# orange-vertex/depthmapX

Hardware: AMD Instinct MI355X
Metric: grid cells/sec for VISPREP makeGraph + VGA global on N×N grid (higher is better)
Workload: dtype f64

## Files before the change

depthmapx_amd/_native.py:

```python
import ctypes
import os

import numpy as np

_HERE = os.path.dirname(os.path.abspath(__file__))
LIB_PATH = os.environ.get("DMX_LIB") or os.path.join(_HERE, "_lib", "libdmx.so")

DMX_OK = 0
STATUS_NAMES = {-1: "DMX_ERR_ARG", -2: "DMX_ERR_HIP", -3: "DMX_ERR_CAPACITY", -4: "DMX_ERR_STATE",
                -5: "DMX_ERR_UNSUPPORTED", -6: "DMX_ERR_OUTSIDE", -7: "DMX_ERR_CANCELLED"}
PROGRESS_FN = ctypes.CFUNCTYPE(ctypes.c_int32, ctypes.c_void_p, ctypes.c_int32, ctypes.c_int64, ctypes.c_int64)

_vp, _i64, _i32, _dbl, _cs = ctypes.c_void_p, ctypes.c_int64, ctypes.c_int, ctypes.c_double, ctypes.c_char_p
SIGNATURES = {
    "dmx_abi_version": (_i32, []),
    "dmx_last_error": (ctypes.c_char_p, []),
    "dmx_ctx_create": (_i32, [_i32, _vp]),
    "dmx_ctx_free": (_i32, [_vp]),
    "dmx_ctx_last_timing": (_i32, [_vp, _vp, _vp]),
    "dmx_ctx_last_stats": (_i32, [_vp, _vp, _i32]),
    "dmx_pointmap_create": (_i32, [_vp, _dbl, _vp, _i64, _vp]),
    "dmx_pointmap_free": (_i32, [_vp]),
    "dmx_pointmap_fill": (_i32, [_vp, _dbl, _dbl, _vp]),
    "dmx_pointmap_fill_device": (_i32, [_vp, _vp, _dbl, _dbl, _vp]),
    "dmx_pointmap_make_points": (_i32, [_vp, _dbl, _dbl, _i32, _vp]),
    "dmx_graph_special_nodes": (_i32, [_vp, _vp, _vp]),
    "dmx_pointmap_make_points_device": (_i32, [_vp, _vp, _dbl, _dbl, _i32, _vp]),
    "dmx_ctx_last_fill": (_i32, [_vp, _vp, _vp, _vp]),
    "dmx_pointmap_info": (_i32, [_vp, _vp, _vp, _vp, _vp, _vp]),
    "dmx_pointmap_state": (_i32, [_vp, _vp]),
    "dmx_pointmap_cell_lines": (_i32, [_vp, _vp, _vp, _vp]),
    "dmx_makegraph": (_i32, [_vp, _vp, _dbl, _i32, _i64, _i64, _vp]),
    "dmx_makegraph_balance": (_i32, [_vp, _vp, _dbl, _i32, _i32, _i64, _vp]),
    "dmx_graph_free": (_i32, [_vp]),
    "dmx_graph_info": (_i32, [_vp, _vp, _vp, _vp, _vp]),
    "dmx_graph_copy": (_i32, [_vp, _vp, _vp, _vp, _vp]),
    "dmx_graph_copy_range": (_i32, [_vp, _i64, _i64, _vp, _vp, _vp, _i64, _vp, _vp]),
    "dmx_graph_blob_size": (_i32, [_vp, _vp]),
    "dmx_graph_blob_write_device": (_i32, [_vp, _vp, _i64]),
    "dmx_graph_assemble_device": (_i32, [_vp, _vp, _vp, _vp, _i32, _vp]),
    "dmx_vga_global": (_i32, [_vp, _vp, _dbl, _i32, _i64, _i64, _vp, _vp]),
    "dmx_vga_global_device": (_i32, [_vp, _vp, _dbl, _i32, _i64, _i64, _vp]),
    "dmx_metric_stepdepth": (_i32, [_vp, _vp, _vp, _i64, _vp]),
    "dmx_visual_stepdepth": (_i32, [_vp, _vp, _vp, _i64, _vp]),
    "dmx_vga_global_device_list": (_i32, [_vp, _vp, _dbl, _i32, _vp, _i64, _vp]),
    "dmx_graph_set_prep_shard": (_i32, [_vp, _i64, _i64, _vp, _vp]),
    "dmx_vga_local": (_i32, [_vp, _vp, _i32, _i64, _i64, _vp]),
    "dmx_vga_thruvision": (_i32, [_vp, _vp, _i64, _i64, _vp, _vp]),
    "dmx_graph_connections": (_i32, [_vp, _vp, _i64, _i64, _i32, _vp, _vp, _i64, _vp]),
    "dmx_graph_connections_csv": (_i32, [_vp, _vp, _i64, _i64, _cs, _vp, _vp, _i64, _vp]),
    "dmx_ctx_last_connections": (_i32, [_vp, _vp, _vp, _vp]),
    "dmx_agent_schedule": (_i32, [_vp, ctypes.c_uint32, _i32, _dbl, _i32, _vp, _i64, _i32, _vp, _vp, _vp, _i64, _vp]),
    "dmx_agents": (_i32, [_vp, _vp, _i32, _i32, _i64, _vp, _vp, _vp, _vp, _vp, _vp, _vp, _vp, _i64]),
    "dmx_ctx_last_agents": (_i32, [_vp, _vp, _vp]),
    "dmx_ctx_last_agents_detail": (_i32, [_vp, _vp, _vp]),
    "dmx_vga_isovist": (_i32, [_vp, _vp, _i32, _i64, _i64, _vp, _vp, _vp, _vp, _i64, _vp]),
    "dmx_ctx_last_isovist": (_i32, [_vp, _vp, _vp, _vp]),
    "dmx_isovists": (_i32, [_vp, _vp, _i64, _vp, _vp, _vp, _i64, _i32, _vp, _vp, _vp, _i64, _vp]),
    "dmx_chunk_occlusion": (_i32, [_vp, _vp, _vp, _vp, _i64, _vp]),
    "dmx_chunk_set_occlusion": (_i32, [_vp, _vp, _vp, _vp]),
    "dmx_vga_metric": (_i32, [_vp, _vp, _dbl, _i32, _i64, _i64, _vp]),
    "dmx_vga_angular": (_i32, [_vp, _vp, _dbl, _i32, _i64, _i64, _vp]),
    "dmx_angular_stepdepth": (_i32, [_vp, _vp, _vp, _i64, _vp]),
    "dmx_release_cached_memory": (_i32, []),
    "dmx_ctx_set_progress": (_i32, [_vp, PROGRESS_FN, _vp, _dbl]),
    "dmx_ctx_cancel": (_i32, [_vp]),
    "dmx_ctx_last_stepdepth": (_i32, [_vp, _vp, _vp, _vp]),
    "dmx_ctx_last_stepdepth_detail": (_i32, [_vp, _vp]),
    "dmx_ctx_last_stepdepth_attempts": (_i32, [_vp, _vp]),
    "dmx_ctx_last_stepdepth_batched": (_i32, [_vp, _vp]),
    "dmx_ctx_last_phase_cycles": (_i32, [_vp, _vp]),
    "dmx_ctx_last_mk_reruns": (_i32, [_vp, _vp, ctypes.c_int64, _vp]),
    "dmx_chunk_write": (_i32, [_vp, _i64, _vp, _vp, _i64, _vp, _i32, _vp, _vp, _vp, _vp, _i32, _i32, _vp, _i64, _vp]),
    "dmx_pointmap_set_state": (_i32, [_vp, _vp]),
    "dmx_chunk_parse": (_i32, [_vp, _i64, _vp]),
    "dmx_chunk_free": (_i32, [_vp]),
    "dmx_chunk_info": (_i32, [_vp, _vp, _vp, _vp, _vp, _vp, _vp, _vp, _vp, _vp]),
    "dmx_chunk_column": (_i32, [_vp, _i32, _vp, _i32, _vp, _vp]),
    "dmx_chunk_arrays": (_i32, [_vp, _vp, _vp, _vp, _vp]),
    "dmx_chunk_load": (_i32, [_vp, _vp, _vp, _vp, _vp]),
    "dmx_graph_from_runs": (_i32, [_vp, _vp, _i64, _vp, _vp, _i64, _vp, _vp, _vp]),
    "dmx_graph_set_merges": (_i32, [_vp, _vp, _i64]),
    "dmx_graph_set_drawing": (_i32, [_vp, _vp, _i64]),
    "dmx_pointmap_set_merges": (_i32, [_vp, _vp, _i64]),
    "dmx_chunk_merges": (_i32, [_vp, _vp, _vp]),
    "dmx_chunk_rows": (_i32, [_vp, _vp, _vp]),
    "dmx_chunk_merge_records": (_i32, [_vp, _vp, _vp]),
    "dmx_chunk_flags": (_i32, [_vp, _vp, _vp, _vp, _vp]),
    "dmx_chunk_set_column": (_i32, [_vp, _cs, _vp, _vp, _i32, _i32]),
    "dmx_chunk_set_displayed": (_i32, [_vp, _i32]),
    "dmx_chunk_set_name": (_i32, [_vp, _cs]),
    "dmx_chunk_select_cells": (_i32, [_vp, _vp, _i64]),
    "dmx_chunk_unmake": (_i32, [_vp, _i32]),
    "dmx_chunk_serialize": (_i32, [_vp, _vp, _i64, _vp]),
    "dmx_graph_chunk_write": (_i32, [_vp, _cs, _i32, _vp, _vp, _vp, _vp, _i32, _i32, _vp, _i64, _vp]),
    "dmx_chunk_scan": (_i32, [_vp, _i64, _vp, _vp, _vp, _vp, _vp]),
    "dmx_chunk_load_bytes": (_i32, [_vp, _vp, _i64, _vp, _vp, _vp]),
    "dmx_graphfile_read": (_i32, [_cs, _vp]),
    "dmx_graphfile_free": (_i32, [_vp]),
    "dmx_graphfile_write": (_i32, [_vp, _cs]),
    "dmx_graphfile_info": (_i32, [_vp, _vp, _vp, _vp, _vp, _vp, _vp]),
    "dmx_graphfile_lines": (_i32, [_vp, _vp]),
    "dmx_graphfile_set_view": (_i32, [_vp, _i32, _i32]),
    "dmx_graphfile_pointmap": (_i32, [_vp, _i32, _vp, _vp]),
    "dmx_graphfile_put_pointmap": (_i32, [_vp, _i32, _vp, _i64]),
    "dmx_graphfile_new_pointmap_name": (_i32, [_vp, _vp, _i32]),
    "dmx_view_vga_top": (_i32, [_i32]),
}


ALLREDUCE_FN = ctypes.CFUNCTYPE(ctypes.c_int, ctypes.c_void_p, ctypes.c_int64, ctypes.c_int, ctypes.c_void_p)


class DmxError(RuntimeError):
    def __init__(self, status, message):
        super().__init__("%s (%d): %s" % (STATUS_NAMES.get(status, "?"), status, message))
        self.status = status


_lib = None


def _share_hip_runtime_with_torch():
    try:
        import torch
    except Exception:
        pass


def lib():
    global _lib
    if _lib is None:
        _share_hip_runtime_with_torch()
        if not os.path.exists(LIB_PATH):
            raise DmxError(-2, "native library %s is missing: run depthmapx_amd.build.build()" % LIB_PATH)
        L = ctypes.CDLL(LIB_PATH)
        for name, (res, args) in SIGNATURES.items():
            if os.environ.get("DMX_LIB") and not hasattr(L, name):
                continue
            fn = getattr(L, name)
            fn.restype = res
            fn.argtypes = args
        _lib = L
    return _lib


def check(status):
    if status != DMX_OK:
        raise DmxError(status, lib().dmx_last_error().decode(errors="replace"))
    return status


def ptr(a):
    return None if a is None else a.ctypes.data_as(ctypes.c_void_p)
```

depthmapx_amd/csrc/api/vga_global.hip:

```cpp

static void prep_range(const dmx_graph* g, int64_t& b, int64_t& e) {
    b = 0; e = g->nnodes;
    if (g->prep_fn && g->prep_e >= 0) { b = g->prep_b; e = g->prep_e; }
}
static int prep_allreduce(dmx_graph* g, void* p, int64_t count, int dtype) {
    if (!g->prep_fn || count <= 0) return DMX_OK;
    HIPCHK(hipStreamSynchronize(g->ctx->stream));
    if (g->prep_fn(p, count, dtype, g->prep_user) != 0)
        return fail(DMX_ERR_STATE, "prep all-reduce callback failed");
    return DMX_OK;
}
static int prepare_symmetry(dmx_graph* g);
static int build_scan_order(dmx_graph* g);
static int prepare_uf(dmx_graph* g) {
    if (g->scan_ready) return DMX_OK;
    if (int rc = prepare_symmetry(g)) return rc;
    dmx_ctx* ctx = g->ctx;
    hipStream_t s = ctx->stream;
    PointMapHost& h = *g->pm->host;
    const int cols = h.cols(), rows = h.rows();
    const int tw = (cols + 7) / 8, th = (rows + 7) / 8;
    const int64_t C = (int64_t)cols * rows, N = g->nnodes;
    DevBuf<int> cov;
    DevBuf<unsigned long long> cnt;
    HIPCHK(cnt.alloc(1));
    HIPCHK(hipMemsetAsync(cnt.p, 0, 8, s));
    const bool have_uf = g->uf_count >= 0;
    if (!have_uf) {
        HIPCHK(cov.alloc((size_t)4 * C));
        HIPCHK(g->uf_tiles.alloc((size_t)tw * th));
        HIPCHK(g->notuf_tiles.alloc((size_t)tw * th));
        HIPCHK(hipMemsetAsync(cov.p, 0, (size_t)4 * C * 4, s));
        int64_t pb, pe;
        prep_range(g, pb, pe);
        if (pe > pb) {
            hipLaunchKernelGGL(cov_scatter_kernel, dim3((unsigned)std::min<int64_t>(pe - pb, 4096)), dim3(256), 0, s,
                               cols, rows, pe - pb, g->node_run_start.p + pb, g->node_nruns.p + pb, g->pool.p, cov.p);
            HIPCHK(hipGetLastError());
        }
        if (int rc = prep_allreduce(g, cov.p, (int64_t)4 * C, DMX_I32)) return rc;
        hipLaunchKernelGGL(cov_lines_kernel, dim3((cols + rows + 127) / 128, 4), dim3(128), 0, s, cols, rows, cov.p);
        HIPCHK(hipGetLastError());
        hipLaunchKernelGGL(cov_tiles_kernel, dim3((tw * th + 255) / 256), dim3(256), 0, s, cols, rows, tw, th,
                           g->pm->d_cell_node.p, cov.p, g->uf_tiles.p, g->notuf_tiles.p, cnt.p);
        HIPCHK(hipGetLastError());
    }
    unsigned long long ufc = have_uf ? (unsigned long long)g->uf_count : 0ull;
    if (!have_uf) HIPCHK(copy_sync(s, &ufc, cnt.p, 8, hipMemcpyDeviceToHost));
    if (int rc = build_scan_order(g)) return rc;
    g->uf_count = (int64_t)ufc;
    g->scan_ready = true;
    return DMX_OK;
}

static int build_scan_order(dmx_graph* g) {
    dmx_ctx* ctx = g->ctx;
    hipStream_t s = ctx->stream;
    PointMapHost& h = *g->pm->host;
    const int rows = h.rows();
    const int64_t C = (int64_t)h.cols() * rows, N = g->nnodes;
    std::vector<int32_t> nr((size_t)std::max<int64_t>(N, 1));
    if (N) HIPCHK(copy_sync(s, nr.data(), g->node_nruns.p, N * 4, hipMemcpyDeviceToHost));
    std::vector<int64_t> ss((size_t)std::max<int64_t>(N, 1));
    int64_t acc = 0;
    for (int64_t k = 0; k < N; k++) { ss[k] = acc; acc += nr[k]; }
    DevBuf<int64_t>& d_ss = g->scan_start;
    HIPCHK(d_ss.alloc(std::max<int64_t>(N, 1)));
    HIPCHK(g->scan_pool.alloc(std::max<int64_t>(acc, 1)));
    HIPCHK(g->cell_scan_start.alloc(C));
    HIPCHK(g->cell_nruns.alloc(C));
    HIPCHK(hipMemsetAsync(g->cell_nruns.p, 0, C * 4, s));
    if (N) {
        HIPCHK(hipMemcpyAsync(d_ss.p, ss.data(), N * 8, hipMemcpyHostToDevice, s));
        hipLaunchKernelGGL(scan_pool_kernel, dim3((unsigned)std::min<int64_t>(N, 8192)), dim3(256), 0, s, rows,
                           g->pm->d_node_cell.p, N, g->node_run_start.p, g->node_nruns.p, g->bin_nruns.p, g->pool.p, d_ss.p,
                           g->scan_pool.p, g->cell_scan_start.p, g->cell_nruns.p);
        HIPCHK(hipGetLastError());
    }
    HIPCHK(hipStreamSynchronize(s));
    g->scan_released = false;
    return DMX_OK;
}

static int restore_scan_order(dmx_graph* g) {
    if (!g->scan_released) return DMX_OK;
    g->pmask.reset(); g->ppre.reset(); g->poff.reset();
    g->tvis.reset(); g->ftvis.reset(); g->tvsum.reset(); g->tvnz.reset(); g->tvblk.reset(); g->ttvis.reset();
    g->tvw = 0;
    g->tiles_ready = false;
    return build_scan_order(g);
}

static int prepare_symmetry(dmx_graph* g) {
    if (g->symmetric >= 0) return DMX_OK;
    const char* force = getenv("DMX_VGA_KERNEL");
    if (force && std::string(force) == "topdown") {
        g->symmetric = 0;
        g->sym_diff.reset(); g->sym_ho.reset(); g->sym_fused = false;
        return DMX_OK;
    }
    dmx_ctx* ctx = g->ctx;
    hipStream_t s = ctx->stream;
    PointMapHost& h = *g->pm->host;
    const int cols = h.cols(), rows = h.rows();
    const int64_t C = (int64_t)cols * rows, N = g->nnodes;
    const int kSpecLimit = 4096;
    DevBuf<unsigned long long> prefix, diff_own, ho_own;
    DevBuf<int32_t> flist;
    DevBuf<int> fcount;
    HIPCHK(flist.alloc(kSpecLimit));
    HIPCHK(fcount.alloc(1));
    HIPCHK(hipMemsetAsync(fcount.p, 0, 4, s));
    const int maxlines = cols + rows;
    unsigned long long *diff = nullptr, *ho = nullptr;
    if (g->sym_fused) {
        diff = g->sym_diff.p;
        ho = g->sym_ho.p;
        ctx->last_stats[39] = 0;
    } else {
        const double t_sym = now_s();
        HIPCHK(prefix.alloc((size_t)4 * C));
        HIPCHK(diff_own.alloc((size_t)4 * C));
        HIPCHK(ho_own.alloc(std::max<int64_t>(N, 1)));
        diff = diff_own.p;
        ho = ho_own.p;
        HIPCHK(hipMemsetAsync(diff, 0, (size_t)4 * C * 8, s));
        HIPCHK(hipMemsetAsync(ho, 0, (size_t)std::max<int64_t>(N, 1) * 8, s));
        hipLaunchKernelGGL(sym_lines_kernel, dim3((maxlines + 127) / 128, 4), dim3(128), 0, s, cols, rows,
                           g->pm->d_cell_node.p, prefix.p, 0);
        HIPCHK(hipGetLastError());
        int64_t pb, pe;
        prep_range(g, pb, pe);
        if (pe > pb) {
            hipLaunchKernelGGL(sym_scatter_kernel, dim3((unsigned)std::min<int64_t>(pe - pb, 4096)), dim3(256), 0, s,
                               cols, rows, g->pm->d_node_cell.p + pb, pe - pb, g->node_run_start.p + pb,
                               g->node_nruns.p + pb, g->pool.p, prefix.p, diff, ho + pb);
            HIPCHK(hipGetLastError());
        }
        if (int rc = prep_allreduce(g, diff, (int64_t)4 * C, DMX_I64)) return rc;
        if (int rc = prep_allreduce(g, ho, N, DMX_I64)) return rc;
        HIPCHK(hipStreamSynchronize(s));
        ctx->last_stats[39] = (long long)((now_s() - t_sym) * 1e6);
    }
    hipLaunchKernelGGL(sym_lines_kernel, dim3((maxlines + 127) / 128, 4), dim3(128), 0, s, cols, rows,
                       g->pm->d_cell_node.p, diff, 1);
    HIPCHK(hipGetLastError());
    if (N) {
        hipLaunchKernelGGL(sym_flag_kernel, dim3((unsigned)((N + 255) / 256)), dim3(256), 0, s, rows,
                           g->pm->d_node_cell.p, N, C, diff, ho, fcount.p, flist.p, kSpecLimit);
        HIPCHK(hipGetLastError());
    }
    const int tw = (cols + 7) / 8, th = (rows + 7) / 8;
    DevBuf<unsigned long long> ufcnt;
    HIPCHK(ufcnt.alloc(1));
    HIPCHK(hipMemsetAsync(ufcnt.p, 0, 8, s));
    HIPCHK(g->uf_tiles.alloc((size_t)tw * th));
    HIPCHK(g->notuf_tiles.alloc((size_t)tw * th));
    hipLaunchKernelGGL(uf_hi_tiles_kernel, dim3((tw * th + 255) / 256), dim3(256), 0, s, cols, rows, tw, th,
                       g->pm->d_cell_node.p, diff, g->uf_tiles.p, g->notuf_tiles.p, ufcnt.p);
    HIPCHK(hipGetLastError());
    int nspec = 0;
    unsigned long long ufc = 0;
    HIPCHK(hipMemcpyAsync(&nspec, fcount.p, 4, hipMemcpyDeviceToHost, s));
    HIPCHK(hipMemcpyAsync(&ufc, ufcnt.p, 8, hipMemcpyDeviceToHost, s));
    HIPCHK(hipStreamSynchronize(s));
    g->sym_diff.reset(); g->sym_ho.reset(); g->sym_fused = false;
    g->uf_count = (int64_t)ufc;
    g->nspecial = nspec;
    if (nspec == 0) { g->symmetric = 1; return DMX_OK; }
    if (nspec > kSpecLimit) { g->symmetric = 0; return DMX_OK; }
    std::vector<int32_t> specs((size_t)nspec);
    HIPCHK(copy_sync(g->ctx->stream, specs.data(), flist.p, nspec * 4, hipMemcpyDeviceToHost));
    std::sort(specs.begin(), specs.end());
    g->special_nodes = specs;
    std::vector<uint8_t> is_spec((size_t)N, 0);
    std::vector<int32_t> sidx((size_t)N, -1);
    for (int i = 0; i < nspec; i++) { is_spec[specs[i]] = 1; sidx[specs[i]] = i; }
    DevBuf<uint8_t> d_is;
    DevBuf<int32_t> d_specs, d_out;
    DevBuf<int> d_outn;
    HIPCHK(d_is.alloc(N));
    HIPCHK(d_specs.alloc(nspec));
    HIPCHK(d_out.alloc((size_t)nspec * nspec));
    HIPCHK(d_outn.alloc(nspec));
    HIPCHK(copy_sync(g->ctx->stream, d_is.p, is_spec.data(), N, hipMemcpyHostToDevice));
    HIPCHK(copy_sync(g->ctx->stream, d_specs.p, specs.data(), nspec * 4, hipMemcpyHostToDevice));
    HIPCHK(hipMemsetAsync(d_outn.p, 0, nspec * 4, s));
    hipLaunchKernelGGL(sym_special_out_kernel, dim3(nspec), dim3(256), 0, s, rows, d_specs.p, nspec,
                       g->pm->d_node_cell.p, g->pm->d_cell_node.p, d_is.p, g->node_run_start.p, g->node_nruns.p,
                       g->pool.p, d_out.p, d_outn.p, nspec);
    HIPCHK(hipGetLastError());
    std::vector<int32_t> outn((size_t)nspec), out((size_t)nspec * nspec);
    HIPCHK(hipMemcpyAsync(outn.data(), d_outn.p, nspec * 4, hipMemcpyDeviceToHost, s));
    HIPCHK(hipMemcpyAsync(out.data(), d_out.p, (size_t)nspec * nspec * 4, hipMemcpyDeviceToHost, s));
    HIPCHK(hipStreamSynchronize(s));
    std::vector<std::vector<char>> A((size_t)nspec, std::vector<char>((size_t)nspec, 0));
    for (int a = 0; a < nspec; a++) {
        if (outn[a] < 0) return fail(DMX_ERR_STATE, "internal: special-node list count out of range");
        for (int j = 0; j < std::min(outn[a], nspec); j++) {
            const int32_t v = out[(size_t)a * nspec + j];
            if (v < 0 || v >= N || sidx[v] < 0) return fail(DMX_ERR_STATE, "internal: special-node list entry out of range");
            A[a][sidx[v]] = 1;
        }
    }
    std::vector<std::vector<int32_t>> extra((size_t)nspec), missing((size_t)nspec);
    for (int a = 0; a < nspec; a++)
        for (int b = 0; b < nspec; b++)
            if (A[a][b] && !A[b][a]) {
                extra[b].push_back(specs[a]);
                missing[a].push_back(specs[b]);
            }
    std::vector<int32_t> eoff(1, 0), moff(1, 0), ev, mv;
    for (int i = 0; i < nspec; i++) {
        ev.insert(ev.end(), extra[i].begin(), extra[i].end());
        mv.insert(mv.end(), missing[i].begin(), missing[i].end());
        eoff.push_back((int32_t)ev.size());
        moff.push_back((int32_t)mv.size());
    }
    HIPCHK(g->spec_index.alloc(N));
    HIPCHK(g->extra_off.alloc(eoff.size()));
    HIPCHK(g->missing_off.alloc(moff.size()));
    HIPCHK(g->extra.alloc(std::max<size_t>(ev.size(), 1)));
    HIPCHK(g->missing.alloc(std::max<size_t>(mv.size(), 1)));
    HIPCHK(copy_sync(g->ctx->stream, g->spec_index.p, sidx.data(), N * 4, hipMemcpyHostToDevice));
    HIPCHK(copy_sync(g->ctx->stream, g->extra_off.p, eoff.data(), eoff.size() * 4, hipMemcpyHostToDevice));
    HIPCHK(copy_sync(g->ctx->stream, g->missing_off.p, moff.data(), moff.size() * 4, hipMemcpyHostToDevice));
    if (!ev.empty()) HIPCHK(copy_sync(g->ctx->stream, g->extra.p, ev.data(), ev.size() * 4, hipMemcpyHostToDevice));
    if (!mv.empty()) HIPCHK(copy_sync(g->ctx->stream, g->missing.p, mv.data(), mv.size() * 4, hipMemcpyHostToDevice));
    g->symmetric = 1;
    return DMX_OK;
}

static int prepare_pmask(dmx_graph* g, int rows, int tw, int th, int tvw, int64_t Ct, bool wide) {
    dmx_ctx* ctx = g->ctx;
    hipStream_t s = ctx->stream;
    DevBuf<int64_t> cnt, scratch;
    HIPCHK(cnt.alloc(Ct));
    HIPCHK(g->poff.alloc(Ct + 1));
    HIPCHK(g->ppre.alloc((size_t)Ct * tvw));
    HIPCHK(scratch.alloc(scan_scratch_size(Ct)));
    hipLaunchKernelGGL(tile_pcount_kernel, dim3((unsigned)((Ct + 3) / 4)), dim3(256), 0, s, Ct, tvw, g->tvis.p, g->ftvis.p,
                       cnt.p, g->ppre.p);
    HIPCHK(hipGetLastError());
    scan_excl(s, cnt.p, Ct, g->poff.p, scratch.p);
    HIPCHK(hipGetLastError());
    int64_t total = 0;
    HIPCHK(copy_sync(s, &total, g->poff.p + Ct, 8, hipMemcpyDeviceToHost));
    size_t free_b = 0, total_b = 0;
    HIPCHK(hipMemGetInfo(&free_b, &total_b));
    const size_t mask_b = (size_t)total * 8;
    bool build = total > 0 && mask_b <= free_b / policy::kMemShareDiv;
    const int pmcap = wide ? PM_CAP_WIDE : PM_CAP;
    if (wide && total > 0 && tile_pmask_lds(tvw, pmcap) <= policy::kLdsPassBudget) {
        const size_t reserve = 16ull << 30;
        const size_t free_all = free_b + cached_bytes();
        const size_t scan_b = g->scan_pool.p ? g->scan_pool.n * sizeof(Run) + (size_t)g->nnodes * 8 +
                                                   (size_t)g->cell_scan_start.n * 12 : 0;
        if (mask_b + reserve <= free_all) {
            build = true;
        } else if (g->scan_pool.p && mask_b + reserve <= free_all + scan_b) {
            g->scan_pool.reset(); g->scan_start.reset(); g->cell_scan_start.reset(); g->cell_nruns.reset();
            g->scan_released = true;
            hipLaunchKernelGGL(tile_pool_order_kernel, dim3((unsigned)((g->nnodes + 255) / 256)), dim3(256), 0, s, rows, tw,
                               g->pm->d_node_cell.p, g->nnodes, g->node_run_start.p, g->tscan_start.p);
            HIPCHK(hipGetLastError());
            VLOG("vga prep: scan order released for %.1f GB of partial-tile masks\n", mask_b / 1e9);
            build = true;
            if (getenv("DMX_VGA_PMASK_FAIL"))
                return fail(DMX_ERR_HIP, "injected failure after the scan order was released");
        } else {
            build = false;
        }
    }
    if (!build) {
        g->poff.reset();
        g->ppre.reset();
        return DMX_OK;
    }
    HIPCHK(g->pmask.alloc((size_t)total));
    HIPCHK(hipMemsetAsync(g->pmask.p, 0, mask_b, s));
    const int64_t N = g->nnodes;
    if (N > 0) {
        const int64_t nb = std::min<int64_t>(N, (int64_t)ctx->num_cu * 16);
        hipLaunchKernelGGL(tile_pmask_kernel, dim3((unsigned)nb), dim3(64 * TV_WAVES), tile_pmask_lds(tvw, pmcap), s, rows,
                           tw, th, g->pm->d_node_cell.p, N, g->node_run_start.p, g->node_nruns.p, g->pool.p, g->tvis.p,
                           g->ftvis.p, g->poff.p, g->pmask.p, pmcap);
        HIPCHK(hipGetLastError());
    }
    return DMX_OK;
}

static void prep_state_stats(dmx_ctx* ctx, const dmx_graph* g) {
    long long f = 0;
    if (g->scan_pool.p) f |= 1;
    if (g->scan_released) f |= 2;
    if (g->tvis.p) f |= 4;
    if (g->ftvis.p) f |= 8;
    if (g->ttvis.p) f |= 16;
    if (g->pmask.p) f |= 32;
    if (g->tvsum.p || g->tvnz.p) f |= 64;
    ctx->last_stats[40] = f;
    ctx->last_stats[41] = (long long)((g->tvis.p ? g->tvis.n * 8 : 0) + (g->ftvis.p ? g->ftvis.n * 8 : 0) +
                                      (g->ttvis.p ? g->ttvis.n * 8 : 0) + (g->tvsum.p ? g->tvsum.n * 8 : 0) + (g->tvnz.p ? g->tvnz.n * 8 : 0) +
                                      (g->tvblk.p ? g->tvblk.n * 8 : 0));
    ctx->last_stats[42] = (long long)(g->scan_pool.p ? g->scan_pool.n * sizeof(Run) : 0);
}

static size_t tile_lds_layout(int tw, int th, bool* fg, bool* rbm) {
    const size_t nt = (size_t)tw * th, wr_ = (tw + 63) / 64, wc_ = (th + 63) / 64;
    const size_t lds_f = nt * 8, lds_h = (size_t)VGA_HMAX * 4;
    const size_t lds_sc = (size_t)(th * wr_ + tw * wc_) * 8, lds_rbcb = (size_t)(th * wr_ + th * 8 * wr_ + tw * 8 * wc_) * 8;
    const size_t lds_cap = (size_t)160 * 1024 - 1024;
    const char* rb_env = getenv("DMX_VGA_RB");
    const bool rb_ok = !(rb_env && atoi(rb_env) == 0);
    *fg = false;
    *rbm = false;
    if (rb_ok && lds_f + lds_rbcb + lds_h <= lds_cap) { *rbm = true; return lds_f + lds_rbcb + lds_h; }
    if (lds_f + lds_sc + lds_h <= lds_cap) return lds_f + lds_sc + lds_h;
    if (rb_ok && lds_rbcb + lds_h <= lds_cap) { *fg = true; *rbm = true; return lds_rbcb + lds_h; }
    if (lds_sc + lds_h <= lds_cap) { *fg = true; return lds_sc + lds_h; }
    return 0;
}

static int prepare_tiles(dmx_graph* g) {
    if (g->tiles_ready) return DMX_OK;
    if (g->scan_released)
        if (int rc = restore_scan_order(g)) return rc;
    dmx_ctx* ctx = g->ctx;
    hipStream_t s = ctx->stream;
    PointMapHost& h = *g->pm->host;
    const int cols = h.cols(), rows = h.rows();
    const int tw = (cols + 7) / 8, th = (rows + 7) / 8, nt = tw * th;
    const int64_t N = g->nnodes, Ct = (int64_t)nt * 64;
    HIPCHK(g->tscan_start.alloc(Ct));
    HIPCHK(g->tnruns.alloc(Ct));
    HIPCHK(g->heads.alloc((size_t)KH * Ct));
    HIPCHK(g->cr.alloc((size_t)CRK * nt));
    HIPCHK(g->regular_tiles.alloc(nt));
    HIPCHK(hipMemsetAsync(g->tnruns.p, 0, Ct * 4, s));
    HIPCHK(hipMemsetAsync(g->tscan_start.p, 0, Ct * 8, s));
    HIPCHK(hipMemsetAsync(g->heads.p, 0xFF, (size_t)KH * Ct * sizeof(Run), s));
    std::vector<unsigned long long> uf((size_t)nt);
    HIPCHK(hipMemcpyAsync(uf.data(), g->uf_tiles.p, nt * 8, hipMemcpyDeviceToHost, s));
    HIPCHK(hipStreamSynchronize(s));
    for (int32_t k : g->special_nodes) {
        const int c = g->pm->node_cell[k];
        const int x = c / rows, y = c % rows;
        uf[(size_t)(y >> 3) * tw + (x >> 3)] &= ~(1ull << ((y & 7) * 8 + (x & 7)));
    }
    HIPCHK(hipMemcpyAsync(g->regular_tiles.p, uf.data(), nt * 8, hipMemcpyHostToDevice, s));
    if (N) {
        hipLaunchKernelGGL(tile_heads_kernel, dim3((unsigned)((N + 255) / 256)), dim3(256), 0, s, rows, tw,
                           g->pm->d_node_cell.p, N, g->node_nruns.p, g->scan_pool.p, g->scan_start.p,
                           g->tscan_start.p, g->tnruns.p, g->heads.p, (size_t)Ct);
        HIPCHK(hipGetLastError());
    }
    const int dmax = std::max(cols, rows);
    const size_t lds = (size_t)8 * (dmax + 2) * 4;
    if (lds > policy::kLdsPassBudget) return fail(DMX_ERR_CAPACITY, "grid too long for the tile-common-run pass");
    hipLaunchKernelGGL(tile_cr_kernel, dim3((unsigned)std::min<int64_t>(nt, (int64_t)ctx->num_cu * 8)), dim3(CR_THREADS),
                       lds, s, cols, rows, tw, th, g->regular_tiles.p, g->pm->d_cell_node.p, g->node_run_start.p,
                       g->node_nruns.p, g->scan_start.p, g->scan_pool.p, g->pool.p, dmax, g->cr.p);
    HIPCHK(hipGetLastError());
    const int tvw = th * ((tw + 63) / 64);
    const size_t tv_bytes = (size_t)Ct * tvw * 8;
    size_t free_b = 0, total_b = 0;
    HIPCHK(hipMemGetInfo(&free_b, &total_b));
    const char* tv_env = getenv("DMX_VGA_TVIS");
    const bool tv_on = !(tv_env && atoi(tv_env) == 0);
    const char* ftv_env = getenv("DMX_VGA_FTVIS");
    const bool ftv_on = !(ftv_env && atoi(ftv_env) == 0);
    const bool wide = tvw > 256;
    const size_t free_all = free_b + cached_bytes();
    bool fg_grid = false, rbm_grid = false;
    tile_lds_layout(tw, th, &fg_grid, &rbm_grid);
    bool ftv = ftv_on && (!wide || (fg_grid && 2 * tv_bytes + (24ull << 30) <= free_all));
    bool tv_build = tv_on && N && tv_bytes <= (32ull << 30) &&
                    (wide ? tv_bytes <= free_all / policy::kMemShareWideDiv : tv_bytes * (ftv ? 2 : 1) <= free_b / policy::kMemShareDiv);
    if (g->prep_fn) {
        DevBuf<int64_t> veto;
        HIPCHK(veto.alloc(1));
        const int64_t v = (tv_build ? 0 : 1) + (ftv ? 0 : (1ll << 20));
        HIPCHK(hipMemcpyAsync(veto.p, &v, 8, hipMemcpyHostToDevice, s));
        if (int rc = prep_allreduce(g, veto.p, 1, DMX_I64)) return rc;
        int64_t vs = 0;
        HIPCHK(copy_sync(g->ctx->stream, &vs, veto.p, 8, hipMemcpyDeviceToHost));
        tv_build = (vs & ((1ll << 20) - 1)) == 0;
        ftv = (vs >> 20) == 0;
    }
    if (tv_build) {
        HIPCHK(g->tvis.alloc(Ct * tvw));
        HIPCHK(hipMemsetAsync(g->tvis.p, 0, tv_bytes, s));
        if (ftv) {
            HIPCHK(g->ftvis.alloc(Ct * tvw));
            HIPCHK(hipMemsetAsync(g->ftvis.p, 0, tv_bytes, s));
        }
        const int ncw = (nt + 3) / 4;
        const size_t tv_lds = ((size_t)(ncw + 1) / 2 + (size_t)(tvw + (ncw + 1) / 2)) * 8;
        if (tv_lds > policy::kLdsPassBudget) return fail(DMX_ERR_CAPACITY, "grid too large for the tile-visibility pass");
        int64_t pb, pe;
        prep_range(g, pb, pe);
        if (pe > pb) {
            const int64_t nb = std::min<int64_t>(pe - pb, (int64_t)ctx->num_cu * 16);
            hipLaunchKernelGGL(tile_vis_kernel, dim3((unsigned)nb), dim3(64 * TV_WAVES), tv_lds, s, rows, tw, th,
                               g->pm->d_node_cell.p + pb, pe - pb, g->node_run_start.p + pb, g->node_nruns.p + pb,
                               g->pool.p, g->notuf_tiles.p, g->tvis.p, ftv ? g->ftvis.p : nullptr);
            HIPCHK(hipGetLastError());
        }
        if (int rc = prep_allreduce(g, g->tvis.p, Ct * tvw, DMX_I64)) return rc;
        if (ftv)
            if (int rc = prep_allreduce(g, g->ftvis.p, Ct * tvw, DMX_I64)) return rc;
        const char* tt_env = getenv("DMX_VGA_TTVIS");
        if (ftv && !(tt_env && atoi(tt_env) == 0)) {
            HIPCHK(g->ttvis.alloc((size_t)2 * nt * tvw));
            hipLaunchKernelGGL(tile_tt_kernel, dim3((unsigned)((nt + 3) / 4)), dim3(256), 0, s, nt, tvw, g->regular_tiles.p,
                               g->ftvis.p, g->tvis.p, g->ttvis.p, g->ttvis.p + (size_t)nt * tvw);
            HIPCHK(hipGetLastError());
        }
        const char* pm_env = getenv("DMX_VGA_PMASK");
        if (ftv && !(pm_env && atoi(pm_env) == 0) && (!wide || ((tvw + 63) / 64 <= 64 && nt <= 65535)))
            if (int rc = prepare_pmask(g, rows, tw, th, tvw, Ct, wide)) return rc;
        if (wide && (tvw + 63) / 64 <= 64) {
            HIPCHK(g->tvsum.alloc((size_t)Ct * ((tvw + 63) / 64)));
            hipLaunchKernelGGL(tile_vsum_kernel, dim3((unsigned)((Ct + 3) / 4)), dim3(256), 0, s, Ct, tvw, g->tvis.p,
                               g->tvsum.p);
            HIPCHK(hipGetLastError());
        }
        const char* nz_env = getenv("DMX_VGA_TVNZ");
        if (VGA_TVNZ && !wide && ftv && g->pmask.p && !(nz_env && atoi(nz_env) == 0)) {
            HIPCHK(g->tvnz.alloc((size_t)Ct * ((tvw + 63) / 64)));
            hipLaunchKernelGGL(tile_vsum_kernel, dim3((unsigned)((Ct + 3) / 4)), dim3(256), 0, s, Ct, tvw, g->tvis.p,
                               g->tvnz.p);
            HIPCHK(hipGetLastError());
        }
        if (!wide && ftv && g->pmask.p && ((tw + 7) / 8) * ((th + 7) / 8) <= 256) {
            HIPCHK(g->tvblk.alloc((size_t)Ct * 4));
            hipLaunchKernelGGL(tile_vblk_kernel, dim3((unsigned)((Ct + 3) / 4)), dim3(256), 0, s, Ct, tvw, (tw + 63) / 64,
                               (tw + 7) / 8, g->tvis.p, g->tvblk.p);
            HIPCHK(hipGetLastError());
        }
        g->tvw = tvw;
    }
    HIPCHK(hipStreamSynchronize(s));
    g->tiles_ready = true;
    return DMX_OK;
}

#ifndef VGA_NT_BIG
#define VGA_NT_BIG 1024
#endif
static int ordered_search(dmx_ctx* ctx, dmx_graph* g, double radius, const std::vector<int32_t>& src,
                          const std::vector<int32_t>& seed_cells, float* outp, int64_t* d_levels, int32_t* d_cell_level) {
    const PointMapHost& h = *g->pm->host;
    const int64_t C = h.cells(), N = g->nnodes;
    const bool vsd = !seed_cells.empty();
    const int64_t nsearch = vsd ? 1 : (int64_t)src.size();
    if (nsearch == 0) return DMX_OK;
    size_t free_b = 0, total_b = 0;
    HIPCHK(hipMemGetInfo(&free_b, &total_b));
    const size_t per = (size_t)C * 5 + (size_t)N * 8;
    const int64_t blocks = std::max<int64_t>(1, std::min<int64_t>({nsearch, (int64_t)ctx->num_cu,
                                                                    (int64_t)((free_b + cached_bytes()) / policy::kMemShareDiv / per)}));
    DevBuf<uint8_t> misc;
    DevBuf<int16_t> ext;
    DevBuf<int32_t> vec, d_src, d_seeds, hist, nlev;
    DevBuf<unsigned long long> junk;
    HIPCHK(misc.alloc((size_t)blocks * C));
    HIPCHK(ext.alloc((size_t)blocks * 2 * C));
    HIPCHK(vec.alloc((size_t)blocks * 2 * std::max<int64_t>(N, 1)));
    OrderedParams P;
    P.rows = h.rows(); P.C = C; P.N = N;
    P.node_run_start = g->node_run_start.p; P.node_nruns = g->node_nruns.p; P.pool = g->pool.p;
    P.cell_node = g->pm->d_cell_node.p; P.node_cell = g->pm->d_node_cell.p; P.node_flags = g->pm->d_node_flags.p;
    P.merge_cell = g->merges.empty() ? nullptr : g->d_merge_cell.p;
    P.src = nullptr; P.nsrc = 0; P.radius = (int)radius; P.hist_all = nullptr; P.nlev_all = nullptr;
    P.hmax = (radius == -1.0) ? 4096 : (int)std::min<double>(4096.0, radius + 2.0);
    P.seeds = nullptr; P.nseeds = 0; P.cell_level = d_cell_level;
    P.misc = misc.p; P.ext = ext.p; P.vec = vec.p;
    P.error = ctx->counters.p + 1;
    P.work_counter = ctx->counters.p + 0;
    P.ctl = ctx->d_ctl;
    ctx->h_ctl->progress = 0;
    HIPCHK(hipMemsetAsync(ctx->counters.p, 0, 2 * sizeof(int), ctx->stream));
    if (vsd) {
        HIPCHK(d_seeds.alloc(seed_cells.size()));
        HIPCHK(hipMemcpyAsync(d_seeds.p, seed_cells.data(), seed_cells.size() * 4, hipMemcpyHostToDevice, ctx->stream));
        P.seeds = d_seeds.p; P.nseeds = (int)seed_cells.size();
    } else {
        HIPCHK(d_src.alloc(src.size()));
        HIPCHK(hist.alloc((size_t)nsearch * P.hmax));
        HIPCHK(nlev.alloc(nsearch));
        HIPCHK(hipMemcpyAsync(d_src.p, src.data(), src.size() * 4, hipMemcpyHostToDevice, ctx->stream));
        P.src = d_src.p; P.nsrc = (int)src.size(); P.hist_all = hist.p; P.nlev_all = nlev.p;
    }
    DevBuf<OrderedParams> dP;
    HIPCHK(dP.alloc(1));
    HIPCHK(hipMemcpyAsync(dP.p, &P, sizeof(P), hipMemcpyHostToDevice, ctx->stream));
    hipLaunchKernelGGL(vga_ordered_kernel, dim3((unsigned)blocks), dim3(ORD_NT), 0, ctx->stream, (const OrderedParams*)dP.p);
    HIPCHK(hipGetLastError());
    HIPCHK(wait_progress(ctx, DMX_PHASE_VGA, nsearch, 1));
    CANCEL_POINT(ctx);
    int err = 0;
    HIPCHK(copy_sync(ctx->stream, &err, ctx->counters.p + 1, sizeof(int), hipMemcpyDeviceToHost));
    if (err) return fail(DMX_ERR_UNSUPPORTED, "VGA BFS in the reference's order deeper than 4096 levels");
    if (!vsd) {
        HIPCHK(junk.alloc(32));
        hipLaunchKernelGGL(vga_measures_kernel, dim3((unsigned)((nsearch + 255) / 256)), dim3(256), 0, ctx->stream,
                           (int64_t)0, nsearch, hist.p, nlev.p, outp, d_levels, junk.p, (const int32_t*)d_src.p, P.hmax, true);
        HIPCHK(hipGetLastError());
    }
    HIPCHK(hipStreamSynchronize(ctx->stream));
    VLOG("reference-order searches: %lld on %lld workgroups\n", (long long)nsearch, (long long)blocks);
    return DMX_OK;
}

static int vga_order_rerun(dmx_ctx* ctx, dmx_graph* g, double radius, const uint8_t* d_oflag, float* outp,
                           int64_t* d_levels) {
    const int64_t N = g->nnodes;
    std::vector<uint8_t> fl((size_t)N);
    HIPCHK(copy_sync(ctx->stream, fl.data(), d_oflag, (size_t)N, hipMemcpyDeviceToHost));
    std::vector<int32_t> src;
    for (int64_t k = 0; k < N; k++)
        if (fl[k]) src.push_back((int32_t)k);
    const double t0 = now_s();
    int rc = ordered_search(ctx, g, radius, src, {}, outp, d_levels, nullptr);
    ctx->last_vga_s += now_s() - t0;
    ctx->last_stats[38] = (int64_t)src.size();
    return rc;
}

extern "C++" template <int NT, bool SPECIAL, bool RBM, bool FG>
static int launch_tile(dmx_ctx* ctx, const VgaTileParams& Q, int64_t nsrc, size_t lds, int64_t* blocks_out,
                       DevBuf<unsigned long long>& xg, DevBuf<int4>& queue, DevBuf<int32_t>& list) {
    {
        const int64_t nt = (int64_t)Q.tw * Q.th;
        const char* why = nullptr;
        if (Q.tw != (Q.cols + 7) / 8 || Q.th != (Q.rows + 7) / 8 || nt <= 0) why = "tile grid does not cover the cells";
        else if (lds > (size_t)160 * 1024) why = "dynamic LDS above 160 KiB";
        else if (!FG && (size_t)nt * 8 > lds) why = "frontier bitmap larger than the dynamic LDS";
        else if (Q.tvis && Q.tvw != Q.th * ((Q.tw + 63) / 64)) why = "tile-visibility row width differs from the tile grid";
        else if (!FG && Q.pmask && Q.tvw > 256) why = "row words past the fused phase-C test (256)";
        else if (Q.tvnz && (FG || Q.tvw > 256)) why = "narrow row summaries on a wide grid";
        else if (Q.tvblk && (FG || ((Q.tw + 7) / 8) * ((Q.th + 7) / 8) > 256)) why = "tile-block summaries past 256 blocks";
        else if (Q.pmask && !FG && nt > 32767) why = "narrow mask hint: tile index above 15 bits";
        else if (Q.asym_tiles && Q.alist_cap <= 0) why = "asymmetric mode without an A-cell list";
        if (why) return fail(DMX_ERR_STATE, (std::string("VGA tile launch: ") + why).c_str());
        hipFuncAttributes fa;
        HIPCHK(hipFuncGetAttributes(&fa, reinterpret_cast<const void*>(&vga_tile_kernel<NT, SPECIAL, RBM, FG>)));
        if (fa.sharedSizeBytes + lds > (size_t)160 * 1024)
            return fail(DMX_ERR_STATE, "VGA tile launch: static plus dynamic LDS above 160 KiB");
    }
    int occ = 0;
    HIPCHK(hipOccupancyMaxActiveBlocksPerMultiprocessor(&occ, vga_tile_kernel<NT, SPECIAL, RBM, FG>, NT, lds));
    if (occ < 1) occ = 1;
    const int64_t blocks = std::max<int64_t>(1, std::min<int64_t>((int64_t)ctx->num_cu * occ, nsrc));
    const int64_t nt = (int64_t)Q.tw * Q.th;
    HIPCHK(xg.alloc((size_t)blocks * (FG ? 3 : 2) * nt));
// ... 394 lines not shown
    DevBuf<int32_t> frontier;
    HIPCHK(frontier.alloc((size_t)blocks * 2 * std::max<int64_t>(N, 1)));
    DevBuf<unsigned long long> gbm_buf;
    if (gbm) HIPCHK(gbm_buf.alloc((size_t)blocks * 3 * tw * th));
    DevBuf<float> d_out;
    float* outp = out;
    if (!out_on_device) {
        HIPCHK(d_out.alloc(std::max<int64_t>(N, 1) * 7));
        outp = d_out.p;
    }
    DevBuf<int64_t> d_lv;
    if (levels) HIPCHK(d_lv.alloc(std::max<int64_t>(N, 1) * 3));
    HIPCHK(hipMemsetAsync(ctx->counters.p, 0, 16 * sizeof(int), ctx->stream));
    HIPCHK(hipMemsetAsync(ctx->stats.p, 0, 32 * sizeof(unsigned long long), ctx->stream));
    VgaParams P;
    P.cols = h.cols(); P.rows = h.rows(); P.tw = tw; P.th = th;
    P.seed_tiles = g->pm->d_seed_tiles.p; P.uf_tiles = g->uf_tiles.p; P.uf_count = g->uf_count;
    P.node_cell = g->pm->d_node_cell.p; P.cell_node = g->pm->d_cell_node.p; P.node_flags = g->pm->d_node_flags.p;
    P.node_run_start = g->node_run_start.p; P.node_nruns = g->node_nruns.p; P.pool = g->pool.p;
    P.src_begin = sb; P.src_end = se; P.radius = (int)radius; P.gates_only = gates_only;
    P.work_counter = ctx->counters.p + 0; P.error = ctx->counters.p + 1;
    P.frontier = frontier.p; P.nnodes = N; P.maxlev = maxlev;
    P.out = outp; P.levels_out = levels ? d_lv.p : nullptr;
    P.stats = ctx->stats.p;
    VgaDoParams Q;
    Q.cols = h.cols(); Q.rows = h.rows(); Q.tw = tw; Q.th = th;
    Q.seed_tiles = g->notuf_tiles.p; Q.uf_tiles = g->uf_tiles.p; Q.nonexp_tiles = g->pm->d_nonexp_tiles.p;
    Q.node_cell = P.node_cell; Q.cell_node = P.cell_node; Q.node_flags = P.node_flags;
    Q.node_run_start = P.node_run_start; Q.node_nruns = P.node_nruns; Q.pool = P.pool;
    Q.cell_scan_start = g->cell_scan_start.p; Q.cell_nruns = g->cell_nruns.p; Q.scan_pool = g->scan_pool.p;
    Q.src_begin = sb; Q.src_end = se; Q.radius = P.radius; Q.gates_only = gates_only;
    Q.uf_count = g->uf_count; Q.symmetric = g->symmetric;
    const bool corr = g->symmetric == 1 && g->nspecial > 0;
    Q.spec_index = corr ? g->spec_index.p : nullptr;
    Q.extra_off = corr ? g->extra_off.p : nullptr;
    Q.extra = corr ? g->extra.p : nullptr;
    Q.missing_off = corr ? g->missing_off.p : nullptr;
    Q.missing = corr ? g->missing.p : nullptr;
    Q.alpha = policy::hook_int("DMX_VGA_ALPHA", policy::kVgaDoAlpha);
    Q.kshort = policy::hook_int("DMX_VGA_KSHORT", policy::kVgaDoShortList);
    Q.work_counter = P.work_counter; Q.scratch = frontier.p; Q.nnodes = N; Q.maxlev = maxlev;
    Q.out = outp; Q.levels_out = P.levels_out; Q.error = P.error; Q.stats = P.stats;
    Q.gbm = gbm ? gbm_buf.p : nullptr;
    Q.nmp = (int)(g->merges.size() / 2);
    Q.mpairs = Q.nmp ? g->d_mpairs.p : nullptr;
    if (!use_do && Q.nmp) return fail(DMX_ERR_UNSUPPORTED, "the top-down v1 kernel does not follow merge links");
    Q.nmamb = Q.nmp && radius != -1.0 ? g->nmamb : 0;
    Q.mamb = Q.nmamb ? g->d_mamb.p : nullptr;
    DevBuf<int32_t> mseen;
    DevBuf<uint8_t> oflag;
    if (Q.nmamb) {
        HIPCHK(mseen.alloc((size_t)blocks * Q.nmamb));
        HIPCHK(hipMemsetAsync(mseen.p, 0, (size_t)blocks * Q.nmamb * 4, ctx->stream));
        Q.mseen = mseen.p;
        HIPCHK(oflag.alloc(N));
        HIPCHK(hipMemsetAsync(oflag.p, 0, (size_t)N, ctx->stream));
        Q.oflag = oflag.p;
    }
    HIPCHK(hipEventRecord(ctx->ev0, ctx->stream));
    if (nsrc > 0) {
        if (gbm) hipLaunchKernelGGL(vga_do_kernel<true>, dim3((unsigned)blocks), dim3(DO_THREADS), lds, ctx->stream, Q);
        else if (use_do) hipLaunchKernelGGL(vga_do_kernel<false>, dim3((unsigned)blocks), dim3(DO_THREADS), lds, ctx->stream, Q);
        else hipLaunchKernelGGL(vga_global_kernel, dim3((unsigned)blocks), dim3(VGA_THREADS), lds, ctx->stream, P);
        HIPCHK(hipGetLastError());
    }
    HIPCHK(hipEventRecord(ctx->ev1, ctx->stream));
    ctx->h_ctl->progress = 0;
    HIPCHK(wait_progress(ctx, DMX_PHASE_VGA, nsrc, 1));
    CANCEL_POINT(ctx);
    float ms = 0;
    HIPCHK(hipEventElapsedTime(&ms, ctx->ev0, ctx->ev1));
    ctx->last_vga_s = ms * 1e-3;
    int hc[2];
    HIPCHK(copy_sync(ctx->stream, hc, ctx->counters.p, sizeof(hc), hipMemcpyDeviceToHost));
    if (hc[1] & ~KERR_ORDER) return fail(DMX_ERR_CAPACITY, "VGA BFS exceeded its level/frontier capacity");
    ctx->last_stats[38] = 0;
    if (hc[1] & KERR_ORDER)
        if (int rc2 = vga_order_rerun(ctx, g, radius, oflag.p, outp, P.levels_out)) return rc2;
    unsigned long long st[8];
    HIPCHK(copy_sync(ctx->stream, st, ctx->stats.p, sizeof(st), hipMemcpyDeviceToHost));
    ctx->last_stats[8] = (long long)st[5];
    ctx->last_stats[9] = (long long)st[6];
    ctx->last_stats[10] = gbm ? 1 : 0;
    for (int i = 13; i < 24; i++) ctx->last_stats[i] = 0;
    ctx->last_stats[3] = (long long)(use_do ? (g->symmetric ? 2 : 1) : 0) | ((long long)g->nspecial << 8);
    ctx->last_stats[4] = (long long)st[0];
    ctx->last_stats[5] = (long long)(st[3] | (st[4] << 32));
    ctx->last_stats[6] = (long long)st[2];
    ctx->last_stats[7] = nsrc;
    if (!out_on_device && nsrc > 0)
        HIPCHK(copy_sync(ctx->stream, out + sb * 7, d_out.p + sb * 7, nsrc * 7 * 4, hipMemcpyDeviceToHost));
    if (levels && nsrc > 0)
        HIPCHK(copy_sync(ctx->stream, levels + sb * 3, d_lv.p + sb * 3, nsrc * 3 * 8, hipMemcpyDeviceToHost));
    return DMX_OK;
}

int dmx_vga_global(dmx_ctx* ctx, dmx_graph* g, double radius, int gates_only, int64_t sb, int64_t se, float* out,
                   int64_t* levels) {
    SAME_DEVICE(ctx, g);
    if (int rc = prepare_merges(g)) return rc;
    return vga_impl(ctx, g, radius, gates_only, sb, se, out, false, levels);
}

int dmx_vga_global_device(dmx_ctx* ctx, dmx_graph* g, double radius, int gates_only, int64_t sb, int64_t se,
                          float* out_device) {
    SAME_DEVICE(ctx, g);
    if (int rc = prepare_merges(g)) return rc;
    return vga_impl(ctx, g, radius, gates_only, sb, se, out_device, true, nullptr);
}

int dmx_vga_global_device_list(dmx_ctx* ctx, dmx_graph* g, double radius, int gates_only, const int64_t* nodes,
                               int64_t n, float* out_device) {
    SAME_DEVICE(ctx, g);
    if (!ctx || !g || !out_device || (n > 0 && !nodes)) return fail(DMX_ERR_ARG, "bad arguments");
    if (int rc = prepare_merges(g)) return rc;
    if (g->node_begin != 0 || g->node_end != g->nnodes)
        return fail(DMX_ERR_STATE, "VGA needs the whole graph (assemble the shards first)");
    HIPCHK(hipSetDevice(ctx->device));
    const int64_t N = g->nnodes;
    std::vector<int32_t> lst((size_t)std::max<int64_t>(n, 1));
    for (int64_t i = 0; i < n; i++) {
        if (nodes[i] < 0 || nodes[i] >= N) return fail(DMX_ERR_ARG, "source node out of range");
        lst[i] = (int32_t)nodes[i];
    }
    int rc = prepare_uf(g);
    if (rc) return rc;
    rc = prepare_symmetry(g);
    if (rc) return rc;
    PointMapHost& h = *g->pm->host;
    const int tw = (h.cols() + 7) / 8, th = (h.rows() + 7) / 8;
    if (g->symmetric == 1 && !ctx->tile_disabled) {
        DevBuf<int32_t> d_list;
        HIPCHK(d_list.alloc(lst.size()));
        HIPCHK(hipMemcpyAsync(d_list.p, lst.data(), lst.size() * 4, hipMemcpyHostToDevice, ctx->stream));
        rc = vga_tile_impl(ctx, g, radius, gates_only, 0, n, out_device, true, nullptr, tw, th, nullptr, 0, nullptr, d_list.p);
        if (rc != DMX_ERR_CAPACITY) return rc;
    }
    const bool was_disabled = ctx->tile_disabled;
    ctx->tile_disabled = true;
    double total = 0.0;
    for (int64_t i = 0; i < n;) {
        int64_t j = i + 1;
        while (j < n && lst[j] == lst[j - 1] + 1) j++;
        rc = vga_impl(ctx, g, radius, gates_only, lst[i], (int64_t)lst[j - 1] + 1, out_device, true, nullptr);
        if (rc) break;
        total += ctx->last_vga_s;
        i = j;
    }
    ctx->tile_disabled = was_disabled;
    if (rc) return rc;
    ctx->last_vga_s = total;
    return DMX_OK;
}
```

depthmapx_amd/csrc/dmx_api.hip:

```cpp
#include <hip/hip_runtime.h>

#include <execinfo.h>
#include <signal.h>
#include <unistd.h>

#include <algorithm>
#include <array>
#include <chrono>
#include <cstdio>
#include <cstring>
#include <map>
#include <memory>
#include <mutex>
#include <string>
#include <thread>
#include <vector>

#include "../../include/dmx.h"
#include "policy.hpp"
#include "host/bsptree.hpp"
#include "host/graphfile.hpp"
#include "host/graphio.hpp"
#include "host/pointmap.hpp"
#include "kernels/makegraph.hip"
// ... 9 lines not shown
#include "kernels/isovist.hip"
#include "kernels/isovist_points.hip"
#include "kernels/chunk_codec.hip"
#include "kernels/connections.hip"
#include "kernels/agents.hip"

using namespace dmx;

namespace {
thread_local std::string g_err;
double now_s() {
    return std::chrono::duration<double>(std::chrono::steady_clock::now().time_since_epoch()).count();
}
bool verbose() {
    static int v = -1;
    if (v < 0) {
        const char* e = getenv("DMX_VERBOSE");
        v = (e && *e && strcmp(e, "0") != 0) ? 1 : 0;
    }
    return v == 1;
}
#define VLOG(...)                                      \
    do {                                               \
        if (verbose()) fprintf(stderr, "[dmx] " __VA_ARGS__); \
    } while (0)
hipError_t copy_sync(hipStream_t s, void* dst, const void* src, size_t bytes, hipMemcpyKind kind) {
    hipError_t e = hipMemcpyAsync(dst, src, bytes, kind, s);
    if (e != hipSuccess) return e;
    return hipStreamSynchronize(s);
}
int fail(int code, const std::string& msg) {
    g_err = msg;
    return code;
}
#define HIPCHK(expr)                                                                              \
    do {                                                                                          \
        hipError_t e_ = (expr);                                                                   \
        if (e_ != hipSuccess) return fail(DMX_ERR_HIP, std::string(#expr) + ": " + hipGetErrorString(e_)); \
    } while (0)

struct BlockCache {
    static constexpr size_t kMin = 64ull << 20;
    std::mutex m;
    std::multimap<std::pair<int, size_t>, void*> free_blocks;
    std::map<void*, std::pair<int, size_t>> live;
    size_t cached = 0;
    void release_all() {
        for (auto& kv : free_blocks) (void)hipFree(kv.second);
        free_blocks.clear();
        cached = 0;
    }
    size_t cached_on(int dev) const {
        size_t b = 0;
        for (auto it = free_blocks.lower_bound({dev, 0}); it != free_blocks.end() && it->first.first == dev; ++it)
            b += it->first.second;
        return b;
    }
};
BlockCache& block_cache() {
    static BlockCache* c = new BlockCache();
    return *c;
}
size_t cached_bytes() {
    BlockCache& c = block_cache();
    int dev = 0;
    (void)hipGetDevice(&dev);
    std::lock_guard<std::mutex> g(c.m);
    return c.cached_on(dev);
}
hipError_t cached_malloc(void** p, size_t bytes) {
    BlockCache& c = block_cache();
    int dev = 0;
    (void)hipGetDevice(&dev);
    if (bytes >= BlockCache::kMin) {
        bool hit = false;
        {
            std::lock_guard<std::mutex> g(c.m);
            auto it = c.free_blocks.lower_bound({dev, bytes});
            if (it != c.free_blocks.end() && it->first.first == dev && it->first.second - it->first.second / 8 <= bytes) {
                *p = it->second;
                c.cached -= it->first.second;
                c.live[*p] = it->first;
                c.free_blocks.erase(it);
                hit = true;
            }
        }
        if (hit) return hipDeviceSynchronize();
    }
    hipError_t e = hipMalloc(p, bytes);
    if (e != hipSuccess) {
        std::lock_guard<std::mutex> g(c.m);
        if (c.cached) {
            (void)hipGetLastError();
            c.release_all();
            e = hipMalloc(p, bytes);
        }
    }
    if (e == hipSuccess && bytes >= BlockCache::kMin) {
        std::lock_guard<std::mutex> g(c.m);
        c.live[*p] = {dev, bytes};
    }
    return e;
}
void cached_free(void* p) {
    BlockCache& c = block_cache();
    {
        std::lock_guard<std::mutex> g(c.m);
        auto it = c.live.find(p);
        if (it != c.live.end()) {
            c.free_blocks.insert({it->second, p});
            c.cached += it->second.second;
            c.live.erase(it);
            return;
        }
    }
    (void)hipFree(p);
}

template <typename T> struct DevBuf {
    T* p = nullptr;
    size_t n = 0;
    ~DevBuf() { reset(); }
    void reset() {
        if (p) cached_free(p);
        p = nullptr;
        n = 0;
    }
    hipError_t alloc(size_t count) {
        if (count <= n && p) return hipSuccess;
        reset();
        hipError_t e = cached_malloc((void**)&p, std::max<size_t>(count, 1) * sizeof(T));
        if (e == hipSuccess) n = count;
        return e;
    }
};
}

struct dmx_ctx {
    int device = 0;
    bool tile_disabled = false;
    hipStream_t stream = nullptr;
    hipStream_t codec_stream = nullptr;
    hipEvent_t ev0 = nullptr, ev1 = nullptr;
    int num_cu = 0;
    double last_mk_s = 0, last_vga_s = 0, last_sd_s = 0;
    long long last_sd_stats[3] = {0, 0, 0};
    int last_sd_attempts = 0;
    long long last_sd_extra[2] = {0, 0};
    int last_sd_mode = 0;
    long long last_sd_batched[5] = {0, 0, 0, 0, 0};
    long long phase_cycles[5] = {0, 0, 0, 0, 0};
    DevBuf<int> counters;
    DevBuf<unsigned long long> stats;
    long long last_stats[51] = {};
    std::vector<int64_t> last_mk_reruns;
    DmxCtl* h_ctl = nullptr;
    DmxCtl* d_ctl = nullptr;
    dmx_progress_fn progress = nullptr;
    void* progress_user = nullptr;
    double progress_interval = 0.5;
    hipEvent_t ev_poll = nullptr;
    double last_fill_s[2] = {0, 0};
    double last_iso_bsp_s = 0, last_iso_kernel_s = 0;
    long long last_iso[4] = {0, 0, 0, 0};
    double sqrt_err = 0.0;
    long long sqrt_err_nmax = 0;
    long long last_fill_levels = 0;
    double last_conn_s[2] = {0, 0};
    long long last_conn[4] = {0, 0, 0, 0};
    double last_agents_s = 0, last_agents_host_s = 0;
    long long last_agents[7] = {};
};

struct dmx_pointmap {
    std::unique_ptr<PointMapHost> host;
    int uploaded_for = -1;
    uint64_t version = 1, uploaded_version = 0;
    int wall_sides = 0;
    bool uploaded_nowall = false;
    int64_t nnodes = 0;
    std::vector<int32_t> node_cell;
    DevBuf<uint32_t> d_cellw;
    DevBuf<double> d_segs;
    DevBuf<int32_t> d_node_cell;
    DevBuf<int32_t> d_cell_node;
    DevBuf<uint8_t> d_node_flags;
    DevBuf<unsigned long long> d_seed_tiles;
    DevBuf<unsigned long long> d_nonexp_tiles;
};

struct dmx_graph {
    dmx_ctx* ctx = nullptr;
    dmx_pointmap* pm = nullptr;
    std::vector<int32_t> merges;
    bool merges_ready = false;
    DevBuf<int2> d_mpairs;
    DevBuf<int2> d_mamb;
    int nmamb = 0;
    DevBuf<int32_t> d_merge_cell;
    int64_t nnodes = 0, node_begin = 0, node_end = 0;
    int64_t nruns = 0;
    DevBuf<Run> pool;
    DevBuf<int64_t> node_run_start;
    DevBuf<int32_t> node_nruns;
    DevBuf<int32_t> bin_nruns;
    DevBuf<uint16_t> bin_count;
    DevBuf<float> bin_dist;
    DevBuf<float> attrs;
    DevBuf<uint8_t> gridconn;
    DevBuf<unsigned long long> uf_tiles;
    DevBuf<unsigned long long> notuf_tiles;
    int64_t uf_count = -1;
    bool scan_ready = false;
    bool scan_released = false;
    DevBuf<Run> scan_pool;
    DevBuf<int64_t> cell_scan_start;
    DevBuf<int32_t> cell_nruns;
    DevBuf<int64_t> scan_start;
    int symmetric = -1;
    int nspecial = 0;
    std::vector<int32_t> special_nodes;
    DevBuf<int32_t> spec_index, extra_off, extra, missing_off, missing;
    DevBuf<unsigned long long> sym_prefix, sym_diff, sym_ho;
    bool sym_fused = false;
    bool tiles_ready = false;
    DevBuf<int64_t> tscan_start;
    DevBuf<int32_t> tnruns;
    DevBuf<Run> heads, cr;
    DevBuf<unsigned long long> tvis;
    DevBuf<unsigned long long> ftvis;
    DevBuf<unsigned long long> ttvis;
    DevBuf<unsigned long long> tvsum;
    DevBuf<unsigned long long> tvnz;
    DevBuf<unsigned long long> tvblk;
    DevBuf<unsigned long long> pmask;
    DevBuf<int64_t> poff;
    DevBuf<uint16_t> ppre;
    int tvw = 0;
    DevBuf<unsigned long long> regular_tiles;
    int64_t prep_b = 0, prep_e = -1;
    dmx_allreduce_fn prep_fn = nullptr;
    void* prep_user = nullptr;
    std::vector<double> drawing;
    bool has_drawing = false;
    int asym_state = 0;
    std::string asym_why;
    std::unique_ptr<dmx_pointmap> aref_pm;
    std::unique_ptr<dmx_graph> aref;
    DevBuf<unsigned long long> asym_tiles;
    int64_t nasym = 0;
    ~dmx_graph();
};
dmx_graph::~dmx_graph() = default;

namespace {

void inherit_merges(dmx_graph* g) {
    const std::vector<int32_t>& pc = g->pm->host->merge();
    g->merges.clear();
    for (size_t c = 0; c < pc.size(); c++)
        if (pc[c] > (int32_t)c) { g->merges.push_back((int32_t)c); g->merges.push_back(pc[c]); }
    g->merges_ready = false;
}

int prepare_merges(dmx_graph* g) {
    if (!g || g->merges_ready || g->merges.empty()) return DMX_OK;
    HIPCHK(hipSetDevice(g->ctx->device));
    const PointMapHost& h = *g->pm->host;
    const int64_t C = h.cells(), m = (int64_t)g->merges.size() / 2;
    const auto& st = h.state();
    const int rows = h.rows();
    auto cf_odd = [&](int32_t c) {
        const int x = c / rows, y = c % rows;
        return (st[c] & CELL_CONTEXTFILLED) && !((x % 2) == 0 && (y % 2) == 0);
    };
    std::vector<int32_t> per_cell((size_t)C, -1);
    std::vector<int2> pairs((size_t)m), amb;
    for (int64_t i = 0; i < m; i++) {
        const int32_t a = g->merges[2 * i], b = g->merges[2 * i + 1];
        if (!(st[a] & CELL_FILLED) || !(st[b] & CELL_FILLED)) return fail(DMX_ERR_ARG, "merge link to a cell without a node");
        per_cell[a] = b;
        per_cell[b] = a;
        pairs[i] = make_int2(a, b);
        if (cf_odd(a) != cf_odd(b)) amb.push_back(cf_odd(a) ? make_int2(a, b) : make_int2(b, a));
    }
    HIPCHK(g->d_mpairs.alloc(m));
    HIPCHK(g->d_merge_cell.alloc(C));
    HIPCHK(hipMemcpyAsync(g->d_mpairs.p, pairs.data(), m * sizeof(int2), hipMemcpyHostToDevice, g->ctx->stream));
    HIPCHK(hipMemcpyAsync(g->d_merge_cell.p, per_cell.data(), C * 4, hipMemcpyHostToDevice, g->ctx->stream));
    g->nmamb = (int)amb.size();
    if (g->nmamb) {
        HIPCHK(g->d_mamb.alloc(amb.size()));
        HIPCHK(hipMemcpyAsync(g->d_mamb.p, amb.data(), amb.size() * sizeof(int2), hipMemcpyHostToDevice, g->ctx->stream));
    }
    HIPCHK(hipStreamSynchronize(g->ctx->stream));
    g->merges_ready = true;
    return DMX_OK;
}

static void clean_distance(const PointMapHost& h, std::vector<uint32_t>& cellw, int sides) {
    const int W = h.cols(), H = h.rows();
    std::vector<uint32_t> d((size_t)W * H);
    for (int x = 0; x < W; x++)
        for (int y = 0; y < H; y++) {
            const size_t c = (size_t)x * H + y;
            const bool clean = (cellw[c] & 0xFFu) == 1u;
            const bool online = ((sides & 1) && x == 0) || ((sides & 2) && x == W - 1) || ((sides & 4) && y == 0) ||
                                ((sides & 8) && y == H - 1);
            const bool wallc = online && (cellw[c] & 0xFFu) == 2u;
            uint32_t b = CELL_DIST_MAX;
            if (!(sides & 1)) b = std::min(b, (uint32_t)(x + 1));
            if (!(sides & 2)) b = std::min(b, (uint32_t)(W - x));
            if (!(sides & 4)) b = std::min(b, (uint32_t)(y + 1));
            if (!(sides & 8)) b = std::min(b, (uint32_t)(H - y));
            d[c] = (clean || wallc) ? b : 0u;
        }
    for (int x = 0; x < W; x++)
        for (int y = 0; y < H; y++) {
            const size_t c = (size_t)x * H + y;
            uint32_t v = d[c];
            if (!v) continue;
            if (y > 0) v = std::min(v, d[c - 1] + 1);
            if (x > 0) {
                const size_t l = c - H;
                v = std::min(v, d[l] + 1);
                if (y > 0) v = std::min(v, d[l - 1] + 1);
                if (y + 1 < H) v = std::min(v, d[l + 1] + 1);
            }
            d[c] = v;
        }
    for (int x = W - 1; x >= 0; x--)
        for (int y = H - 1; y >= 0; y--) {
            const size_t c = (size_t)x * H + y;
            uint32_t v = d[c];
            if (!v) continue;
            if (y + 1 < H) v = std::min(v, d[c + 1] + 1);
            if (x + 1 < W) {
                const size_t r = c + H;
                v = std::min(v, d[r] + 1);
                if (y > 0) v = std::min(v, d[r - 1] + 1);
                if (y + 1 < H) v = std::min(v, d[r + 1] + 1);
            }
            d[c] = v;
        }
    for (size_t c = 0; c < d.size(); c++)
        if ((cellw[c] & 0xFFu) == 1u) cellw[c] = (std::min(d[c], CELL_DIST_MAX) << 8) | 1u;
}

static int closed_sides(int W, int H, const std::vector<uint32_t>& cellw) {
    if (W < 3 || H < 3) return 0;
    int sides = 15;
    for (int y = 1; y < H - 1; y++) {
        if (cellw[(size_t)y] & 1u) sides &= ~1;
        if (cellw[(size_t)(W - 1) * H + y] & 1u) sides &= ~2;
    }
    for (int x = 1; x < W - 1; x++) {
        if (cellw[(size_t)x * H] & 1u) sides &= ~4;
        if (cellw[(size_t)x * H + H - 1] & 1u) sides &= ~8;
    }
    return sides;
}

int upload_pointmap(dmx_ctx* ctx, dmx_pointmap* pm) {
    PointMapHost& h = *pm->host;
    if (!h.lines_blocked()) h.block_lines();
    const bool nowall = getenv("DMX_MK_NOWALL") != nullptr;
    if (pm->uploaded_version == pm->version && pm->uploaded_for == ctx->device && pm->uploaded_nowall == nowall) return DMX_OK;
    if (pm->uploaded_for >= 0 && pm->uploaded_for != ctx->device) {
        pm->d_cellw.reset(); pm->d_segs.reset(); pm->d_node_cell.reset(); pm->d_cell_node.reset();
        pm->d_node_flags.reset(); pm->d_seed_tiles.reset(); pm->d_nonexp_tiles.reset();
        pm->uploaded_for = -1;
// ... 94 lines not shown
}

size_t makegraph_lds(int gcap, int bcap, int D) {
    size_t b = 0;
    b += 16 * (size_t)gcap * 2 + 16 * (size_t)bcap;
    b += 4 * 32 * 3 + 4 * 32;
    b += 16 * (size_t)bcap;
    b += 4 * (size_t)gcap + 8 * (size_t)gcap + 4 * (size_t)bcap + 4 * ((size_t)gcap + 4);
    b += 4 * (size_t)std::min(D + 4, MK_OPEN_LDS);
    return (b + 15) & ~(size_t)15;
}

}

namespace {
struct sigaction g_prev_abrt, g_prev_segv;
void dmx_crash_handler(int sig, siginfo_t* info, void* uc) {
    void* frames[64];
    const int n = backtrace(frames, 64);
    const char hdr[] = "[dmx] native backtrace:\n";
    (void)!write(2, hdr, sizeof(hdr) - 1);
    backtrace_symbols_fd(frames, n, 2);
    struct sigaction* prev = sig == SIGABRT ? &g_prev_abrt : &g_prev_segv;
    sigaction(sig, prev, nullptr);
    if (prev->sa_flags & SA_SIGINFO) {
        if (prev->sa_sigaction) prev->sa_sigaction(sig, info, uc);
    } else if (prev->sa_handler != SIG_DFL && prev->sa_handler != SIG_IGN) {
        prev->sa_handler(sig);
    }
    raise(sig);
}
void install_crash_handler() {
    static bool done = false;
    const char* e = getenv("DMX_ABORT_BACKTRACE");
    if (done || !e || strcmp(e, "1") != 0) return;
    done = true;
    void* warm[2];
    backtrace(warm, 2);
    struct sigaction sa;
    memset(&sa, 0, sizeof(sa));
    sa.sa_sigaction = dmx_crash_handler;
    sa.sa_flags = SA_SIGINFO;
    sigemptyset(&sa.sa_mask);
    sigaction(SIGABRT, &sa, &g_prev_abrt);
    sigaction(SIGSEGV, &sa, &g_prev_segv);
}
}

extern "C" {

int dmx_abi_version(void) { return DMX_ABI_VERSION; }
const char* dmx_last_error(void) { return g_err.c_str(); }

int dmx_ctx_create(int device, dmx_ctx** out) {
    if (!out) return fail(DMX_ERR_ARG, "out is NULL");
    int ndev = 0;
    HIPCHK(hipGetDeviceCount(&ndev));
    if (device < 0 || device >= ndev) return fail(DMX_ERR_ARG, "device ordinal out of range");
    HIPCHK(hipSetDevice(device));
    install_crash_handler();
    auto* c = new dmx_ctx();
    c->device = device;
    hipDeviceProp_t prop;
    HIPCHK(hipGetDeviceProperties(&prop, device));
    c->num_cu = prop.multiProcessorCount;
    HIPCHK(hipStreamCreateWithFlags(&c->stream, hipStreamNonBlocking));
    HIPCHK(hipEventCreate(&c->ev0));
    HIPCHK(hipEventCreate(&c->ev1));
    HIPCHK(c->counters.alloc(16));
    HIPCHK(c->stats.alloc(32));
    HIPCHK(hipEventCreateWithFlags(&c->ev_poll, hipEventDisableTiming));
    HIPCHK(hipHostMalloc((void**)&c->h_ctl, sizeof(DmxCtl), hipHostMallocMapped | hipHostMallocCoherent));
    std::memset(c->h_ctl, 0, sizeof(DmxCtl));
    HIPCHK(hipHostGetDevicePointer((void**)&c->d_ctl, c->h_ctl, 0));
    *out = c;
    return DMX_OK;
}

int dmx_ctx_set_progress(dmx_ctx* ctx, dmx_progress_fn fn, void* user, double interval_s) {
    if (!ctx || interval_s != interval_s) return fail(DMX_ERR_ARG, "bad arguments");
    ctx->progress = fn;
    ctx->progress_user = user;
    ctx->progress_interval = interval_s > 0.0 ? interval_s : 0.5;
    return DMX_OK;
}

int dmx_ctx_cancel(dmx_ctx* ctx) {
    if (!ctx || !ctx->h_ctl) return fail(DMX_ERR_ARG, "bad context");
    __atomic_store_n(&ctx->h_ctl->cancel, 1, __ATOMIC_SEQ_CST);
    return DMX_OK;
}

static hipError_t wait_progress(dmx_ctx* ctx, int32_t phase, int64_t total, int64_t unit) {
    if (!ctx->progress) return hipStreamSynchronize(ctx->stream);
    hipError_t e = hipEventRecord(ctx->ev_poll, ctx->stream);
    if (e != hipSuccess) return e;
    double next = now_s() + ctx->progress_interval;
    for (;;) {
        e = hipEventQuery(ctx->ev_poll);
        if (e == hipSuccess) break;
        if (e != hipErrorNotReady) return e;
        if (now_s() >= next) {
            const int64_t done = std::min<int64_t>(total, (int64_t)__atomic_load_n(&ctx->h_ctl->progress,
                                                                                  __ATOMIC_RELAXED) * unit);
            if (ctx->progress(ctx->progress_user, phase, done, total)) dmx_ctx_cancel(ctx);
            next = now_s() + ctx->progress_interval;
        }
        std::this_thread::sleep_for(std::chrono::microseconds(500));
    }
    if (!__atomic_load_n(&ctx->h_ctl->cancel, __ATOMIC_SEQ_CST) && ctx->progress(ctx->progress_user, phase, total, total))
        dmx_ctx_cancel(ctx);
    return hipSuccess;
}

static bool take_cancel(dmx_ctx* ctx) {
    if (!__atomic_load_n(&ctx->h_ctl->cancel, __ATOMIC_SEQ_CST)) return false;
    __atomic_store_n(&ctx->h_ctl->cancel, 0, __ATOMIC_SEQ_CST);
    return true;
}
#define SAME_DEVICE(ctx, g)                                                                          \
    do {                                                                                             \
        if ((ctx) && (g) && (g)->ctx && (g)->ctx->device != (ctx)->device)                           \
            return fail(DMX_ERR_ARG, "graph was built on another device than the context's");        \
    } while (0)
#define CANCEL_POINT(ctx)                                                        \
    do {                                                                         \
        if (take_cancel(ctx)) return fail(DMX_ERR_CANCELLED, "operation cancelled"); \
    } while (0)

int dmx_release_cached_memory(void) {
    BlockCache& c = block_cache();
    std::lock_guard<std::mutex> g(c.m);
    c.release_all();
    return DMX_OK;
}

int dmx_ctx_free(dmx_ctx* c) {
    if (!c) return DMX_OK;
    (void)hipSetDevice(c->device);
    c->counters.reset();
    c->stats.reset();
    if (c->ev0) (void)hipEventDestroy(c->ev0);
    if (c->ev1) (void)hipEventDestroy(c->ev1);
    if (c->ev_poll) (void)hipEventDestroy(c->ev_poll);
    if (c->h_ctl) (void)hipHostFree(c->h_ctl);
    if (c->codec_stream) (void)hipStreamDestroy(c->codec_stream);
    if (c->stream) (void)hipStreamDestroy(c->stream);
    delete c;
    return DMX_OK;
}

int dmx_ctx_last_stats(dmx_ctx* c, int64_t* out, int n) {
    if (!c || !out) return fail(DMX_ERR_ARG, "bad arguments");
    for (int i = 0; i < n && i < 51; i++) out[i] = c->last_stats[i];
    return DMX_OK;
}

int dmx_ctx_last_timing(dmx_ctx* c, double* mk, double* vga) {
    if (!c) return fail(DMX_ERR_ARG, "ctx is NULL");
    if (mk) *mk = c->last_mk_s;
    if (vga) *vga = c->last_vga_s;
    return DMX_OK;
}

#include "api/pointmap.hip"
#include "api/makegraph.hip"
#include "api/shard.hip"
#include "api/vga_global.hip"
#include "api/vga_other.hip"
#include "api/thruvision.hip"
#include "api/connections.hip"
#include "api/agents.hip"
#include "api/isovist.hip"
#include "api/isovist_points.hip"
#include "api/stepdepth.hip"
#include "api/chunk.hip"
#include "api/graphfile.hip"

}
```

depthmapx_amd/csrc/kernels/vga_do.hip:

```cpp
#include "common.hpp"

namespace dmx {

struct VgaDoParams {
    int cols, rows, tw, th;
    const unsigned long long* seed_tiles;
    const unsigned long long* uf_tiles;
    const unsigned long long* nonexp_tiles;
    const int32_t* node_cell;
    const int32_t* cell_node;
    const uint8_t* node_flags;
    const int64_t* node_run_start;
    const int32_t* node_nruns;
    const Run* pool;
    const int64_t* cell_scan_start;
    const int32_t* cell_nruns;
    const Run* scan_pool;
    int64_t src_begin, src_end;
    int radius, gates_only;
    int64_t uf_count;
    int symmetric;
    const int32_t* spec_index;
    const int32_t* extra_off;
    const int32_t* extra;
// ... 427 lines not shown
                                   unsigned long long* diff, unsigned long long* ho) {
    const int64_t C = (int64_t)cols * rows;
    for (int64_t k = blockIdx.x; k < n; k += gridDim.x) {
        const int c = node_cell[k];
        const unsigned long long su = cell_weight((unsigned long long)c);
        const int64_t rs = node_run_start[k];
        const int nr = node_nruns[k];
        unsigned long long acc = 0;
        for (int r = threadIdx.x; r < nr; r += blockDim.x) acc += sym_run_scatter(pool[rs + r], su, cols, rows, prefix, diff);
        for (int off = 32; off >= 1; off >>= 1) acc += __shfl_xor(acc, off);
        __shared__ unsigned long long red[16];
        if ((threadIdx.x & 63) == 0) red[threadIdx.x >> 6] = acc;
        __syncthreads();
        if (threadIdx.x == 0) {
            unsigned long long t = 0;
            for (int w = 0; w < (int)(blockDim.x >> 6); w++) t += red[w];
            ho[k] = t;
        }
        __syncthreads();
    }
}

__global__ void sym_flag_kernel(int rows, const int32_t* node_cell, int64_t n, int64_t C, const unsigned long long* hi4,
                                const unsigned long long* ho, int* count, int32_t* list, int cap) {
    const int64_t k = (int64_t)blockIdx.x * blockDim.x + threadIdx.x;
    if (k >= n) return;
    const int64_t c = node_cell[k];
    const unsigned long long hi = hi4[c] + hi4[C + c] + hi4[2 * C + c] + hi4[3 * C + c];
    if (hi != ho[k]) {
        const int pos = atomicAdd(count, 1);
        if (pos < cap) list[pos] = (int32_t)k;
    }
}

__global__ void cov_scatter_kernel(int cols, int rows, int64_t n, const int64_t* node_run_start, const int32_t* node_nruns,
                                   const Run* pool, int* diff) {
    const int64_t C = (int64_t)cols * rows;
    for (int64_t k = blockIdx.x; k < n; k += gridDim.x) {
        const int64_t rs = node_run_start[k];
        const int nr = node_nruns[k];
        for (int r = threadIdx.x; r < nr; r += blockDim.x) {
            const Run ru = pool[rs + r];
            const int dir = run_dir(ru);
            int dx, dy;
            dir_step(dir, dx, dy);
            const int ex = ru.x1 + dx, ey = ru.y1 + dy;
            int* D = diff + (int64_t)dir * C;
            atomicAdd(&D[(int64_t)ru.x0 * rows + ru.y0], 1);
            if (ex >= 0 && ex < cols && ey >= 0 && ey < rows) atomicAdd(&D[(int64_t)ex * rows + ey], -1);
        }
    }
}
__global__ void cov_lines_kernel(int cols, int rows, int* arr) {
    const int64_t C = (int64_t)cols * rows;
    const int dir = blockIdx.y;
    const int line = blockIdx.x * blockDim.x + threadIdx.x;
    int x, y, dx, dy;
    if (!line_start(dir, line, cols, rows, x, y)) return;
    dir_step(dir, dx, dy);
    int* A = arr + (int64_t)dir * C;
    int acc = 0;
    for (; x >= 0 && x < cols && y >= 0 && y < rows; x += dx, y += dy) {
        const int64_t c = (int64_t)x * rows + y;
        acc += A[c];
        A[c] = acc;
    }
}
__global__ void cov_tiles_kernel(int cols, int rows, int tw, int th, const int32_t* cell_node, const int* cov,
                                 unsigned long long* uf, unsigned long long* notuf, unsigned long long* count) {
    const int64_t C = (int64_t)cols * rows;
    const int t = blockIdx.x * blockDim.x + threadIdx.x;
    if (t >= tw * th) return;
    const int tx = t % tw, ty = t / tw;
    unsigned long long w = 0;
    for (int b = 0; b < 64; b++) {
        const int x = tx * 8 + (b & 7), y = ty * 8 + (b >> 3);
        if (x >= cols || y >= rows) continue;
        const int64_t c = (int64_t)x * rows + y;
        if (cell_node[c] >= 0 && (cov[c] + cov[C + c] + cov[2 * C + c] + cov[3 * C + c]) > 0) w |= 1ull << b;
    }
    uf[t] = w;
    notuf[t] = ~w;
    if (w) atomicAdd(count, (unsigned long long)__popcll(w));
}

__global__ void uf_hi_tiles_kernel(int cols, int rows, int tw, int th, const int32_t* cell_node,
                                   const unsigned long long* hi4, unsigned long long* uf, unsigned long long* notuf,
                                   unsigned long long* count) {
    const int64_t C = (int64_t)cols * rows;
    const int t = blockIdx.x * blockDim.x + threadIdx.x;
    if (t >= tw * th) return;
    const int tx = t % tw, ty = t / tw;
    unsigned long long w = 0;
    for (int b = 0; b < 64; b++) {
        const int x = tx * 8 + (b & 7), y = ty * 8 + (b >> 3);
        if (x >= cols || y >= rows) continue;
        const int64_t c = (int64_t)x * rows + y;
        if (cell_node[c] >= 0 && (hi4[c] + hi4[C + c] + hi4[2 * C + c] + hi4[3 * C + c]) != 0ull) w |= 1ull << b;
    }
    uf[t] = w;
    notuf[t] = ~w;
    if (w) atomicAdd(count, (unsigned long long)__popcll(w));
}

__global__ void scan_pool_kernel(int rows, const int32_t* node_cell, int64_t n, const int64_t* node_run_start,
                                 const int32_t* node_nruns, const int32_t* bin_nruns, const Run* pool,
                                 const int64_t* scan_start, Run* scan_pool, int64_t* cell_scan_start, int32_t* cell_nruns) {
    __shared__ int cnt[8][16], cur[8][16], ng[8], pre[33];
    for (int64_t k = blockIdx.x; k < n; k += gridDim.x) {
        const int64_t rs = node_run_start[k], ss = scan_start[k];
        const int nr = node_nruns[k];
        if (threadIdx.x < 128) cnt[threadIdx.x >> 4][threadIdx.x & 15] = 0;
        if (threadIdx.x < 32) pre[threadIdx.x + 1] = bin_nruns[k * 32 + threadIdx.x];
        if (threadIdx.x == 0) pre[0] = 0;
        __syncthreads();
        if (threadIdx.x == 0)
            for (int b = 1; b <= 32; b++) pre[b] += pre[b - 1];
        __syncthreads();
        for (int r = threadIdx.x; r < nr; r += blockDim.x) {
            int b = 0;
            while (pre[b + 1] <= r) b++;
            const Run ru = pool[rs + r];
            const int len = max(ru.x1 - ru.x0, max(ru.y1 - ru.y0, ru.y0 - ru.y1)) + 1;
            atomicAdd(&cnt[b >> 2][15 - min(15, 31 - __clz(len))], 1);
        }
        __syncthreads();
        if (threadIdx.x < 8) {
            const int g = threadIdx.x;
            int acc = 0;
            for (int b = 0; b < 16; b++) { cur[g][b] = acc; acc += cnt[g][b]; }
            ng[g] = acc;
        }
        if (threadIdx.x == 0) {
            const int c = node_cell[k];
            cell_scan_start[c] = ss;
            cell_nruns[c] = nr;
        }
        __syncthreads();
        for (int r = threadIdx.x; r < nr; r += blockDim.x) {
            int b = 0;
            while (pre[b + 1] <= r) b++;
            const int g = b >> 2;
            const Run ru = pool[rs + r];
            const int len = max(ru.x1 - ru.x0, max(ru.y1 - ru.y0, ru.y0 - ru.y1)) + 1;
            const int p = atomicAdd(&cur[g][15 - min(15, 31 - __clz(len))], 1);
            int idx = 0;
            for (int h = 0; h < 8; h++) idx += min(p, ng[h]) + ((h < g && ng[h] > p) ? 1 : 0);
            scan_pool[ss + idx] = ru;
        }
        __syncthreads();
    }
}

__global__ void sym_special_out_kernel(int rows, const int32_t* specials, int nspec, const int32_t* node_cell,
                                       const int32_t* cell_node, const uint8_t* is_special, const int64_t* node_run_start,
                                       const int32_t* node_nruns, const Run* pool, int32_t* out, int* out_n, int cap) {
    const int si = blockIdx.x;
    if (si >= nspec) return;
    const int k = specials[si];
    const int64_t rs = node_run_start[k];
    const int nr = node_nruns[k];
    for (int r = threadIdx.x; r < nr; r += blockDim.x) {
        const Run ru = pool[rs + r];
        int dx, dy;
        dir_step(run_dir(ru), dx, dy);
        int x = ru.x0, y = ru.y0;
        for (;;) {
            const int v = cell_node[(int64_t)x * rows + y];
            if (v >= 0 && is_special[v]) {
                const int pos = atomicAdd(&out_n[si], 1);
                if (pos < cap) out[(int64_t)si * cap + pos] = v;
            }
            if (x == ru.x1 && y == ru.y1) break;
            x += dx;
            y += dy;
        }
    }
}

}
```

depthmapx_amd/csrc/kernels/vga_tile.hip:

```cpp
#include "common.hpp"

namespace dmx {

constexpr int KH = 8;
constexpr int CRK = 4;
constexpr int BEXT_DEFAULT = 0;
constexpr int VGA_HMAX = 64;

struct VgaTileParams {
    int cols, rows, tw, th;
    const unsigned long long* seed_tiles;
    const unsigned long long* regular_tiles;
    const unsigned long long* nonexp_tiles;
    const Run* cr;
    const Run* heads;
    const int64_t* tscan_start;
    const int32_t* tnruns;
    const Run* scan_pool;
    const unsigned long long* tvis;
    const unsigned long long* ftvis;
    const unsigned long long* ttvis;
    const unsigned long long* ttany;
    const unsigned long long* pmask;
    const int64_t* poff;
// ... 1845 lines not shown
                        if (!RBM) atomicOr(&Fsc[tx * wc + (ty >> 6)], 1ull << (ty & 63));
                    }
                }
                F[t] = x;
                }
                const unsigned long long om = __ballot(open);
                if (om) {
                    int base = 0;
                    if (lane == 0) base = atomicAdd(&S.tn[(level + 1) & 1], __popcll(om));
                    base = __shfl(base, 0);
                    if (open) TLn[base + lanes_below(om)] = t;
                }
            }
            for (int off = 32; off >= 1; off >>= 1) {
                c_loc += __shfl_xor(c_loc, off);
                m_loc += __shfl_xor(m_loc, off);
            }
            if (lane == 0 && c_loc) { atomicAdd(&S.cnt, c_loc); atomicAdd(&S.mass, m_loc); }
            if (P.nmp && (P.radius == -1 || level + 1 < P.radius)) {
                __syncthreads();
                merge_level_pass(P.mpairs, P.nmp, rows, tw, NT, F, Vg, false, P.seed_tiles, Fsr, RBM ? nullptr : Fsc, wr,
                                 wc, P.cell_level, level + 1, &S.mcorr, &S.mdisc, &S.mass);
                if (P.nmamb && !seeded) {
                    __syncthreads();
                    merge_order_check(P.mamb, P.nmamb, rows, tw, NT, F, Vg, false, P.seed_tiles,
                                      P.mseen + (size_t)blockIdx.x * P.nmamb, (int32_t)node + 1, P.error, P.oflag, node);
                }
            }
            if (RBM) {
                __syncthreads();
                const int th = P.th;
                for (int i = tid; i < th * wr + tw * wc; i += NT) {
                    unsigned long long b[8];
#pragma unroll
                    for (int k = 0; k < 8; k++) b[k] = 0ull;
                    if (i < th * wr) {
                        const int ty = i / wr, w = i % wr;
                        const unsigned long long* fr = F + ty * tw + w * 64;
                        for (unsigned long long m = Fsr[ty * wr + w]; m; m &= m - 1) {
                            const int j = __ffsll((long long)m) - 1;
                            const unsigned long long f = fr[j];
#pragma unroll
                            for (int k = 0; k < 8; k++) b[k] |= (unsigned long long)(((f >> (8 * k)) & 0xFFull) != 0ull) << j;
                        }
#pragma unroll
                        for (int k = 0; k < 8; k++) RB[(ty * 8 + k) * wr + w] = b[k];
                    } else {
                        const int q = i - th * wr, tx = q / wc, w = q % wc;
                        const int n = min(64, th - w * 64);
                        for (int j = 0; j < n; j++) {
                            unsigned long long y = F[(w * 64 + j) * tw + tx];
                            y |= y >> 32;
                            y |= y >> 16;
                            y |= y >> 8;
#pragma unroll
                            for (int k = 0; k < 8; k++) b[k] |= ((y >> k) & 1ull) << j;
                        }
#pragma unroll
                        for (int k = 0; k < 8; k++) CB[(tx * 8 + k) * wc + w] = b[k];
                    }
                }
            }
            sync_global();
            if (!FG && P.tvblk && tid < P.th * wr) {
                const unsigned long long fw = Fsr[tid];
                if (fw) {
                    int wd;
                    unsigned long long lo, hi;
                    blk_place(fw, tid, wr, (tw + 7) >> 3, wd, lo, hi);
                    atomicOr(&S.fblk[wd], lo);
                    if (hi) atomicOr(&S.fblk[min(wd + 1, 3)], hi);
                }
            }
            const long long cnt = uni64(S.cnt), mass = uni64(S.mass);
            const long long mcorr = uni64(S.mcorr), mdisc = uni64(S.mdisc);
            if (tid == 0) { const unsigned long long n = __builtin_amdgcn_s_memtime(); ST(12, n - tmark); tmark = n; }
            __syncthreads();
            if (tid == 0) {
                S.cnt = 0; S.mass = 0; S.qn = 0; S.hn = 0; S.item = 0; S.bn = 0; S.mcorr = 0; S.mdisc = 0;
                S.q2n = 0; S.b2n = 0; S.en = 0; S.eitem = 0;
                S.tn[level & 1] = 0;
                S.disc += cnt + mdisc;
                S.m_u -= cnt + mdisc;
                S.m_f = mass;
            }
            __syncthreads();
            if (cnt == 0) break;
            if (level + 1 >= VGA_HMAX) { overflow = true; break; }
            if (tid == 0) hist[level + 1] = (int)(cnt - mcorr);
            level++;
            nlev = level + 1;
            if (tid == 0) ST(bottom_up ? 3 : 4, 1);
        }
        __syncthreads();
        if (overflow) {
            if (tid == 0) { atomicOr(P.error, KERR_LEVELS); P.nlev_out[node] = 0; }
            continue;
        }
        {
            unsigned r = rt;
            for (int off = 32; off >= 1; off >>= 1) r += __shfl_xor(r, off);
            if (lane == 0 && r) ST(0, r);
            rt = 0;
            unsigned m = nlt;
            for (int off = 32; off >= 1; off >>= 1) m += __shfl_xor(m, off);
            if (lane == 0 && m) ST(30, m);
            nlt = 0;
        }
        for (int l = tid; l < nlev; l += NT) P.hist_out[node * VGA_HMAX + l] = hist[l];
        if (tid == 0) P.nlev_out[node] = nlev;
        __syncthreads();
    }
    for (int off = 32; off >= 1; off >>= 1) rt += __shfl_xor(rt, off);
    if (lane == 0 && rt) ST(0, rt);
    for (int off = 32; off >= 1; off >>= 1) nlt += __shfl_xor(nlt, off);
    if (lane == 0 && nlt) ST(30, nlt);
    __syncthreads();
    for (int i = tid; i < 32; i += NT)
        if (SC[i]) {
            if (i == 23 || (VGA_CSTAT && i == 22)) atomicMax(&P.stats[i], SC[i]);
            else atomicAdd(&P.stats[i], SC[i]);
        }
#undef ST
}

__device__ __forceinline__ int run_len(Run ru) {
    return max(ru.x1 - ru.x0, max(ru.y1 - ru.y0, ru.y0 - ru.y1)) + 1;
}

__global__ void tile_heads_kernel(int rows, int tw, const int32_t* node_cell, int64_t n, const int32_t* node_nruns,
                                  const Run* scan_pool, const int64_t* scan_start, int64_t* tscan_start, int32_t* tnruns,
                                  Run* heads, size_t hstride) {
    const int64_t k = (int64_t)blockIdx.x * blockDim.x + threadIdx.x;
    if (k >= n) return;
    const int c = node_cell[k];
    const int id = tile_id_of(c / rows, c % rows, tw);
    const int64_t ss = scan_start[k];
    const int nr = node_nruns[k];
    tscan_start[id] = ss;
    tnruns[id] = nr;
    int o = 0;
    for (int pass = 0; pass < 2; pass++)
        for (int h = 0; h < KH && h < nr; h++) {
            const Run ru = scan_pool[ss + h];
            const bool diag = ru.x0 != ru.x1 && ru.y0 != ru.y1;
            if (diag == (pass == 1)) heads[(o++) * hstride + id] = ru;
        }
}

constexpr int TV_WAVES = 8;
__device__ __forceinline__ void tv_count(uint32_t* cnt, int t, int c) {
    atomicAdd(&cnt[t >> 2], (uint32_t)c << (8 * (t & 3)));
}
__global__ void __launch_bounds__(64 * TV_WAVES) tile_vis_kernel(int rows, int tw, int th, const int32_t* node_cell,
                                                                 int64_t n, const int64_t* node_run_start,
                                                                 const int32_t* node_nruns, const Run* pool,
                                                                 const unsigned long long* seed_tiles,
                                                                 unsigned long long* tvis, unsigned long long* ftvis) {
    extern __shared__ __attribute__((aligned(16))) unsigned long long tvlds[];
    const int nt = tw * th, ncw = (nt + 3) / 4;
    const int wr = (tw + 63) / 64, tvw = th * wr;
    constexpr int TB = 64 * TV_WAVES;
    const int tid = threadIdx.x;
    uint8_t* nsc = (uint8_t*)tvlds;
    unsigned long long* row = tvlds + (ncw + 1) / 2;
    uint32_t* cnt = (uint32_t*)(row + tvw);
    if (ftvis)
        for (int t = tid; t < nt; t += TB) nsc[t] = (uint8_t)__popcll(~seed_tiles[t]);
    for (int64_t k = blockIdx.x; k < n; k += gridDim.x) {
        __syncthreads();
        for (int w = tid; w < tvw; w += TB) row[w] = 0ull;
        if (ftvis)
            for (int w = tid; w < ncw; w += TB) cnt[w] = 0u;
        __syncthreads();
        const int64_t rs = node_run_start[k];
        const int nr = node_nruns[k];
        for (int r = tid; r < nr; r += TB) {
            const Run ru = pool[rs + r];
            if (ru.y0 == ru.y1) {
                const int y = ru.y0, ty = y >> 3, t0 = ru.x0 >> 3, t1 = ru.x1 >> 3;
                for (int w = t0 >> 6; w <= (t1 >> 6); w++) {
                    const int lo = max(t0 - w * 64, 0), hi = min(t1 - w * 64, 63);
                    atomicOr(&row[ty * wr + w], (~0ull << lo) & (~0ull >> (63 - hi)));
                }
                if (ftvis)
                    for (int tx = t0; tx <= t1; tx++) {
                        const int a = max((int)ru.x0, tx * 8) & 7, b = min((int)ru.x1, tx * 8 + 7) & 7;
                        const unsigned long long m = (unsigned long long)((0xFFu >> (7 - b)) & (0xFFu << a) & 0xFFu) << ((y & 7) * 8);
                        const int t = ty * tw + tx;
                        const int c = __popcll(m & ~seed_tiles[t]);
                        if (c) tv_count(cnt, t, c);
                    }
            } else if (ru.x0 == ru.x1) {
                const int x = ru.x0, tx = x >> 3;
                const unsigned long long colm = 0x0101010101010101ull << (x & 7);
                for (int ty = ru.y0 >> 3; ty <= (ru.y1 >> 3); ty++) {
                    atomicOr(&row[ty * wr + (tx >> 6)], 1ull << (tx & 63));
                    if (ftvis) {
                        const int a = max((int)ru.y0, ty * 8) & 7, b = min((int)ru.y1, ty * 8 + 7) & 7;
                        const unsigned long long m = colm & (~0ull >> (8 * (7 - b))) & (~0ull << (8 * a));
                        const int t = ty * tw + tx;
                        const int c = __popcll(m & ~seed_tiles[t]);
                        if (c) tv_count(cnt, t, c);
                    }
                }
            } else {
                const int dy = (ru.y1 > ru.y0) ? 1 : -1;
                int x = ru.x0, y = ru.y0;
                while (x <= ru.x1) {
                    int n;
                    const unsigned long long m = diag_tile_mask(x, y, dy, ru.x1, n);
                    const int tx = x >> 3, ty = y >> 3;
                    atomicOr(&row[ty * wr + (tx >> 6)], 1ull << (tx & 63));
                    if (ftvis) {
                        const int t = ty * tw + tx;
                        const int c = __popcll(m & ~seed_tiles[t]);
                        if (c) tv_count(cnt, t, c);
                    }
                    x += n;
                    y += dy * n;
                }
            }
        }
        __syncthreads();
        const int c = node_cell[k];
        const int id = tile_id_of(c / rows, c % rows, tw);
        unsigned long long* out = tvis + (size_t)id * tvw;
        for (int w = tid; w < tvw; w += TB) out[w] = row[w];
        if (ftvis) {
            unsigned long long* fout = ftvis + (size_t)id * tvw;
            for (int w = tid; w < tvw; w += TB) {
                unsigned long long m = row[w], f = 0ull;
                const int tyw = w / wr, tx0 = (w % wr) * 64;
                while (m) {
                    const int j = __ffsll((long long)m) - 1;
                    m &= m - 1;
                    const int t = tyw * tw + tx0 + j;
                    const int cv = (cnt[t >> 2] >> (8 * (t & 3))) & 0xFF;
                    if (cv == nsc[t] && cv > 0) f |= 1ull << j;
                }
                fout[w] = f;
            }
        }
    }
}

__global__ void tile_pcount_kernel(int64_t Ct, int tvw, const unsigned long long* tvis, const unsigned long long* ftvis,
                                   int64_t* pcount, uint16_t* ppre) {
    const int lane = threadIdx.x & 63;
    const int64_t id = (int64_t)blockIdx.x * (blockDim.x >> 6) + (threadIdx.x >> 6);
    if (id >= Ct) return;
    int run = 0;
    for (int k = 0; k * 64 < tvw; k++) {
        const int w = k * 64 + lane;
        const int c = w < tvw ? __popcll(tvis[id * tvw + w] & ~ftvis[id * tvw + w]) : 0;
        const int incl = wave_incl_scan(c);
        if (w < tvw) ppre[id * tvw + w] = (uint16_t)(run + incl - c);
        run += __builtin_amdgcn_readlane(incl, 63);
    }
    if (lane == 0) pcount[id] = run;
}

constexpr int PM_CAP = 4096;
constexpr int PM_CAP_WIDE = 8192;
__host__ __device__ inline size_t tile_pmask_lds(int tvw, int pmcap) { return (size_t)tvw * 12 + (size_t)pmcap * 8; }
__global__ void __launch_bounds__(64 * TV_WAVES) tile_pmask_kernel(int rows, int tw, int th, const int32_t* node_cell,
                                                                   int64_t n, const int64_t* node_run_start,
                                                                   const int32_t* node_nruns, const Run* pool,
                                                                   const unsigned long long* tvis,
                                                                   const unsigned long long* ftvis, const int64_t* poff,
                                                                   unsigned long long* pmask, int pmcap) {
    extern __shared__ __attribute__((aligned(16))) unsigned long long pmlds[];
    __shared__ int ptotal;
    const int wr = (tw + 63) / 64, tvw = th * wr;
    unsigned long long* part = pmlds;
    unsigned long long* lm = part + tvw;
    int* pre = (int*)(lm + pmcap);
    constexpr int TB = 64 * TV_WAVES;
    const int tid = threadIdx.x, lane = tid & 63;
    for (int64_t k = blockIdx.x; k < n; k += gridDim.x) {
        const int c = node_cell[k];
        const int id = tile_id_of(c / rows, c % rows, tw);
        __syncthreads();
        if (tid < 64) {
            int run = 0;
            for (int kk = 0; kk * 64 < tvw; kk++) {
                const int w = kk * 64 + lane;
                const unsigned long long p = w < tvw ? (tvis[(size_t)id * tvw + w] & ~ftvis[(size_t)id * tvw + w]) : 0ull;
                const int cnt = __popcll(p);
                const int incl = wave_incl_scan(cnt);
                if (w < tvw) {
                    part[w] = p;
                    pre[w] = run + incl - cnt;
                }
                run += __builtin_amdgcn_readlane(incl, 63);
            }
            if (lane == 0) ptotal = run;
        }
        __syncthreads();
        const int P = ptotal;
        const bool in_lds = P <= pmcap;
        unsigned long long* gout = pmask + poff[id];
        if (in_lds)
            for (int i = tid; i < P; i += TB) lm[i] = 0ull;
        __syncthreads();
        auto put = [&](int tx, int ty, unsigned long long m) {
            const int w = ty * wr + (tx >> 6), b = tx & 63;
            const unsigned long long pwv = part[w];
            if (!((pwv >> b) & 1ull)) return;
            const int slot = pre[w] + __popcll(pwv & ((1ull << b) - 1ull));
            if (in_lds) atomicOr(&lm[slot], m);
            else atomicOr(&gout[slot], m);
        };
        const int64_t rs = node_run_start[k];
        const int nr = node_nruns[k];
        for (int r = tid; r < nr; r += TB) {
            const Run ru = pool[rs + r];
            if (ru.y0 == ru.y1) {
                const int y = ru.y0, ty = y >> 3;
                for (int tx = ru.x0 >> 3; tx <= (ru.x1 >> 3); tx++) {
                    const int a = max((int)ru.x0, tx * 8) & 7, b = min((int)ru.x1, tx * 8 + 7) & 7;
                    put(tx, ty, (unsigned long long)((0xFFu >> (7 - b)) & (0xFFu << a) & 0xFFu) << ((y & 7) * 8));
                }
            } else if (ru.x0 == ru.x1) {
                const int x = ru.x0, tx = x >> 3;
                const unsigned long long colm = 0x0101010101010101ull << (x & 7);
                for (int ty = ru.y0 >> 3; ty <= (ru.y1 >> 3); ty++) {
                    const int a = max((int)ru.y0, ty * 8) & 7, b = min((int)ru.y1, ty * 8 + 7) & 7;
                    put(tx, ty, colm & (~0ull >> (8 * (7 - b))) & (~0ull << (8 * a)));
                }
            } else {
                const int dy = (ru.y1 > ru.y0) ? 1 : -1;
                int x = ru.x0, y = ru.y0;
                while (x <= ru.x1) {
                    int nn;
                    const unsigned long long m = diag_tile_mask(x, y, dy, ru.x1, nn);
                    put(x >> 3, y >> 3, m);
                    x += nn;
                    y += dy * nn;
                }
            }
        }
        __syncthreads();
        if (in_lds)
            for (int i = tid; i < P; i += TB) gout[i] = lm[i];
    }
}

__global__ void tile_pool_order_kernel(int rows, int tw, const int32_t* node_cell, int64_t n, const int64_t* node_run_start,
                                       int64_t* tscan_start) {
    const int64_t k = (int64_t)blockIdx.x * blockDim.x + threadIdx.x;
    if (k >= n) return;
    const int c = node_cell[k];
    tscan_start[tile_id_of(c / rows, c % rows, tw)] = node_run_start[k];
}

__global__ void tile_tt_kernel(int nt, int tvw, const unsigned long long* regular_tiles, const unsigned long long* ftvis,
                               const unsigned long long* tvis, unsigned long long* ttvis, unsigned long long* ttany) {
    const int lane = threadIdx.x & 63;
    const int t = blockIdx.x * (blockDim.x >> 6) + (threadIdx.x >> 6);
    if (t >= nt) return;
    const unsigned long long R = regular_tiles[t];
    for (int w = lane; w < tvw; w += 64) {
        unsigned long long acc = R ? ~0ull : 0ull, any = 0ull;
        for (unsigned long long m = R; m; m &= m - 1) {
            const int b = __ffsll((long long)m) - 1;
            acc &= ftvis[((size_t)t * 64 + b) * tvw + w];
            any |= tvis[((size_t)t * 64 + b) * tvw + w];
        }
        ttvis[(size_t)t * tvw + w] = acc;
        ttany[(size_t)t * tvw + w] = any;
    }
}

__global__ void tile_vsum_kernel(int64_t Ct, int tvw, const unsigned long long* tvis, unsigned long long* tvsum) {
    const int lane = threadIdx.x & 63;
    const int64_t c = (int64_t)blockIdx.x * (blockDim.x >> 6) + (threadIdx.x >> 6);
    if (c >= Ct) return;
    const int tvsw = (tvw + 63) / 64;
    const unsigned long long* row = tvis + (size_t)c * tvw;
    for (int j = 0; j < tvsw; j++) {
        const int w = j * 64 + lane;
        const unsigned long long bits = __ballot(w < tvw && row[w] != 0ull);
        if (lane == 0) tvsum[(size_t)c * tvsw + j] = bits;
    }
}

__global__ void tile_vblk_kernel(int64_t Ct, int tvw, int wr, int nbc, const unsigned long long* tvis, unsigned long long* tvblk) {
    const int lane = threadIdx.x & 63;
    const int64_t c = (int64_t)blockIdx.x * (blockDim.x >> 6) + (threadIdx.x >> 6);
    if (c >= Ct) return;
    const unsigned long long* row = tvis + (size_t)c * tvw;
    unsigned long long a0 = 0ull, a1 = 0ull, a2 = 0ull, a3 = 0ull;
    for (int w = lane; w < tvw; w += 64) {
        const unsigned long long t = row[w];
        if (t == 0ull) continue;
        int wd;
        unsigned long long lo, hi;
        blk_place(t, w, wr, nbc, wd, lo, hi);
        a0 |= wd == 0 ? lo : 0ull;
        a1 |= wd == 1 ? lo : (wd == 0 ? hi : 0ull);
        a2 |= wd == 2 ? lo : (wd == 1 ? hi : 0ull);
        a3 |= wd == 3 ? lo : (wd == 2 ? hi : 0ull);
    }
    for (int off = 32; off >= 1; off >>= 1) {
        a0 |= __shfl_xor(a0, off);
        a1 |= __shfl_xor(a1, off);
        a2 |= __shfl_xor(a2, off);
        a3 |= __shfl_xor(a3, off);
    }
    if (lane < 4) tvblk[(size_t)c * 4 + lane] = lane == 0 ? a0 : lane == 1 ? a1 : lane == 2 ? a2 : a3;
}

struct LSeg {
    int x0, y0, dx, dy, len;
};
__device__ __forceinline__ LSeg lseg_of(Run ru) {
    LSeg s;
    s.x0 = ru.x0;
    s.y0 = ru.y0;
    if (ru.y0 == ru.y1) { s.dx = 1; s.dy = 0; s.len = ru.x1 - ru.x0 + 1; }
    else if (ru.x0 == ru.x1) { s.dx = 0; s.dy = 1; s.len = ru.y1 - ru.y0 + 1; }
    else { s.dx = 1; s.dy = (ru.y1 > ru.y0) ? 1 : -1; s.len = ru.x1 - ru.x0 + 1; }
    return s;
}
__device__ __forceinline__ void lseg_overlap(const LSeg& c, const LSeg& s, int* pa, int* pb) {
    *pa = 1;
    *pb = 0;
    const int ux = s.x0 - c.x0, uy = s.y0 - c.y0;
    const int det = -c.dx * s.dy + s.dx * c.dy;
    if (det == 0) {
        if (ux * c.dy - uy * c.dx != 0) return;
        const int a = c.dx ? ux : uy;
        *pa = max(a, 0);
        *pb = min(a + s.len - 1, c.len - 1);
        return;
    }
    const int pn = -ux * s.dy + s.dx * uy, qn = c.dx * uy - c.dy * ux;
    if (pn % det != 0 || qn % det != 0) return;
    const int p = pn / det, q = qn / det;
    if (p < 0 || p >= c.len || q < 0 || q >= s.len) return;
    *pa = p;
    *pb = p;
}

constexpr int CR_THREADS = 256;
__global__ void __launch_bounds__(CR_THREADS) tile_cr_kernel(int cols, int rows, int tw, int th,
                                                             const unsigned long long* regular_tiles,
                                                             const int32_t* cell_node, const int64_t* node_run_start,
                                                             const int32_t* node_nruns, const int64_t* scan_start,
                                                             const Run* scan_pool, const Run* pool, int dmax, Run* cr) {
    extern __shared__ __attribute__((aligned(16))) int diff[];
    __shared__ LSeg cand[8];
    __shared__ int bestlen[8], beststart[8];
    const int nt = tw * th;
    const int tid = threadIdx.x;
    const int stride = dmax + 2;
    for (int t = blockIdx.x; t < nt; t += gridDim.x) {
        const unsigned long long R = regular_tiles[t];
        const int tx = t % tw, ty = t / tw;
        if (R == 0ull) {
            if (tid < CRK) { Run z; z.x0 = z.y0 = z.x1 = z.y1 = -1; cr[CRK * t + tid] = z; }
            continue;
        }
        const int nreg = __popcll(R);
        int cb = 0, cd = 1 << 30;
        for (int b = 0; b < 64; b++)
            if ((R >> b) & 1ull) {
                const int d = (2 * (b & 7) - 7) * (2 * (b & 7) - 7) + (2 * (b >> 3) - 7) * (2 * (b >> 3) - 7);
                if (d < cd) { cd = d; cb = b; }
            }
        const int ck = cell_node[(tx * 8 + (cb & 7)) * rows + ty * 8 + (cb >> 3)];
        for (int i = tid; i < 8 * stride; i += CR_THREADS) diff[i] = 0;
        if (tid < 8) {
            const int nrc = node_nruns[ck];
            if (tid < nrc) cand[tid] = lseg_of(scan_pool[scan_start[ck] + tid]);
            else cand[tid].len = 0;
        }
        __syncthreads();
        for (int b = 0; b < 64; b++) {
            if (!((R >> b) & 1ull)) continue;
            const int wk = cell_node[(tx * 8 + (b & 7)) * rows + ty * 8 + (b >> 3)];
            const int64_t rs = node_run_start[wk];
            const int nr = node_nruns[wk];
            for (int r = tid; r < nr; r += CR_THREADS) {
                const LSeg s = lseg_of(pool[rs + r]);
                for (int g = 0; g < 8; g++) {
                    const LSeg c = cand[g];
                    if (c.len == 0) continue;
                    int pa, pb;
                    lseg_overlap(c, s, &pa, &pb);
                    if (pa <= pb) {
                        atomicAdd(&diff[g * stride + pa], 1);
                        atomicAdd(&diff[g * stride + pb + 1], -1);
                    }
                }
            }
        }
        __syncthreads();
        if (tid < 8) {
            const LSeg c = cand[tid];
            int bl = 0, bs = 0, cur = 0, run = 0, rstart = 0;
            for (int p = 0; p < c.len; p++) {
                cur += diff[tid * stride + p];
                if (cur == nreg) {
                    if (run == 0) rstart = p;
                    run++;
                    if (run > bl) { bl = run; bs = rstart; }
                } else {
                    run = 0;
                }
            }
            bestlen[tid] = bl;
            beststart[tid] = bs;
        }
        __syncthreads();
        if (tid == 0) {
            int used = 0;
            for (int j = 0; j < CRK; j++) {
                int pick = -1;
                auto key = [&](int g) { return bestlen[g] + ((cand[g].dx == 0 || cand[g].dy == 0) ? (1 << 20) : 0); };
                for (int g = 0; g < 8; g++)
                    if (bestlen[g] > 0 && !((used >> g) & 1) && (pick < 0 || key(g) > key(pick))) pick = g;
                Run z;
                z.x0 = z.y0 = z.x1 = z.y1 = -1;
                if (pick >= 0) {
                    used |= 1 << pick;
                    const LSeg c = cand[pick];
                    const int pa = beststart[pick], pb = pa + bestlen[pick] - 1;
                    z.x0 = (int16_t)(c.x0 + pa * c.dx);
                    z.y0 = (int16_t)(c.y0 + pa * c.dy);
                    z.x1 = (int16_t)(c.x0 + pb * c.dx);
                    z.y1 = (int16_t)(c.y0 + pb * c.dy);
                }
                cr[CRK * t + j] = z;
            }
        }
        __syncthreads();
    }
}

__global__ void node_runs_differ_kernel(int64_t n, const int32_t* bins_a, const int64_t* rs_a, const int32_t* nr_a,
                                        const Run* pool_a, const int32_t* bins_b, const int64_t* rs_b, const int32_t* nr_b,
                                        const Run* pool_b, uint8_t* out) {
    const int64_t k = (int64_t)blockIdx.x * blockDim.x + threadIdx.x;
    if (k >= n) return;
    bool d = nr_a[k] != nr_b[k];
    for (int b = 0; b < 32 && !d; b++) d = bins_a[k * 32 + b] != bins_b[k * 32 + b];
    const unsigned long long* ra = (const unsigned long long*)(pool_a + rs_a[k]);
    const unsigned long long* rb = (const unsigned long long*)(pool_b + rs_b[k]);
    for (int r = 0; r < nr_a[k] && !d; r++) d = ra[r] != rb[r];
    out[k] = d ? 1 : 0;
}

__global__ void vga_measures_kernel(int64_t sb, int64_t se, const int32_t* hist_all, const int32_t* nlev_all, float* out,
                                    int64_t* levels_out, unsigned long long* stats, const int32_t* src_list = nullptr,
                                    int hstride = VGA_HMAX, bool by_index = false) {
    const int64_t i = sb + (int64_t)blockIdx.x * blockDim.x + threadIdx.x;
    if (i >= se) return;
    const int64_t src = src_list ? (int64_t)src_list[i] : i;
    const int64_t hi = by_index ? i : src;
    const int nlev = nlev_all[hi];
    float* o = out + src * 7;
    if (nlev <= 0 || nlev > hstride) {
        for (int i = 0; i < 7; i++) o[i] = -1.0f;
        if (levels_out) { levels_out[src * 3] = 0; levels_out[src * 3 + 1] = 0; levels_out[src * 3 + 2] = 0; }
        return;
    }
    long long tn, td;
    vga_measures(hist_all + hi * hstride, nlev, o, tn, td);
    if (levels_out) {
        levels_out[src * 3 + 0] = tn;
        levels_out[src * 3 + 1] = td;
        levels_out[src * 3 + 2] = nlev;
    }
    atomicAdd(&stats[2], (unsigned long long)tn);
}

}
```

depthmapx_amd/csrc/policy.hpp:

```cpp
#pragma once
#include <cstdint>
#include <cstdlib>

namespace dmx {
namespace policy {

constexpr int64_t kMkSample = 4096;
constexpr double kMkSourceCost = 0.0, kMkChunkCost = 0.7;

constexpr int kVgaTileAlpha = 60;
constexpr int kVgaTileAlphaHbm = 1000;
constexpr int kVgaTileCommonRuns = 4;
constexpr int kVgaSourceChunk = 1;
constexpr int kVgaTileBSplit = 3;
constexpr int kVgaTileCSplit = 1;
constexpr int kVgaTileCCert = 1;
constexpr int kVgaTileWalk = 1;
constexpr int kVgaDoAlpha = 15;
constexpr int kVgaDoShortList = 16;

constexpr int kSdbAmbCap = 1 << 16;
constexpr int kSdbEntCap = 1 << 22;

constexpr int kTvWindow = 64;
constexpr int kTvWindowMaxBytes = 64 * 1024;

constexpr int kIsoGapCap = 32;
constexpr int kIsoBlockCap = 128;
constexpr int kIsoRetryFactor = 16;
constexpr int kIsoCapMax = 1 << 16;
constexpr int kIsoWavesPerCu = 8;
constexpr int kIsoPoolPerNode = 48;
constexpr int kIsoVertexPoolPerPoint = 128;
constexpr int kIsoPointsWavesPerCu = 16;
constexpr int kIsoPointsMorton = 1;

constexpr int64_t kCodecSlabBytes = 64ll << 20;

constexpr int kConnStaticLds = 16 * 1024;
constexpr int64_t kConnTextBudget = 256ll << 20;

constexpr int kMemShareDiv = 4;
constexpr int kMemShareWideDiv = 3;
constexpr int kLdsPassBudget = 150 * 1024;

inline const char* hook(const char* name) { return std::getenv(name); }
inline int hook_int(const char* name, int dflt) {
    const char* e = std::getenv(name);
    return e ? std::atoi(e) : dflt;
}

}
}
```

depthmapx_amd/engine.py:

```python
import ctypes
import math

import numpy as np

from . import _native as N

MAKEGRAPH_COLUMNS = ["Connectivity", "Point First Moment", "Point Second Moment"]
STEPDEPTH_COLUMNS = ["Metric Step Shortest-Path Angle", "Metric Step Shortest-Path Length",
                     "Metric Straight-Line Distance"]
VGA_LOCAL_COLUMNS = ["Visual Clustering Coefficient", "Visual Control", "Visual Controllability"]
VGA_METRIC_COLUMNS = ["Metric Mean Shortest-Path Angle", "Metric Mean Shortest-Path Distance",
                      "Metric Mean Straight-Line Distance", "Metric Node Count"]
VGA_ANGULAR_COLUMNS = ["Angular Mean Depth", "Angular Total Depth", "Angular Node Count"]
VGA_COLUMNS = ["Visual Entropy", "Visual Integration [HH]", "Visual Integration [P-value]",
               "Visual Integration [Tekl]", "Visual Mean Depth", "Visual Node Count",
               "Visual Relativised Entropy"]


def isovist_cone(angle, viewangle, degrees=False):
    angle, viewangle = float(angle), float(viewangle)
    if degrees:
        angle = angle / 180.0 * math.pi
        viewangle = viewangle / 180.0 * math.pi
    if viewangle >= 2 * math.pi:
# ... 1 lines not shown
    left = angle - 0.5 * viewangle
    if left < 0:
        left += 2 * math.pi
    right = angle + 0.5 * viewangle
    if right > 2 * math.pi:
        right -= 2 * math.pi
    return left, right


def isovist_path_cones(polyline, fov):
    p = np.asarray(polyline, dtype=np.float64).reshape(-1, 2)
    fov = float(fov)
    pts = np.ascontiguousarray(p[:-1])
    ang = np.zeros((len(pts), 2), dtype=np.float64)
    if fov < 2.0 * math.pi:
        for i in range(len(pts)):
            vx, vy = float(p[i + 1, 0] - p[i, 0]), float(p[i + 1, 1] - p[i, 1])
            s = 1.0 / math.sqrt(vx * vx + vy * vy)
            vx, vy = vx * s, vy * s
            a = (2.0 * math.pi - math.acos(vx)) if vy < 0 else math.acos(vx)
            first, second = a - fov / 2.0, a + fov / 2.0
            if first < 0.0:
                first += 2.0 * math.pi
            if second > 2.0 * math.pi:
                second -= 2.0 * math.pi
            ang[i] = (first, second)
    return pts, ang


class Context:

    def __init__(self, device=0):
        h = ctypes.c_void_p()
        N.check(N.lib().dmx_ctx_create(int(device), ctypes.byref(h)))
        self.h = h
        self.device = device

    def close(self):
        if getattr(self, "h", None):
            N.lib().dmx_ctx_free(self.h)
            self.h = None

    __del__ = close

    def set_progress(self, fn, interval_s=0.5):
        if fn is None:
            self._progress = None
            N.check(N.lib().dmx_ctx_set_progress(self.h, N.PROGRESS_FN(), None, 0.0))
            return

        def tramp(_user, phase, done, total):
            try:
                return 1 if fn(int(phase), int(done), int(total)) else 0
            except Exception:
                return 1
        self._progress = N.PROGRESS_FN(tramp)
        N.check(N.lib().dmx_ctx_set_progress(self.h, self._progress, None, float(interval_s)))

    def cancel(self):
        N.check(N.lib().dmx_ctx_cancel(self.h))

    def last_fill(self):
        b, f, n = ctypes.c_double(), ctypes.c_double(), ctypes.c_int64()
        N.check(N.lib().dmx_ctx_last_fill(self.h, ctypes.byref(b), ctypes.byref(f), ctypes.byref(n)))
        return b.value, f.value, n.value

    def last_timing(self):
        mk, vg = ctypes.c_double(), ctypes.c_double()
        N.check(N.lib().dmx_ctx_last_timing(self.h, ctypes.byref(mk), ctypes.byref(vg)))
        return mk.value, vg.value

    def last_stepdepth(self):
        t, p, r = ctypes.c_double(), ctypes.c_int64(), ctypes.c_int64()
        N.check(N.lib().dmx_ctx_last_stepdepth(self.h, ctypes.byref(t), ctypes.byref(p), ctypes.byref(r)))
        d = np.zeros(4, dtype=np.int64)
        N.check(N.lib().dmx_ctx_last_stepdepth_detail(self.h, N.ptr(d)))
        a = ctypes.c_int64()
        N.check(N.lib().dmx_ctx_last_stepdepth_attempts(self.h, ctypes.byref(a)))
        b = np.zeros(5, dtype=np.int64)
        N.check(N.lib().dmx_ctx_last_stepdepth_batched(self.h, N.ptr(b)))
        why = "+".join(name for bit, name in ((1, "ent"), (2, "amb"), (4, "fold")) if int(b[4]) & bit)
        return dict(seconds=t.value, expanders_popped=p.value, cells_relaxed=r.value,
                    mode=["serial", "batched", "batched-overflow-serial"][int(d[0])], batches=int(d[1]),
                    improved=int(d[2]), ambiguous=int(d[3]), refills=0 if int(d[0]) == 1 else int(d[1]),
                    attempts=a.value, fold_long=int(b[0]), list_max=int(b[1]), amb_max=int(b[2]),
                    ent_max=int(b[3]), overflow=why or None)

    def last_isovist(self):
        b, k = ctypes.c_double(), ctypes.c_double()
        d = np.zeros(4, dtype=np.int64)
        N.check(N.lib().dmx_ctx_last_isovist(self.h, ctypes.byref(b), ctypes.byref(k), N.ptr(d)))
        return dict(bsp_seconds=b.value, kernel_seconds=k.value, tree_nodes=int(d[0]), tree_depth=int(d[1]),
                    reruns=int(d[2]), max_blocks=int(d[3]))

    def last_connections(self):
        c, e = ctypes.c_double(), ctypes.c_double()
        d = np.zeros(4, dtype=np.int64)
        N.check(N.lib().dmx_ctx_last_connections(self.h, ctypes.byref(c), ctypes.byref(e), N.ptr(d)))
        return dict(count_seconds=c.value, emit_seconds=e.value, bitmap_hbm=int(d[0]), dup_nodes=int(d[1]),
                    dup_cells=int(d[2]), outside_cells=int(d[3]))

    def last_agents(self):
        t, ht = ctypes.c_double(), ctypes.c_double()
        d, e = np.zeros(4, dtype=np.int64), np.zeros(3, dtype=np.int64)
        N.check(N.lib().dmx_ctx_last_agents(self.h, ctypes.byref(t), N.ptr(d)))
        N.check(N.lib().dmx_ctx_last_agents_detail(self.h, ctypes.byref(ht), N.ptr(e)))
        return dict(seconds=t.value, moves=int(d[0]), looks=int(d[1]), host_reruns=int(d[2]), clamped=int(d[3]),
                    host_seconds=ht.value, fallbacks=int(e[0]), diag_taken=int(e[1]), stopped=int(e[2]))

    ISOVIST_POLY_GUESS = 128

    def isovists(self, lines, points, angles=None, region=None, simple=False, polygons=False):
        lines = np.ascontiguousarray(lines, dtype=np.float64).reshape(-1, 4)
        points = np.ascontiguousarray(points, dtype=np.float64).reshape(-1, 2)
        n = len(points)
        if angles is not None:
            angles = np.ascontiguousarray(angles, dtype=np.float64).reshape(-1, 2)
            assert len(angles) == n
        if region is not None:
            region = np.ascontiguousarray(region, dtype=np.float64).reshape(4)
        out = np.full((n, 8), -1.0, dtype=np.float32)
        lib = N.lib()
        args = (self.h, N.ptr(lines), len(lines), N.ptr(region), N.ptr(points), N.ptr(angles), n, int(bool(simple)),
                N.ptr(out))
        if not polygons:
            N.check(lib.dmx_isovists(*args, None, None, 0, None))
            return out
        off = np.zeros(n + 1, dtype=np.int64)
        total = ctypes.c_int64()
        xy = np.empty((max(self.ISOVIST_POLY_GUESS * n, 1), 2), dtype=np.float64)
        for _ in range(2):
            N.check(lib.dmx_isovists(*args, N.ptr(off), N.ptr(xy), len(xy), ctypes.byref(total)))
            if total.value <= len(xy):
                break
            xy = np.empty((total.value, 2), dtype=np.float64)
        return out, off, xy[:total.value]

    def last_mk_reruns(self):
        n = ctypes.c_int64()
        N.check(N.lib().dmx_ctx_last_mk_reruns(self.h, None, 0, ctypes.byref(n)))
        out = np.zeros(max(n.value, 1), dtype=np.int64)
        N.check(N.lib().dmx_ctx_last_mk_reruns(self.h, N.ptr(out), n.value, ctypes.byref(n)))
        out = out[:n.value]
        cap = (out >> 62) & 1
        nodes = out & ((1 << 62) - 1)
        return np.unique(nodes[cap == 0]), np.unique(nodes[cap == 1])

    def last_phase_cycles(self):
        out = np.zeros(5, dtype=np.int64)
        N.check(N.lib().dmx_ctx_last_phase_cycles(self.h, N.ptr(out)))
        return dict(zip(["level1", "tile_common", "heads", "hard", "bookkeeping"], (int(v) for v in out)))

    def last_stats(self):
        out = np.zeros(51, dtype=np.int64)
        N.check(N.lib().dmx_ctx_last_stats(self.h, N.ptr(out), 51))
        keys = ["mk_cells_examined", "mk_visible_pairs", "mk_runs", "vga_kernel", "vga_runs_expanded", "vga_levels",
                "vga_cells_reached", "vga_sources", "vga_fail_cells", "vga_fail_runs", "vga_hbm_bitmaps",
                "vga_cr_tiles", "vga_launch", "vga_pruned_cells", "vga_tvis_bytes", "vga_hard_runs", "vga_hard_hits",
                "vga_hard_cells", "vga_hard_certain", "vga_topdown_cycles", "vga_b_tiles", "vga_b_cells", "vga_tt_tiles", "vga_c_busy", "vga_c_scan", "vga_c_spec", "vga_n_spec", "vga_tt_pruned", "vga_b_row_cycles", "vga_b_cell_tiles",
                "vga_b_cell_cycles", "vga_b_ext_cells", "mk_depth_steps", "mk_chunks", "mk_reruns", "vga_pmask_loads", "vga_pmask_cells", "vga_pmask_bytes",
                "vga_order_reruns", "vga_sym_scatter_us", "vga_prep_flags", "vga_tile_rows_bytes", "vga_scan_bytes",
                "vga_asym_nodes", "tv_lines", "tv_pixel_steps", "tv_window", "mk_diag_inexact", "vga_tl_max", "vga_c_row_cells",
                "vga_c_cert_cells"]
        d = {k: int(v) for k, v in zip(keys, out)}
        lv = d.pop("vga_levels")
        d["vga_bottom_up_levels"], d["vga_top_down_levels"] = lv & 0xFFFFFFFF, lv >> 32
        d["vga_special_nodes"] = d["vga_kernel"] >> 8
        d["vga_frontier_hbm"] = (d["vga_launch"] >> 56) & 1
        d["vga_line_summaries"] = (d["vga_launch"] >> 57) & 1
        d["vga_threads"] = (d["vga_launch"] >> 40) & 0xFFFF
        d["vga_launch"] &= (1 << 32) - 1
        f = d["vga_prep_flags"]
        d["vga_scan_order"], d["vga_scan_released"] = f & 1, (f >> 1) & 1
        d["vga_prep"] = "+".join(n for b, n in enumerate(["scan", "scan-released", "tvis", "ftvis", "ttvis", "masks",
                                                            "tvsum", "asymmetric-mode"]) if (f >> b) & 1) or "none"
        d["vga_asym_mode"] = (f >> 7) & 1
        d["vga_kernel"] = ["topdown-v1", "direction-optimizing(top-down only)",
                           "direction-optimizing", "tile-resolved"][d["vga_kernel"] & 0xFF]
        return d


class PointMap:

    def __init__(self, region, lines, spacing):
        self._region = np.ascontiguousarray(region, dtype=np.float64)
        self._lines = np.ascontiguousarray(lines, dtype=np.float64).reshape(-1, 4)
        h = ctypes.c_void_p()
        N.check(N.lib().dmx_pointmap_create(N.ptr(self._region), float(spacing), N.ptr(self._lines),
                                            len(self._lines), ctypes.byref(h)))
        self.h = h
        self.spacing = float(spacing)

    def close(self):
        if getattr(self, "h", None):
            N.lib().dmx_pointmap_free(self.h)
            self.h = None

    __del__ = close

    def info(self):
        c, r, f = ctypes.c_int32(), ctypes.c_int32(), ctypes.c_int64()
        bx, by = ctypes.c_double(), ctypes.c_double()
        N.check(N.lib().dmx_pointmap_info(self.h, ctypes.byref(c), ctypes.byref(r), ctypes.byref(bx),
                                          ctypes.byref(by), ctypes.byref(f)))
        return dict(cols=c.value, rows=r.value, bottom_left=(bx.value, by.value), filled=f.value)

    @property
    def cols(self):
        return self.info()["cols"]

    @property
    def rows(self):
        return self.info()["rows"]

    FULLFILL, SEMIFILL, AUGMENT = 0, 1, 2

    def make_points(self, x, y, ctx=None, fill_type=0):
        made = ctypes.c_int()
        if ctx is None:
            N.check(N.lib().dmx_pointmap_make_points(self.h, float(x), float(y), int(fill_type), ctypes.byref(made)))
        else:
            N.check(N.lib().dmx_pointmap_make_points_device(ctx.h, self.h, float(x), float(y), int(fill_type),
                                                            ctypes.byref(made)))
        return bool(made.value)

    def state(self):
        i = self.info()
        out = np.zeros(i["cols"] * i["rows"], dtype=np.int32)
        N.check(N.lib().dmx_pointmap_state(self.h, N.ptr(out)))
        return out

    def pixelate(self, x, y):
        i = self.info()
        blx, bly = i["bottom_left"]
        px = int(np.floor((x - blx + self.spacing / 2.0) / self.spacing))
        py = int(np.floor((y - bly + self.spacing / 2.0) / self.spacing))
        px = min(max(px, 0), i["cols"] - 1)
        py = min(max(py, 0), i["rows"] - 1)
        return px * i["rows"] + py

    def region_contains(self, x, y):
        r = self._region
        return r[0] <= x <= r[2] and r[1] <= y <= r[3]

    def cell_lines(self):
        i = self.info()
        total = ctypes.c_int64()
        N.check(N.lib().dmx_pointmap_cell_lines(self.h, None, None, ctypes.byref(total)))
        counts = np.zeros(i["cols"] * i["rows"], dtype=np.int32)
        pieces = np.zeros((max(total.value, 1), 4), dtype=np.float64)
        N.check(N.lib().dmx_pointmap_cell_lines(self.h, N.ptr(counts), N.ptr(pieces), ctypes.byref(total)))
        return counts, pieces[:total.value]

    def set_merges(self, cell_pairs):
        arr = np.ascontiguousarray(cell_pairs, dtype=np.int32).reshape(-1, 2)
        N.check(N.lib().dmx_pointmap_set_merges(self.h, N.ptr(arr), len(arr)))

    def agent_schedule(self, seed=0, timesteps=5000, release_rate=0.1, lifetime=1000, release_cells=None, locseed=0):
        rel = np.ascontiguousarray([] if release_cells is None else release_cells, dtype=np.int32).reshape(-1)
        n = ctypes.c_int64()
        args = (self.h, int(seed) & 0xFFFFFFFF, int(timesteps), float(release_rate), int(lifetime), N.ptr(rel), len(rel),
                int(locseed))
        N.check(N.lib().dmx_agent_schedule(*args, None, None, None, 0, ctypes.byref(n)))
        cell = np.zeros(max(n.value, 1), dtype=np.int32)
        aseed = np.zeros(max(n.value, 1), dtype=np.uint32)
        moves = np.zeros(max(n.value, 1), dtype=np.int32)
        N.check(N.lib().dmx_agent_schedule(*args, N.ptr(cell), N.ptr(aseed), N.ptr(moves), n.value, ctypes.byref(n)))
        return np.stack([cell, aseed.view(np.int32), moves], axis=1)[:n.value]

    def make_graph(self, ctx, boundarygraph=False, maxdist=-1.0, node_begin=0, node_end=-1):
        h = ctypes.c_void_p()
        N.check(N.lib().dmx_makegraph(ctx.h, self.h, float(maxdist), int(bool(boundarygraph)), int(node_begin),
                                      int(node_end), ctypes.byref(h)))
        return Graph(h, ctx, self)

    def shard_bounds(self, ctx, world, stride=256, boundarygraph=False, maxdist=-1.0):
        b = np.zeros(int(world) + 1, dtype=np.int64)
        N.check(N.lib().dmx_makegraph_balance(ctx.h, self.h, float(maxdist), int(bool(boundarygraph)), int(world),
                                              int(stride), N.ptr(b)))
        return [int(v) for v in b]

    def assemble(self, ctx, blob_ptrs, blob_sizes):
        ptrs = (ctypes.c_void_p * len(blob_ptrs))(*blob_ptrs)
        sizes = np.ascontiguousarray(blob_sizes, dtype=np.int64)
        h = ctypes.c_void_p()
        N.check(N.lib().dmx_graph_assemble_device(ctx.h, self.h, ptrs, N.ptr(sizes), len(blob_ptrs),
                                                  ctypes.byref(h)))
        return Graph(h, ctx, self)


class Graph:

    def __init__(self, h, ctx, pm):
        self.h, self.ctx, self.pm = h, ctx, pm

    def close(self):
        if getattr(self, "h", None):
            N.lib().dmx_graph_free(self.h)
            self.h = None

    __del__ = close

    def info(self):
        n, b, e, r = (ctypes.c_int64() for _ in range(4))
        N.check(N.lib().dmx_graph_info(self.h, ctypes.byref(n), ctypes.byref(b), ctypes.byref(e), ctypes.byref(r)))
        return dict(nnodes=n.value, node_begin=b.value, node_end=e.value, nruns=r.value)

    def special_nodes(self):
        n = ctypes.c_int64(0)
        N.check(N.lib().dmx_graph_special_nodes(self.h, None, ctypes.byref(n)))
        out = np.zeros(max(n.value, 1), dtype=np.int32)
        N.check(N.lib().dmx_graph_special_nodes(self.h, N.ptr(out), ctypes.byref(n)))
        return out[:n.value]

    def copy(self, runs=True):
        i = self.info()
        n = i["node_end"] - i["node_begin"]
        attrs = np.zeros((n, 3), dtype=np.float32)
        bins = np.zeros((n, 32, 4), dtype=np.int32)
        gc = np.zeros(n, dtype=np.uint8)
        rr = np.zeros((max(i["nruns"], 1), 4), dtype=np.int16) if runs else None
        N.check(N.lib().dmx_graph_copy(self.h, N.ptr(attrs), N.ptr(bins), N.ptr(rr), N.ptr(gc)))
        out = dict(attrs=attrs, bins=bins, gridconn=gc)
        if runs:
            out["runs"] = rr[:i["nruns"]]
        return out

    def copy_range(self, node_begin, node_end, runs=True):
        n = node_end - node_begin
        attrs = np.zeros((n, 3), dtype=np.float32)
        bins = np.zeros((n, 32, 4), dtype=np.int32)
        gc = np.zeros(n, dtype=np.uint8)
        nr = ctypes.c_int64()
        N.check(N.lib().dmx_graph_copy_range(self.h, int(node_begin), int(node_end), N.ptr(attrs), N.ptr(bins), None,
                                             -1, ctypes.byref(nr), N.ptr(gc)))
        out = dict(attrs=attrs, bins=bins, gridconn=gc)
        if runs:
            rr = np.zeros((max(nr.value, 1), 4), dtype=np.int16)
            N.check(N.lib().dmx_graph_copy_range(self.h, int(node_begin), int(node_end), None, None, N.ptr(rr),
                                                 len(rr), None, None))
            out["runs"] = rr[:nr.value]
        return out

    def write_chunk(self, columns, displayed=0, boundary=False, name=None):
        from . import graphio
        return graphio.write_chunk_device(self, columns, displayed=displayed, boundary=boundary, name=name)

    def set_merges(self, cell_pairs):
        arr = np.ascontiguousarray(cell_pairs, dtype=np.int32).reshape(-1, 2)
        N.check(N.lib().dmx_graph_set_merges(self.h, N.ptr(arr), len(arr)))

    def set_drawing(self, lines):
        arr = np.ascontiguousarray(lines, dtype=np.float64).reshape(-1, 4)
        self._drawing = arr
        N.check(N.lib().dmx_graph_set_drawing(self.h, N.ptr(arr), len(arr)))

    def blob_size(self):
        b = ctypes.c_int64()
        N.check(N.lib().dmx_graph_blob_size(self.h, ctypes.byref(b)))
        return b.value

    def write_blob_device(self, dev_ptr, nbytes):
        N.check(N.lib().dmx_graph_blob_write_device(self.h, ctypes.c_void_p(dev_ptr), int(nbytes)))

    def vga_visual_global(self, radius=-1.0, gates_only=False, src_begin=0, src_end=-1, levels=False):
        n = self.info()["nnodes"]
        out = np.full((n, 7), -1.0, dtype=np.float32)
        lv = np.zeros((n, 3), dtype=np.int64) if levels else None
        N.check(N.lib().dmx_vga_global(self.ctx.h, self.h, float(radius), int(bool(gates_only)), int(src_begin),
                                       int(src_end), N.ptr(out), N.ptr(lv)))
        return (out, lv) if levels else out

    def vga_metric(self, radius=-1.0, gates_only=False, src_begin=0, src_end=-1):
        n = self.info()["nnodes"]
        out = np.full((n, 4), -1.0, dtype=np.float32)
        N.check(N.lib().dmx_vga_metric(self.ctx.h, self.h, float(radius), int(bool(gates_only)), int(src_begin),
                                       int(src_end), N.ptr(out)))
        return out

    def vga_angular(self, radius=-1.0, gates_only=False, src_begin=0, src_end=-1):
        n = self.info()["nnodes"]
        out = np.full((n, 3), -1.0, dtype=np.float32)
        N.check(N.lib().dmx_vga_angular(self.ctx.h, self.h, float(radius), int(bool(gates_only)), int(src_begin),
                                        int(src_end), N.ptr(out)))
        return out

    def angular_step_depth(self, points=None, cells=None):
        sel = [] if cells is None else [int(c) for c in cells]
        for (x, y) in (points or []):
            if not self.pm.region_contains(x, y):
                raise N.DmxError(-6, "Point outside of target region")
            sel.append(self.pm.pixelate(x, y))
        arr = np.ascontiguousarray(sel, dtype=np.int32)
        out = np.full(self.info()["nnodes"], -1.0, dtype=np.float32)
        N.check(N.lib().dmx_angular_stepdepth(self.ctx.h, self.h, N.ptr(arr), len(arr), N.ptr(out)))
        return out

    def vga_visual_local(self, gates_only=False, src_begin=0, src_end=-1):
        n = self.info()["nnodes"]
        out = np.full((n, 3), -1.0, dtype=np.float32)
        N.check(N.lib().dmx_vga_local(self.ctx.h, self.h, int(bool(gates_only)), int(src_begin), int(src_end),
                                      N.ptr(out)))
        return out

    def vga_through_vision(self, src_begin=0, src_end=-1, counts=False):
        n = self.info()["nnodes"]
        out = np.zeros(n, dtype=np.float32)
        cnt = np.zeros(n, dtype=np.int64) if counts else None
        N.check(N.lib().dmx_vga_thruvision(self.ctx.h, self.h, int(src_begin), int(src_end), N.ptr(out),
                                           N.ptr(cnt)))
        return (out, cnt) if counts else out

    def agents(self, table, fov=15, steps=3, trails=0):
        table = np.ascontiguousarray(table, dtype=np.int32).reshape(-1, 3)
        n = len(table)
        cell = np.ascontiguousarray(table[:, 0])
        seed = np.ascontiguousarray(table[:, 1]).view(np.uint32)
        moves = np.ascontiguousarray(table[:, 2])
        i = self.pm.info()
        vbin = -1 if int(fov) == 32 else (int(fov) - 1) // 2
        counts = np.zeros(i["cols"] * i["rows"], dtype=np.uint32)
        final_cell = np.zeros(n, dtype=np.int32)
        final_loc = np.zeros((n, 2), dtype=np.float64)
        stuck = np.zeros(n, dtype=np.uint8)
        ntrail = min(int(trails), n)
        trail = np.full((ntrail, int(moves.max()) if n else 0), -1, dtype=np.int32) if ntrail else None
        N.check(N.lib().dmx_agents(self.ctx.h, self.h, vbin, int(steps), n, N.ptr(cell), N.ptr(seed), N.ptr(moves),
                                   N.ptr(counts), N.ptr(final_cell), N.ptr(final_loc), N.ptr(stuck), N.ptr(trail),
                                   ntrail))
        return dict(counts=counts, final_cell=final_cell, final_loc=final_loc, stuck=stuck,
                    trails=trail if ntrail else np.zeros((0, 0), dtype=np.int32))

    def _node_range(self, node_begin, node_end):
        nb, ne = int(node_begin), int(node_end)
        return nb, ne, max((self.info()["nnodes"] if ne < 0 else ne) - nb, 0)

    def connections(self, node_begin=0, node_end=-1, export=False):
        nb, ne, n = self._node_range(node_begin, node_end)
        off = np.zeros(n + 1, dtype=np.int64)
        total = ctypes.c_int64()
        lib = N.lib()
        N.check(lib.dmx_graph_connections(self.ctx.h, self.h, nb, ne, int(bool(export)), N.ptr(off), None, 0,
                                          ctypes.byref(total)))
        refs = np.zeros(total.value, dtype=np.int32)
        if total.value:
            N.check(lib.dmx_graph_connections(self.ctx.h, self.h, nb, ne, int(bool(export)), N.ptr(off), N.ptr(refs),
                                              len(refs), ctypes.byref(total)))
        return off, refs

    def connections_csv(self, node_begin=0, node_end=-1, delim=","):
        nb, ne, _ = self._node_range(node_begin, node_end)
        size = ctypes.c_int64()
        lib = N.lib()
        d = delim.encode() if isinstance(delim, str) else bytes(delim)
        N.check(lib.dmx_graph_connections_csv(self.ctx.h, self.h, nb, ne, d, None, None, 0, ctypes.byref(size)))
        buf = ctypes.create_string_buffer(max(size.value, 1))
        if size.value:
            N.check(lib.dmx_graph_connections_csv(self.ctx.h, self.h, nb, ne, d, None, buf, size.value,
                                                  ctypes.byref(size)))
        return buf.raw[:size.value]

    ISOVIST_COLUMNS = ["Isovist Area", "Isovist Compactness", "Isovist Drift Angle", "Isovist Drift Magnitude",
                       "Isovist Max Radial", "Isovist Min Radial", "Isovist Occlusivity", "Isovist Perimeter"]

    def vga_isovist(self, simple=False, src_begin=0, src_end=-1, occlusion=False, out=None):
        n = self.info()["nnodes"]
# ... 70 lines not shown
```

include/dmx.h:

```cpp
#ifndef DMX_H
#define DMX_H
#include <stdint.h>

#ifdef __cplusplus
extern "C" {
#endif

#define DMX_ABI_VERSION 1

enum {
    DMX_OK = 0,
    DMX_ERR_ARG = -1,
    DMX_ERR_HIP = -2,
    DMX_ERR_CAPACITY = -3,
    DMX_ERR_STATE = -4,
    DMX_ERR_UNSUPPORTED = -5,
    DMX_ERR_OUTSIDE = -6,
    DMX_ERR_CANCELLED = -7
};

enum {
    DMX_PHASE_MAKEGRAPH = 1,
    DMX_PHASE_VGA = 2
};

typedef struct dmx_ctx dmx_ctx;
typedef struct dmx_pointmap dmx_pointmap;
typedef struct dmx_graph dmx_graph;

int dmx_abi_version(void);
const char* dmx_last_error(void);
int dmx_ctx_create(int device, dmx_ctx** out);
int dmx_ctx_free(dmx_ctx* ctx);
int dmx_release_cached_memory(void);

typedef int32_t (*dmx_progress_fn)(void* user, int32_t phase, int64_t done, int64_t total);
int dmx_ctx_set_progress(dmx_ctx* ctx, dmx_progress_fn fn, void* user, double interval_s);
int dmx_ctx_cancel(dmx_ctx* ctx);
int dmx_ctx_last_timing(dmx_ctx* ctx, double* makegraph_s, double* vga_s);
int dmx_ctx_last_stats(dmx_ctx* ctx, int64_t* out, int n);

int dmx_ctx_last_mk_reruns(dmx_ctx* ctx, int64_t* nodes, int64_t cap, int64_t* n);

int dmx_ctx_last_phase_cycles(dmx_ctx* ctx, int64_t* out5);

int dmx_pointmap_create(const double* region, double spacing, const double* lines, int64_t nlines,
                        dmx_pointmap** out);
int dmx_pointmap_free(dmx_pointmap* pm);
int dmx_pointmap_fill(dmx_pointmap* pm, double x, double y, int* made);
int dmx_pointmap_fill_device(dmx_ctx* ctx, dmx_pointmap* pm, double x, double y, int* made);
int dmx_ctx_last_fill(dmx_ctx* ctx, double* block_s, double* fill_s, int64_t* levels);
int dmx_pointmap_make_points(dmx_pointmap* pm, double x, double y, int fill_type, int* made);
int dmx_pointmap_make_points_device(dmx_ctx* ctx, dmx_pointmap* pm, double x, double y, int fill_type, int* made);
int dmx_pointmap_set_state(dmx_pointmap* pm, const int32_t* state);
int dmx_pointmap_info(const dmx_pointmap* pm, int32_t* cols, int32_t* rows, double* bl_x, double* bl_y,
                      int64_t* filled);
int dmx_pointmap_state(const dmx_pointmap* pm, int32_t* out);
int dmx_pointmap_cell_lines(dmx_pointmap* pm, int32_t* counts, double* pieces, int64_t* total);

int dmx_makegraph(dmx_ctx* ctx, dmx_pointmap* pm, double maxdist, int boundary, int64_t node_begin,
                  int64_t node_end, dmx_graph** out);
int dmx_makegraph_balance(dmx_ctx* ctx, dmx_pointmap* pm, double maxdist, int boundary, int32_t world,
                          int64_t stride, int64_t* bounds);
int dmx_graph_free(dmx_graph* g);
int dmx_graph_info(const dmx_graph* g, int64_t* nnodes, int64_t* node_begin, int64_t* node_end, int64_t* nruns);
int dmx_graph_copy(dmx_graph* g, float* attrs, int32_t* bins, int16_t* runs, uint8_t* gridconn);
int dmx_graph_copy_range(dmx_graph* g, int64_t node_b, int64_t node_e, float* attrs, int32_t* bins, int16_t* runs,
                         int64_t runs_cap, int64_t* nruns_out, uint8_t* gridconn);

int dmx_graph_blob_size(dmx_graph* g, int64_t* bytes);
int dmx_graph_blob_write_device(dmx_graph* g, void* dst_device, int64_t bytes);
int dmx_graph_assemble_device(dmx_ctx* ctx, dmx_pointmap* pm, const void* const* blobs, const int64_t* sizes,
                              int nshards, dmx_graph** out);

int dmx_vga_global(dmx_ctx* ctx, dmx_graph* g, double radius, int gates_only, int64_t src_begin, int64_t src_end,
                   float* out, int64_t* levels);
int dmx_vga_global_device(dmx_ctx* ctx, dmx_graph* g, double radius, int gates_only, int64_t src_begin,
                          int64_t src_end, float* out_device);
int dmx_vga_global_device_list(dmx_ctx* ctx, dmx_graph* g, double radius, int gates_only, const int64_t* nodes,
                               int64_t n, float* out_device);
int dmx_graph_special_nodes(dmx_graph* g, int32_t* nodes, int64_t* n);
int dmx_vga_metric(dmx_ctx* ctx, dmx_graph* g, double radius, int gates_only, int64_t src_begin, int64_t src_end,
                   float* out);
int dmx_vga_angular(dmx_ctx* ctx, dmx_graph* g, double radius, int gates_only, int64_t src_begin, int64_t src_end,
                    float* out);
int dmx_vga_local(dmx_ctx* ctx, dmx_graph* g, int gates_only, int64_t src_begin, int64_t src_end, float* out);
int dmx_vga_thruvision(dmx_ctx* ctx, dmx_graph* g, int64_t src_begin, int64_t src_end,
                       float* out , int64_t* counts );
#define DMX_CONN_EXPORT 1
int dmx_graph_connections(dmx_ctx* ctx, dmx_graph* g, int64_t node_begin, int64_t node_end, int flags,
                          int64_t* off , int32_t* refs , int64_t cap, int64_t* total);
int dmx_graph_connections_csv(dmx_ctx* ctx, dmx_graph* g, int64_t node_begin, int64_t node_end, const char* delim,
                              int64_t* off , char* buf , int64_t cap,
                              int64_t* size);
int dmx_ctx_last_connections(dmx_ctx* ctx, double* count_s, double* emit_s, int64_t* out4);
int dmx_agent_schedule(const dmx_pointmap* pm, uint32_t seed, int32_t timesteps, double release_rate,
                       int32_t lifetime, const int32_t* release_cells, int64_t nrelease, int32_t locseed,
                       int32_t* start_cell, uint32_t* agent_seed, int32_t* moves, int64_t cap, int64_t* nagents);
int dmx_agents(dmx_ctx* ctx, dmx_graph* g, int32_t vbin, int32_t steps, int64_t nagents,
               const int32_t* start_cell, const uint32_t* agent_seed, const int32_t* moves,
               uint32_t* counts , int32_t* final_cell, double* final_loc ,
               uint8_t* stuck, int32_t* trail , int64_t ntrail);
int dmx_ctx_last_agents(dmx_ctx* ctx, double* seconds, int64_t* out4);
int dmx_ctx_last_agents_detail(dmx_ctx* ctx, double* host_seconds, int64_t* out3);
int dmx_vga_isovist(dmx_ctx* ctx, dmx_graph* g, int simple_version, int64_t src_begin, int64_t src_end,
                    float* out , float* occ_dist ,
                    int32_t* occ_counts , int32_t* occ_pixels, int64_t occ_cap,
                    int64_t* occ_total);
int dmx_ctx_last_isovist(dmx_ctx* ctx, double* bsp_s, double* kernel_s, int64_t* out4);
int dmx_isovists(dmx_ctx* ctx, const double* lines, int64_t nlines, const double* region ,
                 const double* points , const double* angles ,
                 int64_t n, int simple_version, float* out ,
                 int64_t* poly_off , double* poly_xy ,
                 int64_t poly_cap, int64_t* poly_total );
#define DMX_I32 0
#define DMX_I64 1
typedef int (*dmx_allreduce_fn)(void* device_ptr, int64_t count, int dtype, void* user);
int dmx_graph_set_prep_shard(dmx_graph* g, int64_t node_begin, int64_t node_end, dmx_allreduce_fn fn, void* user);

int dmx_metric_stepdepth(dmx_ctx* ctx, dmx_graph* g, const int32_t* sel_cells, int64_t nsel, float* out);
int dmx_angular_stepdepth(dmx_ctx* ctx, dmx_graph* g, const int32_t* sel_cells, int64_t nsel, float* out);
int dmx_visual_stepdepth(dmx_ctx* ctx, dmx_graph* g, const int32_t* sel_cells, int64_t nsel, float* out);
int dmx_ctx_last_stepdepth(dmx_ctx* ctx, double* seconds, int64_t* expanders_popped, int64_t* cells_relaxed);
int dmx_ctx_last_stepdepth_detail(dmx_ctx* ctx, int64_t* out4);
int dmx_ctx_last_stepdepth_attempts(dmx_ctx* ctx, int64_t* attempts);
int dmx_ctx_last_stepdepth_batched(dmx_ctx* ctx, int64_t* out5);

int dmx_chunk_write(const dmx_pointmap* pm, int64_t nnodes, const int32_t* bins, const int16_t* runs, int64_t nruns,
                    const uint8_t* gridconn, int ncols, const char* const* names, const float* values,
                    const uint8_t* locked, const uint8_t* setmask, int displayed, int boundary, uint8_t* buf, int64_t cap,
                    int64_t* size);
typedef struct dmx_chunk dmx_chunk;
int dmx_chunk_parse(const uint8_t* buf, int64_t size, dmx_chunk** out);
int dmx_chunk_free(dmx_chunk* c);
int dmx_chunk_info(const dmx_chunk* c, int32_t* cols, int32_t* rows, double* spacing, double* bl, int64_t* nnodes,
                   int64_t* nruns, int32_t* ncols, int32_t* displayed_sorted, int64_t* bytes_used);
int dmx_chunk_column(const dmx_chunk* c, int i, char* name, int name_cap, float* values, int* locked);
int dmx_chunk_arrays(const dmx_chunk* c, int32_t* state, int32_t* bins, int16_t* runs, uint8_t* gridconn);
int dmx_chunk_load(dmx_ctx* ctx, const dmx_chunk* c, const double* region, dmx_pointmap** pm, dmx_graph** g);
int dmx_graph_from_runs(dmx_ctx* ctx, dmx_pointmap* pm, int64_t nnodes, const int32_t* bins, const int16_t* runs,
                        int64_t nruns, const uint8_t* gridconn, const float* attrs, dmx_graph** out);
int dmx_graph_set_merges(dmx_graph* g, const int32_t* cell_pairs, int64_t n);
int dmx_graph_set_drawing(dmx_graph* g, const double* lines, int64_t nlines);
int dmx_pointmap_set_merges(dmx_pointmap* pm, const int32_t* cell_pairs, int64_t n);
int dmx_chunk_merges(const dmx_chunk* c, int32_t* cell_pairs, int64_t* n);
int dmx_chunk_rows(const dmx_chunk* c, int32_t* keys, uint8_t* visible);
int dmx_chunk_merge_records(const dmx_chunk* c, int32_t* cell_pairs, int64_t* n);
int dmx_chunk_flags(const dmx_chunk* c, int* processed, int* boundary, int64_t* merges, int64_t* nrows);
int dmx_chunk_set_column(dmx_chunk* c, const char* name, const float* values, const uint8_t* setmask, int locked,
                         int make_displayed);
int dmx_chunk_set_displayed(dmx_chunk* c, int physical_column);
int dmx_chunk_occlusion(const dmx_chunk* c, float* occ_dist, int32_t* occ_counts, int32_t* occ_pixels, int64_t cap,
                        int64_t* total);
int dmx_chunk_set_occlusion(dmx_chunk* c, const float* occ_dist, const int32_t* occ_counts, const int32_t* occ_pixels);

int dmx_chunk_set_name(dmx_chunk* c, const char* name);
int dmx_chunk_select_cells(dmx_chunk* c, const int32_t* cells, int64_t n);
int dmx_chunk_unmake(dmx_chunk* c, int remove_links);
int dmx_chunk_serialize(const dmx_chunk* c, uint8_t* buf, int64_t cap, int64_t* size);

int dmx_graph_chunk_write(dmx_graph* g, const char* map_name, int ncols, const char* const* names,
                          const float* values, const uint8_t* locked, const uint8_t* setmask, int displayed,
                          int boundary, uint8_t* buf, int64_t cap, int64_t* size);
int dmx_chunk_scan(const uint8_t* buf, int64_t size, int32_t* cols, int32_t* rows, int64_t* nnodes,
                   int64_t* nruns, int64_t* bytes_used);
int dmx_chunk_load_bytes(dmx_ctx* ctx, const uint8_t* buf, int64_t size, const double* region,
                         dmx_pointmap** pm, dmx_graph** g);

typedef struct dmx_graphfile dmx_graphfile;
int dmx_graphfile_read(const char* path, dmx_graphfile** out);
int dmx_graphfile_free(dmx_graphfile* g);
int dmx_graphfile_write(const dmx_graphfile* g, const char* path);
int dmx_graphfile_info(const dmx_graphfile* g, int32_t* state, int32_t* view_class, double* region, int64_t* nlines,
                       int32_t* npointmaps, int32_t* displayed);
int dmx_graphfile_lines(const dmx_graphfile* g, double* lines );
int dmx_graphfile_set_view(dmx_graphfile* g, int32_t state, int32_t view_class);
int dmx_graphfile_pointmap(const dmx_graphfile* g, int i, const uint8_t** chunk, int64_t* size);
int dmx_graphfile_put_pointmap(dmx_graphfile* g, int i, const uint8_t* chunk, int64_t size);
int dmx_graphfile_new_pointmap_name(const dmx_graphfile* g, char* name, int cap);
int32_t dmx_view_vga_top(int32_t view_class);

#ifdef __cplusplus
}
#endif
#endif
```

Baseline: 183,600.

## Speed up VGA tile preparation kernels and add prep timing and array export

Result: no change. 185,400, median of 6 (+1.0%).

```diff
diff --git a/depthmapx_amd/_native.py b/depthmapx_amd/_native.py
--- a/depthmapx_amd/_native.py
+++ b/depthmapx_amd/_native.py
@@ -25,7 +25,8 @@
     "dmx_pointmap_fill_device": (_i32, [_vp, _vp, _dbl, _dbl, _vp]),
     "dmx_pointmap_make_points": (_i32, [_vp, _dbl, _dbl, _i32, _vp]),
     "dmx_graph_special_nodes": (_i32, [_vp, _vp, _vp]),
-    "dmx_pointmap_make_points_device": (_i32, [_vp, _vp, _dbl, _dbl, _i32, _vp]),
+    "dmx_graph_vga_prep_copy": (_i32, [_vp, _vp, _i32, _vp, _i64, _vp]),
+    "dmx_pointmap_make_points_device":(_i32, [_vp, _vp, _dbl, _dbl, _i32, _vp]),
     "dmx_ctx_last_fill": (_i32, [_vp, _vp, _vp, _vp]),
     "dmx_pointmap_info": (_i32, [_vp, _vp, _vp, _vp, _vp, _vp]),
     "dmx_pointmap_state": (_i32, [_vp, _vp]),
diff --git a/depthmapx_amd/csrc/api/vga_global.hip b/depthmapx_amd/csrc/api/vga_global.hip
--- a/depthmapx_amd/csrc/api/vga_global.hip
+++ b/depthmapx_amd/csrc/api/vga_global.hip
@@ -10,6 +10,22 @@
         return fail(DMX_ERR_STATE, "prep all-reduce callback failed");
     return DMX_OK;
 }
+struct PrepTimer {
+    dmx_graph* g;
+    double t0 = 0;
+    explicit PrepTimer(dmx_graph* g_) : g(g_) {
+        if (g->prep_depth++ == 0) {
+            (void)hipStreamSynchronize(g->ctx->stream);
+            t0 = now_s();
+        }
+    }
+    ~PrepTimer() {
+        if (--g->prep_depth == 0) {
+            (void)hipStreamSynchronize(g->ctx->stream);
+            g->prep_us += (now_s() - t0) * 1e6;
+        }
+    }
+};
 static int prepare_symmetry(dmx_graph* g);
 static int build_scan_order(dmx_graph* g);
 static int prepare_uf(dmx_graph* g) {
@@ -59,23 +75,42 @@
     PointMapHost& h = *g->pm->host;
     const int rows = h.rows();
     const int64_t C = (int64_t)h.cols() * rows, N = g->nnodes;
+    PrepTimer timer(g);
     std::vector<int32_t> nr((size_t)std::max<int64_t>(N, 1));
     if (N) HIPCHK(copy_sync(s, nr.data(), g->node_nruns.p, N * 4, hipMemcpyDeviceToHost));
     std::vector<int64_t> ss((size_t)std::max<int64_t>(N, 1));
     int64_t acc = 0;
-    for (int64_t k = 0; k < N; k++) { ss[k] = acc; acc += nr[k]; }
+    int nr_max = 1;
+    for (int64_t k = 0; k < N; k++) { ss[k] = acc; acc += nr[k]; nr_max = std::max(nr_max, nr[k]); }
     DevBuf<int64_t>& d_ss = g->scan_start;
     HIPCHK(d_ss.alloc(std::max<int64_t>(N, 1)));
     HIPCHK(g->scan_pool.alloc(std::max<int64_t>(acc, 1)));
     HIPCHK(g->cell_scan_start.alloc(C));
     HIPCHK(g->cell_nruns.alloc(C));
     HIPCHK(hipMemsetAsync(g->cell_nruns.p, 0, C * 4, s));
+    g->scan_twopass = 0;
     if (N) {
         HIPCHK(hipMemcpyAsync(d_ss.p, ss.data(), N * 8, hipMemcpyHostToDevice, s));
-        hipLaunchKernelGGL(scan_pool_kernel, dim3((unsigned)std::min<int64_t>(N, 8192)), dim3(256), 0, s, rows,
-                           g->pm->d_node_cell.p, N, g->node_run_start.p, g->node_nruns.p, g->bin_nruns.p, g->pool.p, d_ss.p,
-                           g->scan_pool.p, g->cell_scan_start.p, g->cell_nruns.p);
-        HIPCHK(hipGetLastError());
+        if (policy::prep_legacy() & policy::kVgaPrepLegacyScan) {
+            hipLaunchKernelGGL(scan_pool_kernel, dim3((unsigned)std::min<int64_t>(N, 8192)), dim3(256), 0, s, rows,
+                               g->pm->d_node_cell.p, N, g->node_run_start.p, g->node_nruns.p, g->bin_nruns.p, g->pool.p, d_ss.p,
+                               g->scan_pool.p, g->cell_scan_start.p, g->cell_nruns.p);
+            HIPCHK(hipGetLastError());
+        } else {
+            const int cap_policy = std::min(policy::kVgaScanLds, std::max(1, policy::hook_int("DMX_VGA_SCAN_LDS", policy::kVgaScanLds)));
+            const int cap = std::min(cap_policy, (nr_max + 63) & ~63);
+            DevBuf<unsigned long long> over;
+            HIPCHK(over.alloc(1));
+            HIPCHK(hipMemsetAsync(over.p, 0, 8, s));
+            hipLaunchKernelGGL(scan_pool_stable_kernel, dim3((unsigned)std::min<int64_t>(N, (int64_t)ctx->num_cu * 8)),
+                               dim3(64 * SP_WAVES), (size_t)cap * 8, s, rows, g->pm->d_node_cell.p, N, g->node_run_start.p,
+                               g->node_nruns.p, g->bin_nruns.p, g->pool.p, d_ss.p, g->scan_pool.p, g->cell_scan_start.p,
+                               g->cell_nruns.p, cap, over.p);
+            HIPCHK(hipGetLastError());
+            unsigned long long nover = 0;
+            HIPCHK(copy_sync(s, &nover, over.p, 8, hipMemcpyDeviceToHost));
+            g->scan_twopass = (int64_t)nover;
+        }
     }
     HIPCHK(hipStreamSynchronize(s));
     g->scan_released = false;
@@ -101,6 +136,7 @@
     }
     dmx_ctx* ctx = g->ctx;
     hipStream_t s = ctx->stream;
+    PrepTimer timer(g);
     PointMapHost& h = *g->pm->host;
     const int cols = h.cols(), rows = h.rows();
     const int64_t C = (int64_t)cols * rows, N = g->nnodes;
@@ -250,7 +286,8 @@
     HIPCHK(hipMemGetInfo(&free_b, &total_b));
     const size_t mask_b = (size_t)total * 8;
     bool build = total > 0 && mask_b <= free_b / policy::kMemShareDiv;
-    const int pmcap = wide ? PM_CAP_WIDE : PM_CAP;
+    const int pmcap_grid = wide ? PM_CAP_WIDE : PM_CAP;
+    const int pmcap = std::min(pmcap_grid, std::max(1, policy::hook_int("DMX_VGA_PMCAP", pmcap_grid)));
     if (wide && total > 0 && tile_pmask_lds(tvw, pmcap) <= policy::kLdsPassBudget) {
         const size_t reserve = 16ull << 30;
         const size_t free_all = free_b + cached_bytes();
@@ -282,7 +319,8 @@
     const int64_t N = g->nnodes;
     if (N > 0) {
         const int64_t nb = std::min<int64_t>(N, (int64_t)ctx->num_cu * 16);
-        hipLaunchKernelGGL(tile_pmask_kernel, dim3((unsigned)nb), dim3(64 * TV_WAVES), tile_pmask_lds(tvw, pmcap), s, rows,
+        auto* kern = (policy::prep_legacy() & policy::kVgaPrepLegacyPmask) ? tile_pmask_kernel<false> : tile_pmask_kernel<true>;
+        hipLaunchKernelGGL(kern, dim3((unsigned)nb), dim3(64 * TV_WAVES), tile_pmask_lds(tvw, pmcap), s, rows,
                            tw, th, g->pm->d_node_cell.p, N, g->node_run_start.p, g->node_nruns.p, g->pool.p, g->tvis.p,
                            g->ftvis.p, g->poff.p, g->pmask.p, pmcap);
         HIPCHK(hipGetLastError());
@@ -304,6 +342,8 @@
                                       (g->ttvis.p ? g->ttvis.n * 8 : 0) + (g->tvsum.p ? g->tvsum.n * 8 : 0) + (g->tvnz.p ? g->tvnz.n * 8 : 0) +
                                       (g->tvblk.p ? g->tvblk.n * 8 : 0));
     ctx->last_stats[42] = (long long)(g->scan_pool.p ? g->scan_pool.n * sizeof(Run) : 0);
+    ctx->last_stats[51] = (long long)g->prep_us;
+    ctx->last_stats[52] = g->scan_twopass;
 }
 
 static size_t tile_lds_layout(int tw, int th, bool* fg, bool* rbm) {
@@ -324,6 +364,7 @@
 
 static int prepare_tiles(dmx_graph* g) {
     if (g->tiles_ready) return DMX_OK;
+    PrepTimer timer(g);
     if (g->scan_released)
         if (int rc = restore_scan_order(g)) return rc;
     dmx_ctx* ctx = g->ctx;
@@ -358,7 +399,9 @@
     const int dmax = std::max(cols, rows);
     const size_t lds = (size_t)8 * (dmax + 2) * 4;
     if (lds > policy::kLdsPassBudget) return fail(DMX_ERR_CAPACITY, "grid too long for the tile-common-run pass");
-    hipLaunchKernelGGL(tile_cr_kernel, dim3((unsigned)std::min<int64_t>(nt, (int64_t)ctx->num_cu * 8)), dim3(CR_THREADS),
+    const int legacy = policy::prep_legacy();
+    auto* cr_kern = (legacy & policy::kVgaPrepLegacyCr) ? tile_cr_kernel<false> : tile_cr_kernel<true>;
+    hipLaunchKernelGGL(cr_kern, dim3((unsigned)std::min<int64_t>(nt, (int64_t)ctx->num_cu * 8)), dim3(CR_THREADS),
                        lds, s, cols, rows, tw, th, g->regular_tiles.p, g->pm->d_cell_node.p, g->node_run_start.p,
                        g->node_nruns.p, g->scan_start.p, g->scan_pool.p, g->pool.p, dmax, g->cr.p);
     HIPCHK(hipGetLastError());
@@ -402,7 +445,9 @@
         prep_range(g, pb, pe);
         if (pe > pb) {
             const int64_t nb = std::min<int64_t>(pe - pb, (int64_t)ctx->num_cu * 16);
-            hipLaunchKernelGGL(tile_vis_kernel, dim3((unsigned)nb), dim3(64 * TV_WAVES), tv_lds, s, rows, tw, th,
+            auto* vis_kern = (legacy & policy::kVgaPrepLegacyVis) ? tile_vis_kernel<0> : tile_vis_kernel<1>;
+            if (policy::hook_int("DMX_VIS_MODE", 1) == 2) vis_kern = tile_vis_kernel<2>;
+            hipLaunchKernelGGL(vis_kern, dim3((unsigned)nb), dim3(64 * TV_WAVES), tv_lds, s, rows, tw, th,
                                g->pm->d_node_cell.p + pb, pe - pb, g->node_run_start.p + pb, g->node_nruns.p + pb,
                                g->pool.p, g->notuf_tiles.p, g->tvis.p, ftv ? g->ftvis.p : nullptr);
             HIPCHK(hipGetLastError());
@@ -1103,3 +1148,31 @@
     ctx->last_vga_s = total;
     return DMX_OK;
 }
+
+static const int kPrepCopyLimit = 256 << 20;
+int dmx_graph_vga_prep_copy(dmx_ctx* ctx, dmx_graph* g, int32_t which, void* out, int64_t cap_bytes, int64_t* nbytes) {
+    if (!ctx || !g || !nbytes || which < 0 || which >= DMX_PREP_ARRAYS) return fail(DMX_ERR_ARG, "bad arguments");
+    if (g->node_begin != 0 || g->node_end != g->nnodes)
+        return fail(DMX_ERR_STATE, "the VGA preparation needs the whole graph (assemble the shards first)");
+    HIPCHK(hipSetDevice(ctx->device));
+    if (int rc = prepare_uf(g)) return rc;
+    if (int rc = prepare_symmetry(g)) return rc;
+    if (g->symmetric != 1) return fail(DMX_ERR_STATE, "the graph is not symmetric: the tile search's preparation does not run");
+    if (int rc = prepare_tiles(g)) return rc;
+    prep_state_stats(ctx, g);
+    const void* p[DMX_PREP_ARRAYS] = {g->tvis.p, g->ftvis.p, g->ttvis.p, g->tvblk.p, g->ppre.p, g->poff.p, g->pmask.p,
+                                      g->cr.p, g->heads.p, g->tscan_start.p, g->tnruns.p, g->scan_pool.p, g->scan_start.p};
+    const size_t b[DMX_PREP_ARRAYS] = {g->tvis.n * 8, g->ftvis.n * 8, g->ttvis.n * 8, g->tvblk.n * 8, g->ppre.n * 2,
+                                       g->poff.n * 8, g->pmask.n * 8, g->cr.n * sizeof(Run), g->heads.n * sizeof(Run),
+                                       g->tscan_start.n * 8, g->tnruns.n * 4, g->scan_pool.n * sizeof(Run),
+                                       g->scan_start.n * 8};
+    size_t all = 0;
+    for (int i = 0; i < DMX_PREP_ARRAYS; i++) all += p[i] ? b[i] : 0;
+    if (all > (size_t)kPrepCopyLimit) return fail(DMX_ERR_CAPACITY, "the preparation's arrays exceed the diagnostic copy's 256 MB");
+    const size_t nb = p[which] ? b[which] : 0;
+    *nbytes = (int64_t)nb;
+    if (!out || nb == 0) return DMX_OK;
+    if (cap_bytes < (int64_t)nb) return fail(DMX_ERR_ARG, "output buffer too small");
+    HIPCHK(copy_sync(ctx->stream, out, p[which], nb, hipMemcpyDeviceToHost));
+    return DMX_OK;
+}
diff --git a/depthmapx_amd/csrc/dmx_api.hip b/depthmapx_amd/csrc/dmx_api.hip
--- a/depthmapx_amd/csrc/dmx_api.hip
+++ b/depthmapx_amd/csrc/dmx_api.hip
@@ -185,7 +185,7 @@
     long long phase_cycles[5] = {0, 0, 0, 0, 0};
     DevBuf<int> counters;
     DevBuf<unsigned long long> stats;
-    long long last_stats[51] = {};
+    long long last_stats[53] = {};
     std::vector<int64_t> last_mk_reruns;
     DmxCtl* h_ctl = nullptr;
     DmxCtl* d_ctl = nullptr;
@@ -250,6 +250,9 @@
     DevBuf<int64_t> cell_scan_start;
     DevBuf<int32_t> cell_nruns;
     DevBuf<int64_t> scan_start;
+    int64_t scan_twopass = 0;
+    double prep_us = 0;
+    int prep_depth = 0;
     int symmetric = -1;
     int nspecial = 0;
     std::vector<int32_t> special_nodes;
@@ -650,7 +653,7 @@
 
 int dmx_ctx_last_stats(dmx_ctx* c, int64_t* out, int n) {
     if (!c || !out) return fail(DMX_ERR_ARG, "bad arguments");
-    for (int i = 0; i < n && i < 51; i++) out[i] = c->last_stats[i];
+    for (int i = 0; i < n && i < 53; i++) out[i] = c->last_stats[i];
     return DMX_OK;
 }
 
diff --git a/depthmapx_amd/csrc/kernels/vga_do.hip b/depthmapx_amd/csrc/kernels/vga_do.hip
--- a/depthmapx_amd/csrc/kernels/vga_do.hip
+++ b/depthmapx_amd/csrc/kernels/vga_do.hip
@@ -603,6 +603,114 @@
     }
 }
 
+constexpr int SP_WAVES = 8;
+__global__ void __launch_bounds__(64 * SP_WAVES) scan_pool_stable_kernel(int rows, const int32_t* node_cell, int64_t n,
+                                                                        const int64_t* node_run_start, const int32_t* node_nruns,
+                                                                        const int32_t* bin_nruns, const Run* pool,
+                                                                        const int64_t* scan_start, Run* scan_pool,
+                                                                        int64_t* cell_scan_start, int32_t* cell_nruns, int cap,
+                                                                        unsigned long long* over) {
+    extern __shared__ __attribute__((aligned(16))) unsigned long long sp_st[];
+    __shared__ int wcnt[SP_WAVES][128], tot[128], ng[8], pre[33];
+    const int tid = threadIdx.x, lane = tid & 63, wv = tid >> 6;
+    const unsigned long long below = lane ? (~0ull >> (64 - lane)) : 0ull;
+    for (int64_t k = blockIdx.x; k < n; k += gridDim.x) {
+        const int64_t rs = node_run_start[k], ss = scan_start[k];
+        const int nr = node_nruns[k];
+        const bool staged = nr <= cap;
+        const unsigned long long* src = (const unsigned long long*)(pool + rs);
+        for (int i = tid; i < SP_WAVES * 128; i += 64 * SP_WAVES) wcnt[i >> 7][i & 127] = 0;
+        if (tid < 32) pre[tid + 1] = bin_nruns[k * 32 + tid];
+        if (tid == 0) {
+            pre[0] = 0;
+            const int c = node_cell[k];
+            cell_scan_start[c] = ss;
+            cell_nruns[c] = nr;
+            if (!staged) atomicAdd(over, 1ull);
+        }
+        __syncthreads();
+        if (tid == 0)
+            for (int b = 1; b <= 32; b++) pre[b] += pre[b - 1];
+        __syncthreads();
+        const int q = (((nr + SP_WAVES - 1) / SP_WAVES) + 63) & ~63;
+        const int rb = min(nr, wv * q), re = min(nr, rb + q);
+        auto key_of = [&](int r, unsigned long long w) {
+            int b = 0;
+#pragma unroll
+            for (int step = 16; step; step >>= 1)
+                if (pre[b + step] <= r) b += step;
+            const Run ru = *(const Run*)&w;
+            const int len = max(ru.x1 - ru.x0, max(ru.y1 - ru.y0, ru.y0 - ru.y1)) + 1;
+            return (b >> 2) * 16 + 15 - min(15, 31 - __clz(len));
+        };
+        for (int r0 = rb; r0 < re; r0 += 64) {
+            const int r = r0 + lane;
+            const bool valid = r < re;
+            unsigned long long w = 0ull;
+            int key = -1;
+            if (valid) {
+                w = src[r];
+                if (staged) sp_st[r] = w;
+                key = key_of(r, w);
+            }
+            unsigned long long todo = __ballot(valid);
+            while (todo) {
+                const int lead = __ffsll((long long)todo) - 1;
+                const int kk = __shfl(key, lead);
+                const unsigned long long mk = __ballot(key == kk);
+                if (lane == lead) wcnt[wv][kk] += __popcll(mk);
+                todo &= ~mk;
+            }
+        }
+        __syncthreads();
+        if (tid < 128) {
+            int t = 0;
+            for (int w = 0; w < SP_WAVES; w++) t += wcnt[w][tid];
+            tot[tid] = t;
+        }
+        __syncthreads();
+        if (tid < 128) {
+            int start = 0;
+            for (int b = tid & ~15; b < tid; b++) start += tot[b];
+            for (int w = 0; w < SP_WAVES; w++) {
+                const int c = wcnt[w][tid];
+                wcnt[w][tid] = start;
+                start += c;
+            }
+            if ((tid & 15) == 15) ng[tid >> 4] = start;
+        }
+        __syncthreads();
+        for (int r0 = rb; r0 < re; r0 += 64) {
+            const int r = r0 + lane;
+            const bool valid = r < re;
+            unsigned long long w = 0ull;
+            int key = -1;
+            if (valid) {
+                w = staged ? sp_st[r] : src[r];
+                key = key_of(r, w);
+            }
+            int p = 0;
+            unsigned long long todo = __ballot(valid);
+            while (todo) {
+                const int lead = __ffsll((long long)todo) - 1;
+                const int kk = __shfl(key, lead);
+                const unsigned long long mk = __ballot(key == kk);
+                const int first = wcnt[wv][kk];
+                if (key == kk) p = first + __popcll(mk & below);
+                if (lane == lead) wcnt[wv][kk] = first + __popcll(mk);
+                todo &= ~mk;
+            }
+            if (valid) {
+                const int g = key >> 4;
+                int idx = 0;
+                for (int h = 0; h < 8; h++) idx += min(p, ng[h]) + ((h < g && ng[h] > p) ? 1 : 0);
+                ((unsigned long long*)scan_pool)[ss + idx] = w;
+            }
+        }
+        __syncthreads();
+    }
+}
+
 __global__ void sym_special_out_kernel(int rows, const int32_t* specials, int nspec, const int32_t* node_cell,
                                        const int32_t* cell_node, const uint8_t* is_special, const int64_t* node_run_start,
                                        const int32_t* node_nruns, const Run* pool, int32_t* out, int* out_n, int cap) {
diff --git a/depthmapx_amd/csrc/kernels/vga_tile.hip b/depthmapx_amd/csrc/kernels/vga_tile.hip
--- a/depthmapx_amd/csrc/kernels/vga_tile.hip
+++ b/depthmapx_amd/csrc/kernels/vga_tile.hip
@@ -2021,6 +2021,10 @@
 __device__ __forceinline__ void tv_count(uint32_t* cnt, int t, int c) {
     atomicAdd(&cnt[t >> 2], (uint32_t)c << (8 * (t & 3)));
 }
+__device__ __forceinline__ int tv_cells(const uint8_t* nsc, const unsigned long long* seed_tiles, int t, unsigned long long m) {
+    return nsc[t] == 64 ? __popcll(m) : __popcll(m & ~seed_tiles[t]);
+}
+template <int MODE>
 __global__ void __launch_bounds__(64 * TV_WAVES) tile_vis_kernel(int rows, int tw, int th, const int32_t* node_cell,
                                                                  int64_t n, const int64_t* node_run_start,
                                                                  const int32_t* node_nruns, const Run* pool,
@@ -2052,12 +2056,34 @@
                     const int lo = max(t0 - w * 64, 0), hi = min(t1 - w * 64, 63);
                     atomicOr(&row[ty * wr + w], (~0ull << lo) & (~0ull >> (63 - hi)));
                 }
-                if (ftvis)
+                if (ftvis && MODE == 1) {
+                    const int ta = ty * tw + t0, tb = ty * tw + t1;
+                    for (int wi = ta >> 2; wi <= (tb >> 2); wi++) {
+                        const int lo = max(ta, wi * 4), hi = min(tb, wi * 4 + 3);
+                        const uint32_t in = (0xFFFFFFFFu << (8 * (lo & 3))) & (0xFFFFFFFFu >> (8 * (3 - (hi & 3))));
+                        if (((((const uint32_t*)nsc)[wi] ^ 0x40404040u) & in) == 0u) {
+                            uint32_t add = 0u;
+                            for (int t = lo; t <= hi; t++) {
+                                const int tx = t - ty * tw;
+                                add |= (uint32_t)(min((int)ru.x1, tx * 8 + 7) - max((int)ru.x0, tx * 8) + 1) << (8 * (t & 3));
+                            }
+                            atomicAdd(&cnt[wi], add);
+                        } else {
+                            for (int t = lo; t <= hi; t++) {
+                                const int tx = t - ty * tw;
+                                const int a = max((int)ru.x0, tx * 8) & 7, b = min((int)ru.x1, tx * 8 + 7) & 7;
+                                const unsigned long long m = (unsigned long long)((0xFFu >> (7 - b)) & (0xFFu << a) & 0xFFu) << ((y & 7) * 8);
+                                const int c = tv_cells(nsc, seed_tiles, t, m);
+                                if (c) tv_count(cnt, t, c);
+                            }
+                        }
+                    }
+                } else if (ftvis)
                     for (int tx = t0; tx <= t1; tx++) {
                         const int a = max((int)ru.x0, tx * 8) & 7, b = min((int)ru.x1, tx * 8 + 7) & 7;
                         const unsigned long long m = (unsigned long long)((0xFFu >> (7 - b)) & (0xFFu << a) & 0xFFu) << ((y & 7) * 8);
                         const int t = ty * tw + tx;
-                        const int c = __popcll(m & ~seed_tiles[t]);
+                        const int c = MODE ? tv_cells(nsc, seed_tiles, t, m) : __popcll(m & ~seed_tiles[t]);
                         if (c) tv_count(cnt, t, c);
                     }
             } else if (ru.x0 == ru.x1) {
@@ -2069,7 +2095,7 @@
                         const int a = max((int)ru.y0, ty * 8) & 7, b = min((int)ru.y1, ty * 8 + 7) & 7;
                         const unsigned long long m = colm & (~0ull >> (8 * (7 - b))) & (~0ull << (8 * a));
                         const int t = ty * tw + tx;
-                        const int c = __popcll(m & ~seed_tiles[t]);
+                        const int c = MODE ? tv_cells(nsc, seed_tiles, t, m) : __popcll(m & ~seed_tiles[t]);
                         if (c) tv_count(cnt, t, c);
                     }
                 }
@@ -2083,7 +2109,7 @@
                     atomicOr(&row[ty * wr + (tx >> 6)], 1ull << (tx & 63));
                     if (ftvis) {
                         const int t = ty * tw + tx;
-                        const int c = __popcll(m & ~seed_tiles[t]);
+                        const int c = MODE ? tv_cells(nsc, seed_tiles, t, m) : __popcll(m & ~seed_tiles[t]);
                         if (c) tv_count(cnt, t, c);
                     }
                     x += n;
@@ -2098,6 +2124,26 @@
         for (int w = tid; w < tvw; w += TB) out[w] = row[w];
         if (ftvis) {
             unsigned long long* fout = ftvis + (size_t)id * tvw;
+            if constexpr (MODE == 1) {
+                for (int w0 = 0; w0 < tvw; w0 += TB / 4) {
+                    const int w = w0 + (tid >> 2), q = tid & 3;
+                    unsigned long long f = 0ull;
+                    if (w < tvw) {
+                        unsigned long long m = row[w] & (0xFFFFull << (16 * q));
+                        const int tyw = w / wr, tx0 = (w % wr) * 64;
+                        while (m) {
+                            const int j = __ffsll((long long)m) - 1;
+                            m &= m - 1;
+                            const int t = tyw * tw + tx0 + j;
+                            const int cv = (cnt[t >> 2] >> (8 * (t & 3))) & 0xFF;
+                            if (cv == nsc[t] && cv > 0) f |= 1ull << j;
+                        }
+                    }
+                    f |= __shfl_xor(f, 1);
+                    f |= __shfl_xor(f, 2);
+                    if (w < tvw && q == 0) fout[w] = f;
+                }
+            } else
             for (int w = tid; w < tvw; w += TB) {
                 unsigned long long m = row[w], f = 0ull;
                 const int tyw = w / wr, tx0 = (w % wr) * 64;
@@ -2133,6 +2179,7 @@
 constexpr int PM_CAP = 4096;
 constexpr int PM_CAP_WIDE = 8192;
 __host__ __device__ inline size_t tile_pmask_lds(int tvw, int pmcap) { return (size_t)tvw * 12 + (size_t)pmcap * 8; }
+template <bool BITS>
 __global__ void __launch_bounds__(64 * TV_WAVES) tile_pmask_kernel(int rows, int tw, int th, const int32_t* node_cell,
                                                                    int64_t n, const int64_t* node_run_start,
                                                                    const int32_t* node_nruns, const Run* pool,
@@ -2187,6 +2234,26 @@
             const Run ru = pool[rs + r];
             if (ru.y0 == ru.y1) {
                 const int y = ru.y0, ty = y >> 3;
+                if constexpr (BITS) {
+                    const int t0 = ru.x0 >> 3, t1 = ru.x1 >> 3;
+                    for (int w = t0 >> 6; w <= (t1 >> 6); w++) {
+                        const int lo = max(t0 - w * 64, 0), hi = min(t1 - w * 64, 63);
+                        const unsigned long long pwv = part[ty * wr + w];
+                        unsigned long long mm = pwv & (~0ull << lo) & (~0ull >> (63 - hi));
+                        if (!mm) continue;
+                        const int pw = pre[ty * wr + w];
+                        while (mm) {
+                            const int bt = __ffsll((long long)mm) - 1;
+                            mm &= mm - 1;
+                            const int tx = w * 64 + bt;
+                            const int a = max((int)ru.x0, tx * 8) & 7, b = min((int)ru.x1, tx * 8 + 7) & 7;
+                            const unsigned long long m = (unsigned long long)((0xFFu >> (7 - b)) & (0xFFu << a) & 0xFFu) << ((y & 7) * 8);
+                            const int slot = pw + __popcll(pwv & ((1ull << bt) - 1ull));
+                            if (in_lds) atomicOr(&lm[slot], m);
+                            else atomicOr(&gout[slot], m);
+                        }
+                    }
+                } else
                 for (int tx = ru.x0 >> 3; tx <= (ru.x1 >> 3); tx++) {
                     const int a = max((int)ru.x0, tx * 8) & 7, b = min((int)ru.x1, tx * 8 + 7) & 7;
                     put(tx, ty, (unsigned long long)((0xFFu >> (7 - b)) & (0xFFu << a) & 0xFFu) << ((y & 7) * 8));
@@ -2293,6 +2360,7 @@
     else { s.dx = 1; s.dy = (ru.y1 > ru.y0) ? 1 : -1; s.len = ru.x1 - ru.x0 + 1; }
     return s;
 }
+template <bool NODIV = false>
 __device__ __forceinline__ void lseg_overlap(const LSeg& c, const LSeg& s, int* pa, int* pb) {
     *pa = 1;
     *pb = 0;
@@ -2306,14 +2374,28 @@
         return;
     }
     const int pn = -ux * s.dy + s.dx * uy, qn = c.dx * uy - c.dy * ux;
-    if (pn % det != 0 || qn % det != 0) return;
-    const int p = pn / det, q = qn / det;
+    int p, q;
+    if constexpr (NODIV) {
+        const bool two = det == 2 || det == -2;
+        if (two && ((pn | qn) & 1)) return;
+        p = det < 0 ? -pn : pn;
+        q = det < 0 ? -qn : qn;
+        if (two) { p >>= 1; q >>= 1; }
+    } else {
+        if (pn % det != 0 || qn % det != 0) return;
+        p = pn / det;
+        q = qn / det;
+    }
     if (p < 0 || p >= c.len || q < 0 || q >= s.len) return;
     *pa = p;
     *pb = p;
 }
 
 constexpr int CR_THREADS = 256;
+struct CrBox {
+    int x0, x1, y0, y1;
+};
+template <bool FAST>
 __global__ void __launch_bounds__(CR_THREADS) tile_cr_kernel(int cols, int rows, int tw, int th,
                                                              const unsigned long long* regular_tiles,
                                                              const int32_t* cell_node, const int64_t* node_run_start,
@@ -2321,6 +2403,7 @@
                                                              const Run* scan_pool, const Run* pool, int dmax, Run* cr) {
     extern __shared__ __attribute__((aligned(16))) int diff[];
     __shared__ LSeg cand[8];
+    __shared__ __attribute__((aligned(16))) CrBox cbox[8];
     __shared__ int bestlen[8], beststart[8];
     const int nt = tw * th;
     const int tid = threadIdx.x;
@@ -2343,8 +2426,17 @@
         for (int i = tid; i < 8 * stride; i += CR_THREADS) diff[i] = 0;
         if (tid < 8) {
             const int nrc = node_nruns[ck];
-            if (tid < nrc) cand[tid] = lseg_of(scan_pool[scan_start[ck] + tid]);
-            else cand[tid].len = 0;
+            CrBox bx;
+            bx.x0 = 1; bx.x1 = 0; bx.y0 = 1; bx.y1 = 0;
+            if (tid < nrc) {
+                const Run cu = scan_pool[scan_start[ck] + tid];
+                cand[tid] = lseg_of(cu);
+                bx.x0 = cu.x0; bx.x1 = cu.x1;
+                bx.y0 = min(cu.y0, cu.y1); bx.y1 = max(cu.y0, cu.y1);
+            } else {
+                cand[tid].len = 0;
+            }
+            cbox[tid] = bx;
         }
         __syncthreads();
         for (int b = 0; b < 64; b++) {
@@ -2353,12 +2445,18 @@
             const int64_t rs = node_run_start[wk];
             const int nr = node_nruns[wk];
             for (int r = tid; r < nr; r += CR_THREADS) {
-                const LSeg s = lseg_of(pool[rs + r]);
+                const Run su = pool[rs + r];
+                const LSeg s = lseg_of(su);
+                const int sy0 = min(su.y0, su.y1), sy1 = max(su.y0, su.y1);
                 for (int g = 0; g < 8; g++) {
+                    if constexpr (FAST) {
+                        const CrBox bx = cbox[g];
+                        if (su.x1 < bx.x0 || su.x0 > bx.x1 || sy1 < bx.y0 || sy0 > bx.y1) continue;
+                    }
                     const LSeg c = cand[g];
                     if (c.len == 0) continue;
                     int pa, pb;
-                    lseg_overlap(c, s, &pa, &pb);
+                    lseg_overlap<FAST>(c, s, &pa, &pb);
                     if (pa <= pb) {
                         atomicAdd(&diff[g * stride + pa], 1);
                         atomicAdd(&diff[g * stride + pb + 1], -1);
diff --git a/depthmapx_amd/csrc/policy.hpp b/depthmapx_amd/csrc/policy.hpp
--- a/depthmapx_amd/csrc/policy.hpp
+++ b/depthmapx_amd/csrc/policy.hpp
@@ -1,6 +1,7 @@
 #pragma once
 #include <cstdint>
 #include <cstdlib>
+#include <cstring>
 
 namespace dmx {
 namespace policy {
@@ -16,6 +17,8 @@
 constexpr int kVgaTileCSplit = 1;
 constexpr int kVgaTileCCert = 1;
 constexpr int kVgaTileWalk = 1;
+constexpr int kVgaPrepLegacyVis = 1, kVgaPrepLegacyPmask = 2, kVgaPrepLegacyCr = 4, kVgaPrepLegacyScan = 8;
+constexpr int kVgaScanLds = 8192;
 constexpr int kVgaDoAlpha = 15;
 constexpr int kVgaDoShortList = 16;
 
@@ -49,6 +52,24 @@
     const char* e = std::getenv(name);
     return e ? std::atoi(e) : dflt;
 }
+inline int prep_legacy() {
+    const char* e = std::getenv("DMX_VGA_PREP_LEGACY");
+    if (!e) return 0;
+    if (*e >= '0' && *e <= '9') return std::atoi(e) & 15;
+    int m = 0;
+    for (const char* p = e; *p;) {
+        const char* q = p;
+        while (*q >= 'a' && *q <= 'z') q++;
+        const size_t n = (size_t)(q - p);
+        if (n == 3 && !std::strncmp(p, "vis", 3)) m |= kVgaPrepLegacyVis;
+        else if (n == 5 && !std::strncmp(p, "pmask", 5)) m |= kVgaPrepLegacyPmask;
+        else if (n == 2 && !std::strncmp(p, "cr", 2)) m |= kVgaPrepLegacyCr;
+        else if (n == 4 && !std::strncmp(p, "scan", 4)) m |= kVgaPrepLegacyScan;
+        else if (n == 3 && !std::strncmp(p, "all", 3)) m |= 15;
+        p = *q ? q + 1 : q;
+    }
+    return m;
+}
 
 }
 }
diff --git a/depthmapx_amd/engine.py b/depthmapx_amd/engine.py
--- a/depthmapx_amd/engine.py
+++ b/depthmapx_amd/engine.py
@@ -177,8 +177,8 @@
         return dict(zip(["level1", "tile_common", "heads", "hard", "bookkeeping"], (int(v) for v in out)))
 
     def last_stats(self):
-        out = np.zeros(51, dtype=np.int64)
-        N.check(N.lib().dmx_ctx_last_stats(self.h, N.ptr(out), 51))
+        out = np.zeros(53, dtype=np.int64)
+        N.check(N.lib().dmx_ctx_last_stats(self.h, N.ptr(out), 53))
         keys = ["mk_cells_examined", "mk_visible_pairs", "mk_runs", "vga_kernel", "vga_runs_expanded", "vga_levels",
                 "vga_cells_reached", "vga_sources", "vga_fail_cells", "vga_fail_runs", "vga_hbm_bitmaps",
                 "vga_cr_tiles", "vga_launch", "vga_pruned_cells", "vga_tvis_bytes", "vga_hard_runs", "vga_hard_hits",
@@ -186,7 +186,7 @@
                 "vga_b_cell_cycles", "vga_b_ext_cells", "mk_depth_steps", "mk_chunks", "mk_reruns", "vga_pmask_loads", "vga_pmask_cells", "vga_pmask_bytes",
                 "vga_order_reruns", "vga_sym_scatter_us", "vga_prep_flags", "vga_tile_rows_bytes", "vga_scan_bytes",
                 "vga_asym_nodes", "tv_lines", "tv_pixel_steps", "tv_window", "mk_diag_inexact", "vga_tl_max", "vga_c_row_cells",
-                "vga_c_cert_cells"]
+                "vga_c_cert_cells", "vga_prep_us", "vga_scan_twopass"]
         d = {k: int(v) for k, v in zip(keys, out)}
         lv = d.pop("vga_levels")
         d["vga_bottom_up_levels"], d["vga_top_down_levels"] = lv & 0xFFFFFFFF, lv >> 32
@@ -337,6 +337,22 @@
         out = np.zeros(max(n.value, 1), dtype=np.int32)
         N.check(N.lib().dmx_graph_special_nodes(self.h, N.ptr(out), ctypes.byref(n)))
         return out[:n.value]
+
+    _PREP_ARRAYS = [("tvis", np.uint64, 0), ("ftvis", np.uint64, 0), ("ttvis", np.uint64, 0), ("tvblk", np.uint64, 0),
+                    ("ppre", np.uint16, 0), ("poff", np.int64, 0), ("pmask", np.uint64, 0), ("cr", np.int16, 4),
+                    ("heads", np.int16, 4), ("tscan_start", np.int64, 0), ("tnruns", np.int32, 0),
+                    ("scan_pool", np.int16, 4), ("scan_start", np.int64, 0)]
+
+    def vga_prep_arrays(self):
+        out = {}
+        for which, (name, dt, ncol) in enumerate(self._PREP_ARRAYS):
+            nb = ctypes.c_int64(0)
+            N.check(N.lib().dmx_graph_vga_prep_copy(self.ctx.h, self.h, which, None, 0, ctypes.byref(nb)))
+            a = np.zeros(nb.value // np.dtype(dt).itemsize, dtype=dt)
+            if nb.value:
+                N.check(N.lib().dmx_graph_vga_prep_copy(self.ctx.h, self.h, which, N.ptr(a), nb.value, ctypes.byref(nb)))
+            out[name] = a.reshape(-1, ncol) if ncol else a
+        return out
 
     def copy(self, runs=True):
         i = self.info()
diff --git a/include/dmx.h b/include/dmx.h
--- a/include/dmx.h
+++ b/include/dmx.h
@@ -80,6 +80,8 @@
 int dmx_vga_global_device_list(dmx_ctx* ctx, dmx_graph* g, double radius, int gates_only, const int64_t* nodes,
                                int64_t n, float* out_device);
 int dmx_graph_special_nodes(dmx_graph* g, int32_t* nodes, int64_t* n);
+#define DMX_PREP_ARRAYS 13
+int dmx_graph_vga_prep_copy(dmx_ctx* ctx, dmx_graph* g, int32_t which, void* out, int64_t cap_bytes, int64_t* nbytes);
 int dmx_vga_metric(dmx_ctx* ctx, dmx_graph* g, double radius, int gates_only, int64_t src_begin, int64_t src_end,
                    float* out);
 int dmx_vga_angular(dmx_ctx* ctx, dmx_graph* g, double radius, int gates_only, int64_t src_begin, int64_t src_end,
```
